# renjie-liang/HUAL

Hardware: AMD Instinct MI355X
Metric: train clips/sec (higher is better)
Workload: dtype f32 (fp16x3 / bf16x3 split-operand MFMA, fp32 accumulate); 1 GPU; Charades-STA SeqPAN train step (fwd+bwd+clip+AdamWD, dropout 0.2), batch 64/GPU, T=128, vdim=1024, L=20, C=8, dim=128, 8 heads, 2 attention layers, random init; ONE batch resident in HBM, batch assembly (hual_assemble_batch) outside the timed region; global_batch=64, T=128, vdim=1024, L=20, parallelism=dp1, launch=hipGraph, video_dtype=f32

## Files before the change

hual_amd/csrc/heads.h:

```cpp
#pragma once
#include "common.h"
#include "rowops.h"

namespace hual {

enum { LA_MATCH_SUM = 0, LA_MASK_SUM = 1, LA_ORTHO = 2, LA_LOC = 3, LA_ALIGN = 4, LA_DENOM = 5 };

struct PoolArgs {
  const float* F2;
  const float* wp;
  const float* Wbot;
  float* alpha;
  float* pooled;
  float* PW;
};
struct AlignPool;
struct AlignPoolBwd;
int launch_pool_align_fwd(const PoolArgs& a, const AlignPool* ap, const RowSpace& rs, hipStream_t s);
struct PoolBwd {
  const float* dFuse;
  float* dPW;
  float* dF2;
  float* dwp;
};
int launch_pool_align_bwd(const PoolArgs& a, const PoolBwd& g, const AlignPool& ap, const AlignPoolBwd& ab, const RowSpace& rs, hipStream_t s);

struct MatchArgs {
  const float* fuse;
  const float* Wm;
  const float* bm;
  const float* E;
  const int32_t* labels;
  float* probs;
  float* probs2;
  float* outputs;
  float* loss_acc;
  float* part;
  const uint32_t* rng;
  float inv_tau;
};
int match_fwd_blocks(int Nv);
struct AlignSim;
int launch_match_fwd(const MatchArgs& a, const RowSpace& rs, const AlignSim* as, hipStream_t s);
struct LossTailArgs {
  float* loss_acc; const float* match_part; int match_nblk; const float* loc_part; int loc_nblk;
  float lambda, override_denom; const float* denom_dev; float* loss_out;
  const uint32_t* ovf; int novf;
  const float* align_rows; int nalign;
};
struct MatchBwd {
  const float* dOut;
  const float* dOut2;
  float* dFuse;
  float* dWm; float* dbm; float* dE;
  const float* dE_ortho;
  float* part;
  float lambda;
  int do_tail; LossTailArgs tail;
};
int match_bwd_blocks(int Nv);
int launch_match_bwd(const MatchArgs& a, const MatchBwd& g, const RowSpace& rs, hipStream_t s);
struct HeadsArgs {
  const float* h[2]; const float* w[2]; const float* b[2];
  float* logit[2];
  const float* vmask;
  const float* y1; const float* y2;
  int64_t* start_index; int64_t* end_index;
  float* ds; float* de;
  int grad_only;
  float* dZ[2];
  float* part[2];
  float* loc_part;
  float inv_batch;
  const uint32_t* ovf; int novf;
};
int launch_heads(const HeadsArgs& a, int B, int T, hipStream_t s);
int launch_loss_tail(const LossTailArgs& a, hipStream_t s);

struct AlignPool {
  const float* F2;
  const float* F1;
  const float* inner;
  float* tpre; float* vpre;
  float* that; float* vhat;
  int ld;
};
struct AlignSim {
  const float* that; const float* vhat; int Bg;
  float* dq; float* da;
  float* row_loss;
  float* dthat; float* dvhat;
  float* loss_acc;
  float scale;
  int ld;
  int row0, nrows;
};
int launch_align_sim(const AlignSim& a, hipStream_t s);
struct AlignPoolBwd {
  const float* dthat; const float* dvhat;
  float* dF2;
  float* dF1;
  const float* col_dq; const float* col_da; int col_Bg;
};

}
```

hual_amd/csrc/heads.hip:

```cpp
#include "heads.h"
#include "philox.h"
#include "prof.h"

using namespace hual;

#if defined(HUAL_STAMPS) && HUAL_STAMPS == 8
static __device__ unsigned long long g_heads_stamps[512 * 64];
extern "C" int hual_debug_stamps(unsigned long long* out, int n) {
  return (int)hipMemcpyFromSymbol(out, HIP_SYMBOL(g_heads_stamps), sizeof(unsigned long long) * (size_t)n);
}
#define HEADS_STAMP(i) do { if (threadIdx.x == 0 && blockIdx.x < 512) g_heads_stamps[blockIdx.x * 64 + (i)] = __builtin_readcyclecounter(); } while (0)
#else
#define HEADS_STAMP(i) do { } while (0)
#endif

__device__ __forceinline__ float block_sum(float v, float* sm) {
  v = wave_sum64(v);
  const int w = threadIdx.x >> 6;
  __syncthreads();
  if ((threadIdx.x & 63) == 0) sm[w] = v;
  __syncthreads();
  float s = 0.f;
  for (int i = 0; i < (int)(blockDim.x >> 6); ++i) s += sm[i];
  return s;
}
__device__ __forceinline__ double block_sum_d(double v, double* sm) {
  for (int off = 32; off >= 1; off >>= 1) v += __shfl_xor(v, off);
  const int w = threadIdx.x >> 6;
  __syncthreads();
  if ((threadIdx.x & 63) == 0) sm[w] = v;
  __syncthreads();
  double s = 0.0;
  for (int i = 0; i < (int)(blockDim.x >> 6); ++i) s += sm[i];
  return s;
}
__device__ __forceinline__ float block_max(float v, float* sm) {
  v = wave_max64(v);
  const int w = threadIdx.x >> 6;
  __syncthreads();
  if ((threadIdx.x & 63) == 0) sm[w] = v;
  __syncthreads();
  float s = -INFINITY;
  for (int i = 0; i < (int)(blockDim.x >> 6); ++i) s = fmaxf(s, sm[i]);
  return s;
}

__device__ __forceinline__ void pool_fwd_body(const PoolArgs& a, const RowSpace& rs, int b) {
  __shared__ float al[256];
  __shared__ float pooled[HUAL_D];
  __shared__ float part[HUAL_D];
  const int tid = threadIdx.x;
  const bool on = tid < 256;
  const int l32 = tid & 31, grp = tid >> 5;
  const int L = rs.L;
  const float* F = a.F2 + (size_t)(rs.Nv + b * L) * HUAL_D;
  const float* m = rs.rowmask + rs.Nv + b * L;
  if (on) {
    const float4 w4 = ld4(a.wp + 4 * l32);
    for (int l = grp; l < L; l += 8) {
      const float4 f = ld4(F + (size_t)l * HUAL_D + 4 * l32);
      const float d = half_sum32(f.x * w4.x + f.y * w4.y + f.z * w4.z + f.w * w4.w);
      if (l32 == 0) al[l] = d * m[l] + HUAL_MASK_VALUE * (1.0f - m[l]);
    }
  }
  __syncthreads();
  float mx = -INFINITY;
  for (int l = 0; l < L; ++l) mx = fmaxf(mx, al[l]);
  float sum = 0.f;
  for (int l = 0; l < L; ++l) sum += __expf(al[l] - mx);
  const float inv = 1.0f / sum;
  const int c = tid & 127, half = (tid >> 7) & 1;
  if (on && half == 0) {
    float p = 0.f;
    for (int l = 0; l < L; ++l) {
      const float alpha = __expf(al[l] - mx) * inv;
      if (c == 0) a.alpha[b * L + l] = alpha;
      p = fmaf(alpha, F[(size_t)l * HUAL_D + c], p);
    }
    pooled[c] = p;
    a.pooled[b * HUAL_D + c] = p;
  }
  __syncthreads();
  float o = 0.f;
  if (on) {
#pragma unroll 8
    for (int k = half * 64; k < half * 64 + 64; ++k) o = fmaf(pooled[k], a.Wbot[(size_t)k * HUAL_D + c], o);
    if (half) part[c] = o;
  }
  __syncthreads();
  if (on && !half) a.PW[b * HUAL_D + c] = o + part[c];
}

__device__ __forceinline__ float gumbel_noise(uint32_t w) {
  const float u = (float)(w >> 8) * 5.9604644775390625e-08f;
  return -logf(-logf(u + 1e-20f) + 1e-20f);
}
__device__ __forceinline__ void match_fwd_body(const MatchArgs& a, const RowSpace& rs, int bid, int nblk) {
  __shared__ float red[2][8];
  const int l32 = threadIdx.x & 31, grp = threadIdx.x >> 5;
  const int col = 4 * l32;
  float ce_sum = 0.f, m_sum = 0.f;
  float4 w0 = ld4(a.Wm + (col + 0) * 4), w1 = ld4(a.Wm + (col + 1) * 4), w2 = ld4(a.Wm + (col + 2) * 4), w3 = ld4(a.Wm + (col + 3) * 4);
  const float4 bm = ld4(a.bm);
  float4 e0 = ld4(a.E + col), e1 = ld4(a.E + HUAL_D + col), e2 = ld4(a.E + 2 * HUAL_D + col), e3 = ld4(a.E + 3 * HUAL_D + col);
  uint3 gk = make_uint3(0u, 0u, 0u);
  if (a.rng) gk = make_uint3(a.rng[0], a.rng[1], a.rng[2]);
  for (int row = bid * 8 + grp; row < rs.Nv; row += nblk * 8) {
    const size_t off = (size_t)row * HUAL_D + col;
    const float4 f = ld4(a.fuse + off);
    float l0 = f.x * w0.x + f.y * w1.x + f.z * w2.x + f.w * w3.x;
    float l1 = f.x * w0.y + f.y * w1.y + f.z * w2.y + f.w * w3.y;
    float l2 = f.x * w0.z + f.y * w1.z + f.z * w2.z + f.w * w3.z;
    float l3 = f.x * w0.w + f.y * w1.w + f.z * w2.w + f.w * w3.w;
    l0 = half_sum32(l0) + bm.x; l1 = half_sum32(l1) + bm.y; l2 = half_sum32(l2) + bm.z; l3 = half_sum32(l3) + bm.w;
    if (a.rng) {
      const uint4_ r = philox4x32(0u, (uint32_t)row, (uint32_t)HUAL_SITE_GUMBEL, gk.z, gk.x, gk.y);
      l0 = (l0 + gumbel_noise(r.x)) * a.inv_tau; l1 = (l1 + gumbel_noise(r.y)) * a.inv_tau;
      l2 = (l2 + gumbel_noise(r.z)) * a.inv_tau; l3 = (l3 + gumbel_noise(r.w)) * a.inv_tau;
    }
    const float mx = fmaxf(fmaxf(l0, l1), fmaxf(l2, l3));
    const float x0 = expf(l0 - mx), x1 = expf(l1 - mx), x2 = expf(l2 - mx), x3 = expf(l3 - mx);
    const float sum = x0 + x1 + x2 + x3;
    const float inv = 1.0f / sum;
    const float p0 = x0 * inv, p1 = x1 * inv, p2 = x2 * inv, p3 = x3 * inv;
    const float mk = rs.rowmask[row];
    if (l32 == 0) {
      *reinterpret_cast<float4*>(a.probs + (size_t)row * 4) = make_float4(p0, p1, p2, p3);
      if (a.probs2) *reinterpret_cast<float4*>(a.probs2 + (size_t)row * 4) = make_float4(p0, p1, p2, p3);
      if (a.labels) {
        const int lab = a.labels[row];
        const float ll = lab == 0 ? l0 : (lab == 1 ? l1 : (lab == 2 ? l2 : l3));
        ce_sum += (mx + logf(sum) - ll) * mk;
        m_sum += mk;
      }
    }
    float4 o = make_float4((f.x + p0 * e0.x + p1 * e1.x + p2 * e2.x + p3 * e3.x) * mk,
                           (f.y + p0 * e0.y + p1 * e1.y + p2 * e2.y + p3 * e3.y) * mk,
                           (f.z + p0 * e0.z + p1 * e1.z + p2 * e2.z + p3 * e3.z) * mk,
                           (f.w + p0 * e0.w + p1 * e1.w + p2 * e2.w + p3 * e3.w) * mk);
    st4(a.outputs + off, o);
  }
  if (a.labels && a.loss_acc) {
    if (l32 == 0) { red[0][grp] = ce_sum; red[1][grp] = m_sum; }
    __syncthreads();
    if (threadIdx.x == 0) {
      float c = 0.f, m = 0.f;
      for (int i = 0; i < 8; ++i) { c += red[0][i]; m += red[1][i]; }
      if (a.part) { a.part[2 * bid] = c; a.part[2 * bid + 1] = m; }
      else { atomicAdd(a.loss_acc + LA_MATCH_SUM, c); atomicAdd(a.loss_acc + LA_MASK_SUM, m); }
    }
  }
}

__device__ __forceinline__ float loss_tail_body(const LossTailArgs& a, float* sm, bool write);
__global__ __launch_bounds__(256) void match_bwd_kernel(MatchArgs a, MatchBwd g, RowSpace rs) {
  __shared__ float4 red[8][8][32];
  __shared__ float redb[8][4];
  const int l32 = threadIdx.x & 31, grp = threadIdx.x >> 5;
  const int col = 4 * l32;
  float4 w0 = ld4(a.Wm + (col + 0) * 4), w1 = ld4(a.Wm + (col + 1) * 4), w2 = ld4(a.Wm + (col + 2) * 4), w3 = ld4(a.Wm + (col + 3) * 4);
  float4 e0 = ld4(a.E + col), e1 = ld4(a.E + HUAL_D + col), e2 = ld4(a.E + 2 * HUAL_D + col), e3 = ld4(a.E + 3 * HUAL_D + col);
  const int row0 = min((int)blockIdx.x * 8 + grp, rs.Nv - 1);
  const size_t off0 = (size_t)row0 * HUAL_D + col;
  float pmk = rs.rowmask[row0];
  float4 pd = ld4(g.dOut + off0), pd2 = g.dOut2 ? ld4(g.dOut2 + off0) : f4zero();
  float4 pf = ld4(a.fuse + off0), pp = *reinterpret_cast<const float4*>(a.probs + (size_t)row0 * 4);
  float denom = 1.0f;
  if (g.do_tail) {
    __shared__ float smt[12];
    denom = loss_tail_body(g.tail, smt, blockIdx.x == 0);
  } else if (a.labels) {
    denom = a.loss_acc[LA_DENOM];
  }
  const float ce_scale = a.labels ? g.lambda / denom : 0.f;
  float4 dE0 = f4zero(), dE1 = f4zero(), dE2 = f4zero(), dE3 = f4zero();
  float4 dW0 = f4zero(), dW1 = f4zero(), dW2 = f4zero(), dW3 = f4zero();
  float db0 = 0.f, db1 = 0.f, db2 = 0.f, db3 = 0.f;
  for (int row = blockIdx.x * 8 + grp; row < rs.Nv; row += gridDim.x * 8) {
    const size_t off = (size_t)row * HUAL_D + col;
    const float mk = pmk;
    float4 d = pd;
    if (g.dOut2) d = make_float4(d.x + pd2.x, d.y + pd2.y, d.z + pd2.z, d.w + pd2.w);
    const float4 f = pf, p = pp;
    {
      const int rn = min(row + (int)gridDim.x * 8, rs.Nv - 1);
      const size_t offn = (size_t)rn * HUAL_D + col;
      pmk = rs.rowmask[rn];
      pd = ld4(g.dOut + offn);
      if (g.dOut2) pd2 = ld4(g.dOut2 + offn);
      pf = ld4(a.fuse + offn);
      pp = *reinterpret_cast<const float4*>(a.probs + (size_t)rn * 4);
    }
    d = make_float4(d.x * mk, d.y * mk, d.z * mk, d.w * mk);
    float q0 = half_sum32(d.x * e0.x + d.y * e0.y + d.z * e0.z + d.w * e0.w);
    float q1 = half_sum32(d.x * e1.x + d.y * e1.y + d.z * e1.z + d.w * e1.w);
    float q2 = half_sum32(d.x * e2.x + d.y * e2.y + d.z * e2.z + d.w * e2.w);
    float q3 = half_sum32(d.x * e3.x + d.y * e3.y + d.z * e3.z + d.w * e3.w);
    const float dot = p.x * q0 + p.y * q1 + p.z * q2 + p.w * q3;
    float dl0 = p.x * (q0 - dot), dl1 = p.y * (q1 - dot), dl2 = p.z * (q2 - dot), dl3 = p.w * (q3 - dot);
    if (a.labels) {
      const int lab = a.labels[row];
      const float cs = ce_scale * mk;
      dl0 += cs * (p.x - (lab == 0 ? 1.f : 0.f));
      dl1 += cs * (p.y - (lab == 1 ? 1.f : 0.f));
      dl2 += cs * (p.z - (lab == 2 ? 1.f : 0.f));
      dl3 += cs * (p.w - (lab == 3 ? 1.f : 0.f));
    }
    if (a.rng) { dl0 *= a.inv_tau; dl1 *= a.inv_tau; dl2 *= a.inv_tau; dl3 *= a.inv_tau; }
    st4(g.dFuse + off, make_float4(d.x + dl0 * w0.x + dl1 * w0.y + dl2 * w0.z + dl3 * w0.w,
                                   d.y + dl0 * w1.x + dl1 * w1.y + dl2 * w1.z + dl3 * w1.w,
                                   d.z + dl0 * w2.x + dl1 * w2.y + dl2 * w2.z + dl3 * w2.w,
                                   d.w + dl0 * w3.x + dl1 * w3.y + dl2 * w3.z + dl3 * w3.w));
    dE0 = make_float4(dE0.x + p.x * d.x, dE0.y + p.x * d.y, dE0.z + p.x * d.z, dE0.w + p.x * d.w);
    dE1 = make_float4(dE1.x + p.y * d.x, dE1.y + p.y * d.y, dE1.z + p.y * d.z, dE1.w + p.y * d.w);
    dE2 = make_float4(dE2.x + p.z * d.x, dE2.y + p.z * d.y, dE2.z + p.z * d.z, dE2.w + p.z * d.w);
    dE3 = make_float4(dE3.x + p.w * d.x, dE3.y + p.w * d.y, dE3.z + p.w * d.z, dE3.w + p.w * d.w);
    dW0 = make_float4(dW0.x + f.x * dl0, dW0.y + f.y * dl0, dW0.z + f.z * dl0, dW0.w + f.w * dl0);
    dW1 = make_float4(dW1.x + f.x * dl1, dW1.y + f.y * dl1, dW1.z + f.z * dl1, dW1.w + f.w * dl1);
    dW2 = make_float4(dW2.x + f.x * dl2, dW2.y + f.y * dl2, dW2.z + f.z * dl2, dW2.w + f.w * dl2);
    dW3 = make_float4(dW3.x + f.x * dl3, dW3.y + f.y * dl3, dW3.z + f.z * dl3, dW3.w + f.w * dl3);
    if (l32 == 0) { db0 += dl0; db1 += dl1; db2 += dl2; db3 += dl3; }
  }
  red[0][grp][l32] = dE0; red[1][grp][l32] = dE1; red[2][grp][l32] = dE2; red[3][grp][l32] = dE3;
  red[4][grp][l32] = dW0; red[5][grp][l32] = dW1; red[6][grp][l32] = dW2; red[7][grp][l32] = dW3;
  if (l32 == 0) { redb[grp][0] = db0; redb[grp][1] = db1; redb[grp][2] = db2; redb[grp][3] = db3; }
  __syncthreads();
  float* part = g.part + (size_t)blockIdx.x * 9 * HUAL_D;
  for (int idx = threadIdx.x; idx < 8 * 128; idx += 256) {
    const int vec = idx >> 7, c = idx & 127;
    float s = 0.f;
#pragma unroll
    for (int k = 0; k < 8; ++k) s += reinterpret_cast<const float*>(&red[vec][k][c >> 2])[c & 3];
    if (vec < 4) {
      if (g.dE_ortho && blockIdx.x == 0) s += g.dE_ortho[vec * HUAL_D + c];
      part[vec * HUAL_D + c] = s;
    } else {
      part[4 * HUAL_D + c * 4 + (vec - 4)] = s;
    }
  }
  if (threadIdx.x < HUAL_D) {
    float s = 0.f;
    if (threadIdx.x < 4)
      for (int k = 0; k < 8; ++k) s += redb[k][threadIdx.x];
    part[8 * HUAL_D + threadIdx.x] = s;
  }
}

__device__ __forceinline__ void block_max2(float& a, float& b, float* sm) {
  a = wave_max64(a); b = wave_max64(b);
  const int w = threadIdx.x >> 6, nw = blockDim.x >> 6;
  __syncthreads();
  if ((threadIdx.x & 63) == 0) { sm[w] = a; sm[nw + w] = b; }
  __syncthreads();
  float x = -INFINITY, y = -INFINITY;
  for (int i = 0; i < nw; ++i) { x = fmaxf(x, sm[i]); y = fmaxf(y, sm[nw + i]); }
  a = x; b = y;
}
__device__ __forceinline__ void block_sum2_d(double& a, double& b, double* sm) {
  for (int off = 32; off >= 1; off >>= 1) { a += __shfl_xor(a, off); b += __shfl_xor(b, off); }
  const int w = threadIdx.x >> 6, nw = blockDim.x >> 6;
  __syncthreads();
  if ((threadIdx.x & 63) == 0) { sm[w] = a; sm[nw + w] = b; }
  __syncthreads();
  double x = 0.0, y = 0.0;
  for (int i = 0; i < nw; ++i) { x += sm[i]; y += sm[nw + i]; }
  a = x; b = y;
}
__device__ __forceinline__ void block_sum3(float& a, float& b, float& c, float* sm) {
  a = wave_sum64(a); b = wave_sum64(b); c = wave_sum64(c);
  const int w = threadIdx.x >> 6, nw = blockDim.x >> 6;
  __syncthreads();
  if ((threadIdx.x & 63) == 0) { sm[w] = a; sm[nw + w] = b; sm[2 * nw + w] = c; }
  __syncthreads();
  float x = 0.f, y = 0.f, z = 0.f;
  for (int i = 0; i < nw; ++i) { x += sm[i]; y += sm[nw + i]; z += sm[2 * nw + i]; }
  a = x; b = y; c = z;
}

template <int NR>
__global__ __launch_bounds__(512) void heads_kernel(HeadsArgs a, int T, int B) {
  __shared__ float zs_[256], ze_[256], ps[256], pe[256], dls[256], dle[256];
  __shared__ float sm[24];
  __shared__ double smd[16];
  __shared__ float wtot[2][4];
  __shared__ float bestv[2][4];
  __shared__ int besti[2][4];
  __shared__ float4 red[2][16][32];
  __shared__ float redb[2][16];
  const int b = xcd_tile(blockIdx.x, gridDim.x), tid = threadIdx.x;
  if (b >= B) return;
  const int l32 = tid & 31, grp = tid >> 5;
  const int col = 4 * l32;
  HEADS_STAMP(0);
  float4 hs[NR], he[NR];
  float4 ws = f4zero(), we = f4zero();
  float poison = 0.f;
  if (a.ovf) {
    bool bad = false;
    for (int i = tid & 63; i < a.novf; i += 64) bad |= a.ovf[i] != 0u;
    if (__any(bad)) poison = __builtin_nanf("");
  }
  if (a.h[0]) {
    ws = ld4(a.w[0] + col); we = ld4(a.w[1] + col);
#pragma unroll
    for (int u = 0; u < NR; ++u) {
      const int t = min(grp + 16 * u, T - 1);
      hs[u] = ld4(a.h[0] + (size_t)(b * T + t) * HUAL_D + col);
      he[u] = ld4(a.h[1] + (size_t)(b * T + t) * HUAL_D + col);
    }
  }
  if (a.grad_only) {
    if (tid < T) { dls[tid] = a.ds[b * T + tid]; dle[tid] = a.de[b * T + tid]; }
  } else if (a.h[0]) {
    const float bs = a.b[0][0] + poison, be = a.b[1][0] + poison;
#pragma unroll
    for (int u = 0; u < NR; ++u) {
      const int t = grp + 16 * u;
      const float ds = half_sum32(hs[u].x * ws.x + hs[u].y * ws.y + hs[u].z * ws.z + hs[u].w * ws.w) + bs;
      const float de = half_sum32(he[u].x * we.x + he[u].y * we.y + he[u].z * we.z + he[u].w * we.w) + be;
      if (l32 == 0 && t < T) { zs_[t] = ds; ze_[t] = de; a.logit[0][b * T + t] = ds; a.logit[1][b * T + t] = de; }
    }
  } else if (tid < T) {
    zs_[tid] = a.logit[0][b * T + tid];
    ze_[tid] = a.logit[1][b * T + tid];
  }
  __syncthreads();
  HEADS_STAMP(1);
  if (!a.grad_only) {
    const int t = tid;
    const bool in = t < T;
    const float m = in ? a.vmask[b * T + t] : 0.f;
    float zs = -INFINITY, ze = -INFINITY;
    if (in) {
      zs = zs_[t] * m + HUAL_MASK_VALUE * (1.0f - m);
      ze = ze_[t] * m + HUAL_MASK_VALUE * (1.0f - m);
    }
    float mxs = zs, mxe = ze;
    block_max2(mxs, mxe, sm);
    const float xs = in ? (float)exp((double)(zs - mxs)) : 0.f;
    const float xe = in ? (float)exp((double)(ze - mxe)) : 0.f;
    double dss = (double)xs, dse = (double)xe;
    block_sum2_d(dss, dse, smd);
    const float sums = (float)dss, sume = (float)dse;
    const float p_s = __fdiv_rn(xs, sums), p_e = __fdiv_rn(xe, sume);
    HEADS_STAMP(2);
    if (a.y1) {
      const float y1 = in ? a.y1[b * T + t] : 0.f, y2 = in ? a.y2[b * T + t] : 0.f;
      const float lsm_s = zs - mxs - logf(sums), lsm_e = ze - mxe - logf(sume);
      float lsum = in ? -(y1 * lsm_s + y2 * lsm_e) : 0.f, y1s = y1, y2s = y2;
      block_sum3(lsum, y1s, y2s, sm);
      if (t == 0 && a.loc_part) a.loc_part[b] = lsum * a.inv_batch;
      if (in) {
        const float ds = (p_s * y1s - y1) * m * a.inv_batch, de = (p_e * y2s - y2) * m * a.inv_batch;
        dls[t] = ds; dle[t] = de;
        if (a.ds) { a.ds[b * T + t] = ds; a.de[b * T + t] = de; }
      }
    }
    HEADS_STAMP(3);
    if (tid < 256) {
      const int lane = tid & 63, w = tid >> 6;
      float pre = in ? p_s : 0.f, suf = in ? p_e : 0.f;
#pragma unroll
      for (int off = 1; off < 64; off <<= 1) {
        const float up = __shfl_up(pre, off), dn = __shfl_down(suf, off);
        if (lane >= off) pre = fmaxf(pre, up);
        if (lane + off < 64) suf = fmaxf(suf, dn);
      }
      if (lane == 63) wtot[0][w] = pre;
      if (lane == 0) wtot[1][w] = suf;
      ps[tid] = pre; pe[tid] = suf;
    }
    const int nanlogit = __syncthreads_or(in && (zs_[t] != zs_[t] || ze_[t] != ze_[t]));
    float vs = -1.f, ve = -1.f;
    if (in) {
      const int w = t >> 6;
      float premax = ps[t], sufmax = pe[t];
      for (int k = 0; k < w; ++k) premax = fmaxf(premax, wtot[0][k]);
      for (int k = w + 1; k < 4; ++k) sufmax = fmaxf(sufmax, wtot[1][k]);
      vs = p_s * sufmax;
      ve = premax * p_e;
    }
    if (tid < 256) {
      int is = t, ie = t;
      for (int off = 32; off >= 1; off >>= 1) {
        float ovs = __shfl_xor(vs, off); int ois = __shfl_xor(is, off);
        if (ovs > vs || (ovs == vs && ois < is)) { vs = ovs; is = ois; }
        float ove = __shfl_xor(ve, off); int oie = __shfl_xor(ie, off);
        if (ove > ve || (ove == ve && oie < ie)) { ve = ove; ie = oie; }
      }
      if ((t & 63) == 0) { bestv[0][t >> 6] = vs; besti[0][t >> 6] = is; bestv[1][t >> 6] = ve; besti[1][t >> 6] = ie; }
    }
    __syncthreads();
    if (t == 0) {
      float v = bestv[0][0]; int i = besti[0][0];
      for (int w = 1; w < 4; ++w) if (bestv[0][w] > v || (bestv[0][w] == v && besti[0][w] < i)) { v = bestv[0][w]; i = besti[0][w]; }
      a.start_index[b] = i;
      v = bestv[1][0]; i = besti[1][0];
      for (int w = 1; w < 4; ++w) if (bestv[1][w] > v || (bestv[1][w] == v && besti[1][w] < i)) { v = bestv[1][w]; i = besti[1][w]; }
      a.end_index[b] = i;
      if (poison != poison || nanlogit) { a.start_index[b] = -1; a.end_index[b] = -1; }
    }
  } else {
    __syncthreads();
  }
  HEADS_STAMP(4);
  HEADS_STAMP(5);
  if (a.dZ[0] && (a.y1 || a.grad_only)) {
    float4 dws = f4zero(), dwe = f4zero();
    float dbs = 0.f, dbe = 0.f;
#pragma unroll
    for (int u = 0; u < NR; ++u) {
      const int tt = grp + 16 * u;
      if (tt >= T) continue;
      const size_t off = (size_t)(b * T + tt) * HUAL_D + col;
      const float dl0 = dls[tt], dl1 = dle[tt];
      st4(a.dZ[0] + off, make_float4(hs[u].x > 0.f ? dl0 * ws.x : 0.f, hs[u].y > 0.f ? dl0 * ws.y : 0.f, hs[u].z > 0.f ? dl0 * ws.z : 0.f,
                                     hs[u].w > 0.f ? dl0 * ws.w : 0.f));
      st4(a.dZ[1] + off, make_float4(he[u].x > 0.f ? dl1 * we.x : 0.f, he[u].y > 0.f ? dl1 * we.y : 0.f, he[u].z > 0.f ? dl1 * we.z : 0.f,
                                     he[u].w > 0.f ? dl1 * we.w : 0.f));
      dws = make_float4(dws.x + dl0 * hs[u].x, dws.y + dl0 * hs[u].y, dws.z + dl0 * hs[u].z, dws.w + dl0 * hs[u].w);
      dwe = make_float4(dwe.x + dl1 * he[u].x, dwe.y + dl1 * he[u].y, dwe.z + dl1 * he[u].z, dwe.w + dl1 * he[u].w);
      if (l32 == 0) { dbs += dl0; dbe += dl1; }
    }
    red[0][grp][l32] = dws; red[1][grp][l32] = dwe;
    if (l32 == 0) { redb[0][grp] = dbs; redb[1][grp] = dbe; }
    __syncthreads();
    if (tid < 256) {
      const int hd = tid >> 7, c = tid & 127;
      float sw = 0.f;
#pragma unroll
      for (int k = 0; k < 16; ++k) sw += reinterpret_cast<const float*>(&red[hd][k][c >> 2])[c & 3];
      float sb = 0.f;
      if (c == 0)
        for (int k = 0; k < 16; ++k) sb += redb[hd][k];
      float* part = a.part[hd] + (size_t)b * 2 * HUAL_D;
      part[c] = sw;
      part[HUAL_D + c] = sb;
    }
  }
  HEADS_STAMP(6);
}

__device__ __forceinline__ float loss_tail_body(const LossTailArgs& a, float* sm, bool write) {
  const int tid = threadIdx.x;
  float cs = 0.f, ms = 0.f, ls = 0.f;
  for (int i = tid; i < a.match_nblk; i += 256) { cs += a.match_part[2 * i]; ms += a.match_part[2 * i + 1]; }
  if (write)
    for (int i = tid; i < a.loc_nblk; i += 256) ls += a.loc_part[i];
  int bad = 0;
  if (write) {
    for (int i = tid; i < a.novf; i += 256) bad |= a.ovf[i] != 0u;
    bad = __syncthreads_or(bad);
  }
  block_sum3(cs, ms, ls, sm);
  const float denom = a.denom_dev ? *a.denom_dev : (a.override_denom > 0.f ? a.override_denom : ms + 1e-12f);
  if (write && tid == 0) {
    float* la = a.loss_acc;
    la[LA_MATCH_SUM] = cs; la[LA_MASK_SUM] = ms; la[LA_LOC] = ls;
    la[LA_DENOM] = denom;
    if (a.align_rows) {
      float l = 0.f;
      for (int i = 0; i < a.nalign; ++i) l += a.align_rows[i];
      la[LA_ALIGN] = l;
    }
    if (a.loss_out) {
      const float match = cs / denom + la[LA_ORTHO];
      const float align = la[LA_ALIGN];
      const float poison = bad ? __builtin_nanf("") : 0.f;
      a.loss_out[0] = ls + a.lambda * match + align + poison;
      a.loss_out[1] = ls + poison;
      a.loss_out[2] = match + poison;
      a.loss_out[3] = align + poison;
    }
  }
  return denom;
}
__global__ __launch_bounds__(256) void loss_tail_kernel(LossTailArgs a) {
  __shared__ float sm[12];
  loss_tail_body(a, sm, true);
}

#define L2_EPS 1e-12f
__device__ __forceinline__ void align_pool_body(const AlignPool& a, const RowSpace& rs, int b) {
  __shared__ float sm[8];
  __shared__ float part[2][4][HUAL_D];
  const int c = threadIdx.x & 127, grp = threadIdx.x >> 7;
  const int L = rs.L, T = rs.T;
  float tc = 0.f, vc = 0.f;
  for (int l = threadIdx.x; l < L; l += 512) tc += rs.rowmask[rs.Nv + b * L + l];
  for (int t = threadIdx.x; t < T; t += 512) vc += rs.rowmask[b * T + t];
  tc = block_sum(tc, sm);
  vc = block_sum(vc, sm);
  float ts = 0.f, vs = 0.f;
#pragma unroll 8
  for (int l = grp; l < L; l += 4) ts += a.F2[(size_t)(rs.Nv + b * L + l) * HUAL_D + c];
#pragma unroll 8
  for (int t = grp; t < T; t += 4) vs += a.F1[(size_t)(b * T + t) * HUAL_D + c] * (a.inner[b * T + t] / vc);
  part[0][grp][c] = ts;
  part[1][grp][c] = vs;
  __syncthreads();
  ts = part[0][0][c] + part[0][1][c] + part[0][2][c] + part[0][3][c];
  vs = part[1][0][c] + part[1][1][c] + part[1][2][c] + part[1][3][c];
  const float tp = ts / tc;
  const float tn = block_sum(grp == 0 ? tp * tp : 0.f, sm);
  const float vn = block_sum(grp == 0 ? vs * vs : 0.f, sm);
  if (grp == 0) {
    a.tpre[b * HUAL_D + c] = tp;
    a.vpre[b * HUAL_D + c] = vs;
    a.that[(size_t)b * a.ld + c] = tp * rsqrtf(fmaxf(tn, L2_EPS));
    a.vhat[(size_t)b * a.ld + c] = vs * rsqrtf(fmaxf(vn, L2_EPS));
  }
}

__device__ __forceinline__ double block_max_d(double v, double* sm) {
  for (int off = 32; off >= 1; off >>= 1) v = fmax(v, __shfl_xor(v, off));
  const int w = threadIdx.x >> 6;
  __syncthreads();
  if ((threadIdx.x & 63) == 0) sm[w] = v;
  __syncthreads();
  double s = sm[0];
  for (int i = 1; i < (int)(blockDim.x >> 6); ++i) s = fmax(s, sm[i]);
  return s;
}
__device__ __forceinline__ void align_sim_rows_body(const AlignSim& a, int i) {
  __shared__ float ti[HUAL_D], vi[HUAL_D];
  __shared__ double sm[4];
  __shared__ double sa[1024], sq[1024];
  const int tid = threadIdx.x, Bg = a.Bg;
  const int ld = a.ld;
  if (tid < HUAL_D) { ti[tid] = a.that[(size_t)i * ld + tid]; vi[tid] = a.vhat[(size_t)i * ld + tid]; }
  __syncthreads();
  double mxa = -INFINITY, mxq = -INFINITY;
  for (int j0 = 0; j0 < Bg; j0 += 64) {
    const int j = j0 + (tid >> 2), kq = (tid & 3) * 32;
    const float* vj = a.vhat + (size_t)min(j, Bg - 1) * ld + kq;
    double da = 0.0, dq = 0.0;
#pragma unroll 8
    for (int k = 0; k < 32; ++k) { const double v = (double)vj[k]; da = fma((double)vi[kq + k], v, da); dq = fma((double)ti[kq + k], v, dq); }
    da += __shfl_xor(da, 1); dq += __shfl_xor(dq, 1);
    da += __shfl_xor(da, 2); dq += __shfl_xor(dq, 2);
    if ((tid & 3) == 0 && j < Bg) { sa[j] = da; sq[j] = dq; }
  }
  __syncthreads();
  for (int j = tid; j < Bg; j += 256) { mxa = fmax(mxa, sa[j]); mxq = fmax(mxq, sq[j]); }
  mxa = block_max_d(mxa, sm);
  mxq = block_max_d(mxq, sm);
  double suma = 0.0, sumq = 0.0;
  for (int j = tid; j < Bg; j += 256) { suma += exp(sa[j] - mxa); sumq += exp(sq[j] - mxq); }
  suma = block_sum_d(suma, sm);
  sumq = block_sum_d(sumq, sm);
  const double lsa = mxa + log(suma), lsq = mxq + log(sumq);
  double li = 0.0, dotq = 0.0, dota = 0.0;
  for (int j = tid; j < Bg; j += 256) {
    const double lpv = sa[j] - lsa, lpq = sq[j] - lsq;
    const double pv = exp(lpv), pq = exp(lpq);
    li += pq * lpq + pv * lpv - 2.0 * pq * pv;
    dotq += pq * (lpq + 1.0 - 2.0 * pv);
    dota += pv * (lpv + 1.0 - 2.0 * pq);
  }
  li = block_sum_d(li, sm);
  dotq = block_sum_d(dotq, sm);
  dota = block_sum_d(dota, sm);
  if (tid == 0) {
    if (a.row_loss) a.row_loss[i] = (float)li;
    else if (a.loss_acc) atomicAdd(a.loss_acc + LA_ALIGN, (float)li);
  }
  __syncthreads();
  for (int j = tid; j < Bg; j += 256) {
    const double lpv = sa[j] - lsa, lpq = sq[j] - lsq;
    const double pv = exp(lpv), pq = exp(lpq);
    const double gq = pq * ((lpq + 1.0 - 2.0 * pv) - dotq) * (double)a.scale;
    const double ga = pv * ((lpv + 1.0 - 2.0 * pq) - dota) * (double)a.scale;
    a.dq[(size_t)i * Bg + j] = (float)gq;
    a.da[(size_t)i * Bg + j] = (float)ga;
    sq[j] = gq; sa[j] = ga;
  }
  __syncthreads();
  if (tid < HUAL_D && i >= a.row0 && i < a.row0 + a.nrows) {
    double st = 0.0, sv = 0.0;
#pragma unroll 8
    for (int j = 0; j < Bg; ++j) {
      const double v = (double)a.vhat[(size_t)j * ld + tid];
      st = fma(sq[j], v, st);
      sv = fma(sa[j], v, sv);
    }
    a.dthat[(i - a.row0) * HUAL_D + tid] = (float)st;
    a.dvhat[(i - a.row0) * HUAL_D + tid] = (float)sv;
  }
}
__global__ __launch_bounds__(256) void align_sim_rows_kernel(AlignSim a) { align_sim_rows_body(a, blockIdx.x); }
__global__ __launch_bounds__(256) void match_align_fwd_kernel(MatchArgs ma, RowSpace rs, AlignSim as, int nmatch) {
  if ((int)blockIdx.x < nmatch) match_fwd_body(ma, rs, blockIdx.x, nmatch);
  else align_sim_rows_body(as, (int)blockIdx.x - nmatch);
}
__global__ __launch_bounds__(256) void align_sim_cols_kernel(AlignSim a) {
  __shared__ float cq[1024], ca[1024];
  __shared__ float part[HUAL_D];
  const int j = a.row0 + blockIdx.x, c = threadIdx.x & 127, half = threadIdx.x >> 7, Bg = a.Bg, ld = a.ld;
  for (int i = threadIdx.x; i < Bg; i += 256) { cq[i] = a.dq[(size_t)i * Bg + j]; ca[i] = a.da[(size_t)i * Bg + j]; }
  __syncthreads();
  float s = 0.f;
#pragma unroll 4
  for (int i = half; i < Bg; i += 2)
    s += cq[i] * a.that[(size_t)i * ld + c] + ca[i] * a.vhat[(size_t)i * ld + c];
  if (half) part[c] = s;
  __syncthreads();
  if (!half) a.dvhat[blockIdx.x * HUAL_D + c] += s + part[c];
  if (a.row_loss && blockIdx.x == 0 && threadIdx.x == 0) {
    float l = 0.f;
    for (int i = 0; i < Bg; ++i) l += a.row_loss[i];
    a.loss_acc[LA_ALIGN] = l;
  }
}

__global__ __launch_bounds__(512) void pool_align_fwd_kernel(PoolArgs pa, AlignPool ap, RowSpace rs) {
  const int clip = xcd_tile(blockIdx.x, gridDim.x);
  if (clip >= rs.B) return;
  if (blockIdx.y == 0) {
    pool_fwd_body(pa, rs, clip);
  } else {
    align_pool_body(ap, rs, clip);
  }
}
template <int KT, int KL>
__global__ __launch_bounds__(512) void pool_align_bwd_kernel(PoolArgs pa, PoolBwd pb, AlignPool ap, AlignPoolBwd ab, RowSpace rs) {
  __shared__ float sm[48];
  __shared__ float part[4][HUAL_D];
  __shared__ float vecs[2][HUAL_D];
  __shared__ float da[256], al[256], qm[256], dap[2][256];
  const int b = xcd_tile(blockIdx.x, gridDim.x), tid = threadIdx.x;
  if (b >= rs.B) return;
  const int c = tid & 127, grp = tid >> 7;
  const int L = rs.L, T = rs.T;
  const size_t vrow0 = (size_t)b * T, qrow0 = (size_t)rs.Nv + (size_t)b * L;
  __shared__ float inl[256];
  float rdf[KT], rf1[KT], rF[KL];
#pragma unroll
  for (int k = 0; k < KT; ++k) {
    const int t = min(grp + 4 * k, T - 1);
    rdf[k] = pb.dFuse[(vrow0 + t) * HUAL_D + c];
    rf1[k] = ab.dF1[(vrow0 + t) * HUAL_D + c];
  }
  for (int t = tid; t < T; t += 512) inl[t] = ap.inner[vrow0 + t];
#pragma unroll
  for (int k = 0; k < KL; ++k) rF[k] = pa.F2[(qrow0 + min(grp + 4 * k, L - 1)) * HUAL_D + c];
  const float tp = ap.tpre[b * HUAL_D + c], vp = ap.vpre[b * HUAL_D + c];
  const float th = ap.that[(size_t)b * ap.ld + c], vh = ap.vhat[(size_t)b * ap.ld + c];
  const float dth = ab.dthat[b * HUAL_D + c];
  float dvh = ab.dvhat[b * HUAL_D + c];
  const float wpc = pa.wp[c];
  float tc = 0.f, vc = 0.f;
  for (int l = tid; l < L; l += 512) { const float m = rs.rowmask[qrow0 + l]; qm[l] = m; al[l] = pa.alpha[b * L + l]; tc += m; }
  for (int t = tid; t < T; t += 512) vc += rs.rowmask[vrow0 + t];
  float colsum = 0.f;
  if (ab.col_dq) {
    const int Bg = ab.col_Bg;
#pragma unroll 4
    for (int i = grp; i < Bg; i += 4)
      colsum += ab.col_dq[(size_t)i * Bg + b] * ap.that[(size_t)i * ap.ld + c] + ab.col_da[(size_t)i * Bg + b] * ap.vhat[(size_t)i * ap.ld + c];
  }
  float sdf = 0.f;
#pragma unroll
  for (int k = 0; k < KT; ++k) sdf += (grp + 4 * k < T) ? rdf[k] : 0.f;
  part[grp][c] = sdf;
  __syncthreads();
  const float dpw = (part[0][c] + part[1][c]) + (part[2][c] + part[3][c]);
  if (grp == 0) { pb.dPW[b * HUAL_D + c] = dpw; vecs[1][c] = dpw; }
  __syncthreads();
  if (ab.col_dq) {
    part[grp][c] = colsum;
    __syncthreads();
    dvh += (part[0][c] + part[1][c]) + (part[2][c] + part[3][c]);
    __syncthreads();
  }
  {
    const float w0 = grp == 0 ? 1.f : 0.f;
    float v[6] = {w0 * tp * tp, w0 * vp * vp, w0 * th * dth, w0 * vh * dvh, tc, vc};
#pragma unroll
    for (int q = 0; q < 6; ++q) v[q] = wave_sum64(v[q]);
    if ((tid & 63) == 0)
      for (int q = 0; q < 6; ++q) sm[q * 8 + (tid >> 6)] = v[q];
  }
  __syncthreads();
  float red6[6];
#pragma unroll
  for (int q = 0; q < 6; ++q) {
    float x = 0.f;
    for (int w = 0; w < 8; ++w) x += sm[q * 8 + w];
    red6[q] = x;
  }
  const float tn = red6[0], vn = red6[1], tdot = red6[2], vdot = red6[3];
  tc = red6[4]; vc = red6[5];
  const float rt = rsqrtf(fmaxf(tn, L2_EPS)), rv = rsqrtf(fmaxf(vn, L2_EPS));
  const float dtp = tn > L2_EPS ? (float)((double)rt * ((double)dth - (double)th * (double)tdot)) : rt * dth;
  const float dvp = vn > L2_EPS ? (float)((double)rv * ((double)dvh - (double)vh * (double)vdot)) : rv * dvh;
  const float dts = dtp / tc;
#pragma unroll
  for (int k = 0; k < KT; ++k) {
    const int t = grp + 4 * k;
    if (t < T) ab.dF1[(vrow0 + t) * HUAL_D + c] = rf1[k] + dvp * (inl[t] / vc);
  }
  {
    float dp = 0.f;
    const float* wrow = pa.Wbot + (size_t)c * HUAL_D + grp * 32;
#pragma unroll
    for (int n = 0; n < 32; n += 4) {
      const float4 w = ld4(wrow + n);
      const float* d = vecs[1] + grp * 32 + n;
      dp += d[0] * w.x + d[1] * w.y + d[2] * w.z + d[3] * w.w;
    }
    part[grp][c] = dp;
  }
  __syncthreads();
  const float dpc = (part[0][c] + part[1][c]) + (part[2][c] + part[3][c]);
  __syncthreads();
#pragma unroll
  for (int k = 0; k < KL; ++k) {
    const int l = grp + 4 * k;
    const float d = wave_sum64(dpc * rF[k]);
    if ((tid & 63) == 0 && l < L) dap[(tid >> 6) & 1][l] = d;
  }
  __syncthreads();
  if (tid < L) da[tid] = dap[0][tid] + dap[1][tid];
  __syncthreads();
  float dot_acc = 0.f;
  for (int l = 0; l < L; ++l) dot_acc += al[l] * da[l];
  float dw = 0.f;
#pragma unroll
  for (int k = 0; k < KL; ++k) {
    const int l = grp + 4 * k;
    if (l >= L) continue;
    const float alpha = al[l];
    const float dal = alpha * (da[l] - dot_acc) * qm[l];
    ab.dF2[(qrow0 + l) * HUAL_D + c] = dts + alpha * dpc + dal * wpc;
    dw = fmaf(dal, rF[k], dw);
  }
  part[grp][c] = dw;
  __syncthreads();
  if (grp == 0) atomicAdd(pb.dwp + c, (part[0][c] + part[1][c]) + (part[2][c] + part[3][c]));
}

namespace hual {

int launch_pool_align_fwd(const PoolArgs& a, const AlignPool* ap, const RowSpace& rs, hipStream_t s) {
  HUAL_REQUIRE(rs.L <= 256, "pool: L <= 256");
  AlignPool z{};
  HUAL_LAUNCH(0.0, 512.0 * (rs.Nq + (ap ? rs.R : 0) + 4.0 * rs.B), pool_align_fwd_kernel, dim3(xcd_round8(rs.B), ap ? 2 : 1), dim3(512), 0, s, a, ap ? *ap : z, rs);
  HUAL_CHECK_HIP(hipGetLastError());
  return 0;
}
int launch_pool_align_bwd(const PoolArgs& a, const PoolBwd& g, const AlignPool& ap, const AlignPoolBwd& ab, const RowSpace& rs, hipStream_t s) {
  HUAL_REQUIRE(rs.T <= 256 && rs.L <= 256, "pool_align_bwd: T, L <= 256");
  HUAL_REQUIRE(ab.dF2 == g.dF2, "pool_align_bwd: the two parts write the same query rows");
  const double pab = 512.0 * (3.0 * rs.Nv + 2.0 * rs.Nq);
#define PAB(KT, KL) HUAL_LAUNCH(0.0, pab, (pool_align_bwd_kernel<KT, KL>), dim3(xcd_round8(rs.B)), dim3(512), 0, s, a, g, ap, ab, rs)
  if (rs.T <= 128) {
    if (rs.L <= 32) PAB(32, 8); else if (rs.L <= 64) PAB(32, 16); else if (rs.L <= 128) PAB(32, 32); else PAB(64, 64);
  } else {
    if (rs.L <= 32) PAB(64, 8); else if (rs.L <= 64) PAB(64, 16); else if (rs.L <= 128) PAB(64, 32); else PAB(64, 64);
  }
#undef PAB
  HUAL_CHECK_HIP(hipGetLastError());
  return 0;
}
static int rowgrid(int R, int cap) {
  int g = cdiv(R, 8);
  return g < cap ? (g > 0 ? g : 1) : cap;
}
int match_fwd_blocks(int Nv) { return rowgrid(Nv, 512); }
int match_bwd_blocks(int Nv) { return rowgrid(Nv, 256); }
int launch_match_fwd(const MatchArgs& a, const RowSpace& rs, const AlignSim* as, hipStream_t s) {
  HUAL_REQUIRE(a.part != nullptr, "match_fwd: partial-sum scratch");
  const int nm = match_fwd_blocks(rs.Nv);
  AlignSim z{};
  if (as) {
    HUAL_REQUIRE(as->Bg >= 1 && as->Bg <= 1024 && as->ld >= HUAL_D && as->row0 == 0 && as->nrows == as->Bg, "align: global batch <= 1024");
    z = *as;
  }
  HUAL_LAUNCH(0.0, (1024.0 + 32.0) * rs.Nv, match_align_fwd_kernel, dim3(nm + (as ? as->Bg : 0)), dim3(256), 0, s, a, rs, z, nm);
  HUAL_CHECK_HIP(hipGetLastError());
  return 0;
}
int launch_match_bwd(const MatchArgs& a, const MatchBwd& g, const RowSpace& rs, hipStream_t s) {
  HUAL_REQUIRE(g.part != nullptr, "match_bwd: partial-sum scratch");
  HUAL_LAUNCH(0.0, 4.0 * 512.0 * rs.Nv, match_bwd_kernel, dim3(match_bwd_blocks(rs.Nv)), dim3(256), 0, s, a, g, rs);
  HUAL_CHECK_HIP(hipGetLastError());
  return 0;
}
int launch_heads(const HeadsArgs& a, int B, int T, hipStream_t s) {
  HUAL_REQUIRE(T >= 1 && T <= 256 && B >= 1, "heads: T <= 256");
  HUAL_REQUIRE(a.grad_only ? (a.ds && a.de && a.dZ[0]) : (a.logit[0] && a.logit[1] && a.vmask && a.start_index && a.end_index), "heads: null tensor");
  HUAL_REQUIRE(!a.h[0] || (a.h[1] && a.w[0] && a.w[1] && a.b[0] && a.b[1]), "heads: hidden layers incomplete");
  HUAL_REQUIRE(!a.dZ[0] || (a.dZ[1] && a.part[0] && a.part[1] && a.h[0]), "heads: gradient outputs incomplete");
  const double hb = (a.dZ[0] ? 4.0 : 2.0) * 512.0 * B * T + 16.0 * B * T;
  if (T <= 128) HUAL_LAUNCH(0.0, hb, heads_kernel<8>, dim3(xcd_round8(B)), dim3(512), 0, s, a, T, B);
  else HUAL_LAUNCH(0.0, hb, heads_kernel<16>, dim3(xcd_round8(B)), dim3(512), 0, s, a, T, B);
  HUAL_CHECK_HIP(hipGetLastError());
  return 0;
}
int launch_loss_tail(const LossTailArgs& a, hipStream_t s) {
  HUAL_REQUIRE(a.loss_acc && a.match_part && a.loc_part, "loss_tail: null");
  HUAL_LAUNCH(0.0, 0.0, loss_tail_kernel, dim3(1), dim3(256), 0, s, a);
  HUAL_CHECK_HIP(hipGetLastError());
  return 0;
}
int launch_align_sim(const AlignSim& a, hipStream_t s) {
  HUAL_REQUIRE(a.Bg >= 1 && a.Bg <= 1024, "align: global batch <= 1024");
  HUAL_REQUIRE(a.ld >= HUAL_D && a.row0 >= 0 && a.nrows >= 1 && a.row0 + a.nrows <= a.Bg, "align: row window / leading dimension");
  HUAL_LAUNCH(0.0, 0.0, align_sim_rows_kernel, dim3(a.Bg), dim3(256), 0, s, a);
  HUAL_LAUNCH(0.0, 0.0, align_sim_cols_kernel, dim3(a.nrows), dim3(256), 0, s, a);
  HUAL_CHECK_HIP(hipGetLastError());
  return 0;
}

}
```

hual_amd/csrc/mproj.hip:

```cpp
#include "mproj.h"
#include "tilecore.h"
#include "prof.h"
#include <cstdlib>
#include <cstddef>

using namespace hual;

#define ld4 ld4_global
#define st4 st4_global

#define MP_ROWS 64
enum { MPF_A2 = 1, MPF_BF16 = 2, MPF_DROP = 4, MPF_ADD = 8, MPF_LN = 16, MPF_REUSE = 32, MPF_QUAD = 64, MPF_POOL = 128 };

template <int NT, int F>
__device__ __forceinline__ void mproj_body(const MProjArgs& a, const DropCfg& drop, int tile = -1) {
  extern __shared__ __attribute__((aligned(16))) char mp_lds[];
  char* S0 = mp_lds;
  char* S1 = S0 + 2 * MP_ROWS * 256;
  float* ainv0 = reinterpret_cast<float*>(S1 + 2 * MP_ROWS * 256);
  float* ainv1 = ainv0 + MP_ROWS;
  const int lane = threadIdx.x & 63, wave = threadIdx.x >> 6;
  const int l32 = threadIdx.x & 31, grp = threadIdx.x >> 5;
  const int col = 4 * l32;
  const int MT = a.MT, R = a.R;
  if (tile < 0) {
    const int nblk = xcd_round8((R + MT - 1) / MT);
    if ((int)blockIdx.x >= nblk) return;
    tile = xcd_tile(blockIdx.x, nblk);
  }
  const int r0 = tile * MT;
  if (r0 >= R) return;
  const int RE = min(R, r0 + MT);
  const int j = lane & 15, g = lane >> 4, ecol = 16 * wave + 4 * g;
  const DropRegs dr = drop_load(drop);
  constexpr int NU = NT;

  constexpr int SW = sizeof(MProjStep) / 4;
  __shared__ uint32_t sdesc[MP_MAX * SW];
  {
    const uint32_t* ka = reinterpret_cast<const uint32_t*>(&a.s[0]);
    for (int i = threadIdx.x; i < a.nsteps * SW; i += CB_THREADS) sdesc[i] = ka[i];
  }
  __syncthreads();
  static_assert(SW <= 64, "a step descriptor fits one dword per lane");
  auto step_at = [&](int si) {
    struct alignas(8) Raw { uint32_t w[SW]; } r;
    const uint32_t mine = sdesc[si * SW + min(lane, SW - 1)];
#pragma unroll
    for (int q = 0; q < SW; ++q) r.w[q] = __builtin_amdgcn_readlane(mine, q);
    return __builtin_bit_cast(MProjStep, r);
  };
  int nflat = 0;
  for (int i = 0; i < a.nsteps; ++i) nflat += (int)__builtin_amdgcn_readfirstlane(sdesc[i * SW + offsetof(MProjStep, rep) / 4]);
  auto expand = [&](int si, int ri) {
    MProjStep st = step_at(si);
    if (st.rep > 1) {
      st.A = st.a_bf16 ? (const void*)(reinterpret_cast<const uint16_t*>(st.A) + 128 * ri) : (const void*)(reinterpret_cast<const float*>(st.A) + 128 * ri);
      st.kw = min(128, st.ktot - 128 * ri);
      st.col0 += 128 * ri;
      st.wimg = reinterpret_cast<const float*>(reinterpret_cast<const char*>(st.wimg) + (size_t)ri * 128 * 512);
      st.first = st.first && ri == 0;
      st.last = st.last && ri == st.rep - 1;
    }
    return st;
  };
  TfW wc, wn;
  tf_load_w(wc, step_at(0).wimg, wave, lane);
  float4 nv[NU], n2[NU];
  auto rows_load = [&](const MProjStep& st) {
    const int kc = min(col, max(st.kw - 4, 0));
#pragma unroll
    for (int u = 0; u < NU; ++u) {
      const size_t row = (size_t)min(r0 + grp + 16 * u, R - 1);
      if ((F & MPF_BF16) && st.a_bf16) {
        const uint2 raw = ld2_global(reinterpret_cast<const uint16_t*>(st.A) + row * st.lda + kc);
        nv[u] = make_float4(__uint_as_float(raw.x), __uint_as_float(raw.y), 0.f, 0.f);
      } else {
        nv[u] = ld4(reinterpret_cast<const float*>(st.A) + row * st.lda + kc);
      }
      if (F & MPF_A2) {
        const float* p2 = st.A2 ? st.A2 : reinterpret_cast<const float*>(st.A);
        const int ld2 = st.A2 ? st.lda2 : st.lda;
        n2[u] = ld4(p2 + row * ld2 + kc);
      }
    }
  };
  auto fill = [&](const MProjStep& st, int slot) {
    char* S = slot ? S1 : S0;
    float* ai = slot ? ainv1 : ainv0;
    const bool cin = col < st.kw;
    uint32_t nb[4] = {15u, 15u, 15u, 15u};
    constexpr int NPR = (NU + 1) / 2;
    if ((F & MPF_DROP) && st.drop_site >= 0 && dr.enabled) {
      const uint32_t c4 = (uint32_t)((st.col0 + col) >> 2);
#pragma unroll
      for (int pr = 0; pr < NPR; ++pr) {
        const int lrA = grp + 32 * pr, lrB = lrA + 16;
        const bool okA = cin && lrA < MT && r0 + lrA < RE, okB = cin && lrB < MT && r0 + lrB < RE;
        uint32_t na, nbb;
        const uint32_t byte = drop_nib2_r(dr, (uint32_t)st.drop_site, a.drop_row0 + (uint32_t)(r0 + lrA), a.drop_row0 + (uint32_t)(r0 + lrB), c4, na, nbb);
        nb[2 * pr] = na; nb[2 * pr + 1] = nbb;
        if (st.keep_out) {
          const bool odd = (c4 & 1u) != 0u;
          if (odd ? okB : okA) st1b_global(st.keep_out + (size_t)(r0 + (odd ? lrB : lrA)) * st.ld_keep + (c4 >> 1), (uint8_t)byte);
        }
      }
    }
#pragma unroll
    for (int u = 0; u < NU; ++u) {
      const int lr = grp + 16 * u, row = r0 + lr;
      const bool ok = row < RE && cin && lr < MT;
      float4 v = nv[u];
      if ((F & MPF_BF16) && st.a_bf16) {
        const uint32_t w0 = __float_as_uint(v.x), w1 = __float_as_uint(v.y);
        v = make_float4(__uint_as_float(w0 << 16), __uint_as_float(w0 & 0xffff0000u), __uint_as_float(w1 << 16), __uint_as_float(w1 & 0xffff0000u));
      }
      if ((F & MPF_A2) && st.A2) v = cb_mul(v, n2[u]);
      if (!ok) v = f4zero();
      if ((F & MPF_DROP) && st.drop_site >= 0 && dr.enabled) v = f4_select(nb[u], make_float4(v.x * dr.scale, v.y * dr.scale, v.z * dr.scale, v.w * dr.scale));
      const float inv = cb_store_operand(S, S + MP_ROWS * 256, lr, l32, v);
      if (l32 == 0) ai[lr] = row < RE ? inv : 0.f;
    }
  };
#define MP_STAMP(i) HUAL_STAMP_K(9, i)
  MP_STAMP(0);
  MProjStep cur = expand(0, 0);
  rows_load(cur);
  fill(cur, 0);
  MP_STAMP(1);
  int slot = 0, si = 0, ri = 0;
  float4 acc[NT];
  float4 qd[(F & MPF_QUAD) ? 4 : 1][NT];
  float4 lastb = f4zero();
  constexpr bool QPRE = (F & MPF_QUAD) && NT <= 3;
  float4 qx[QPRE ? NT : 1], qc[QPRE ? NT : 1], qq[QPRE ? NT : 1];
  if (QPRE && a.quad_x) {
#pragma unroll
    for (int rt = 0; rt < NT; ++rt) {
      const size_t off = (size_t)min(r0 + 16 * rt + j, R - 1) * HUAL_D + ecol;
      qx[rt] = ld4(a.quad_x + off); qc[rt] = ld4(a.quad_c2q + off); qq[rt] = ld4(a.quad_q2c + off);
    }
  }
#pragma unroll
  for (int rt = 0; rt < NT; ++rt) acc[rt] = f4zero();
#pragma unroll 1
  for (int k = 0; k < nflat; ++k) {
    MP_STAMP(2 + 7 * k);
    const MProjStep st = cur;
    const bool more = k + 1 < nflat;
    MProjStep nxt = st;
    if (more) {
      if (++ri == (int)__builtin_amdgcn_readfirstlane(sdesc[si * SW + offsetof(MProjStep, rep) / 4])) { ri = 0; ++si; }
      nxt = expand(si, ri);
    }
    MP_STAMP(3 + 7 * k);
    const bool closes = st.last && st.out && ecol < st.ncol;
    const float* wdummy = st.wimg + 4 * lane;
    const float4 bias = ld4(st.bias ? st.bias + ecol : wdummy);
    float4 addv[NT];
    if (F & MPF_ADD) {
#pragma unroll
      for (int rt = 0; rt < NT; ++rt) {
        const int row = min(r0 + 16 * rt + j, R - 1);
        addv[rt] = ld4((st.add && closes) ? st.add + (size_t)(row / st.add_div) * st.ldadd + ecol : wdummy);
      }
    }
    tf_load_w(wn, nxt.wimg, wave, lane);
    bool refill = true;
    if (F & MPF_REUSE) {
      refill = more && !nxt.reuse;
      if (refill) rows_load(nxt);
    } else {
      rows_load(nxt);
    }
    MP_STAMP(4 + 7 * k);
    cb_barrier();
    MP_STAMP(5 + 7 * k);
    const char* S = slot ? S1 : S0;
    const float* ai = slot ? ainv1 : ainv0;
    f32x4 accp[NT];
    tf_mma<NT, MP_ROWS * 256>(S, wc, lane, accp);
    MP_STAMP(6 + 7 * k);
#pragma unroll
    for (int rt = 0; rt < NT; ++rt) {
      const float ir = ai[16 * rt + j];
      const float4 o = st.first ? f4zero() : acc[rt];
      acc[rt] = make_float4(fmaf(accp[rt][0], ir, o.x), fmaf(accp[rt][1], ir, o.y), fmaf(accp[rt][2], ir, o.z), fmaf(accp[rt][3], ir, o.w));
    }
    lastb = st.bias ? bias : f4zero();
    {
      float* outp = st.out ? st.out : const_cast<float*>(wdummy);
#pragma unroll
      for (int rt = 0; rt < NT; ++rt) {
        const int row = r0 + 16 * rt + j;
        float4 v = st.bias ? cb_add(acc[rt], bias) : acc[rt];
        if (st.act) v = relu_nan4(v);
        if ((F & MPF_ADD) && st.add) v = cb_add(v, addv[rt]);
        if (closes && 16 * rt + j < MT && row < RE) st4(outp + (size_t)row * st.ldo + ecol, v);
        if (F & MPF_QUAD) {
#pragma unroll
          for (int q = 0; q < 4; ++q) if (k == q) qd[q][rt] = v;
        }
      }
    }
    MP_STAMP(7 + 7 * k);
    if (refill && more) { slot ^= 1; fill(nxt, slot); }
    MP_STAMP(8 + 7 * k);
    wc = wn;
    cur = nxt;
  }
  if ((F & MPF_QUAD) && a.quad_x) {
#pragma unroll
    for (int rt = 0; rt < NT; ++rt) {
      const int row = r0 + 16 * rt + j;
      if (16 * rt + j >= MT || row >= RE) continue;
      const size_t off = (size_t)row * HUAL_D + ecol;
      const float4 x = QPRE ? qx[QPRE ? rt : 0] : ld4(a.quad_x + off), c2q = QPRE ? qc[QPRE ? rt : 0] : ld4(a.quad_c2q + off),
                   q2c = QPRE ? qq[QPRE ? rt : 0] : ld4(a.quad_q2c + off);
      const float4 d0 = qd[0][rt], d1 = qd[1][rt], d2 = qd[2][rt], d3 = qd[3][rt];
      st4(a.quad_dc2q + off, make_float4(d1.x + d2.x * x.x, d1.y + d2.y * x.y, d1.z + d2.z * x.z, d1.w + d2.w * x.w));
      st4(a.quad_dq2c + off, make_float4(d3.x * x.x, d3.y * x.y, d3.z * x.z, d3.w * x.w));
      st4(a.quad_dx + off, make_float4(d0.x + d2.x * c2q.x + d3.x * q2c.x, d0.y + d2.y * c2q.y + d3.y * q2c.y,
                                       d0.z + d2.z * c2q.z + d3.z * q2c.z, d0.w + d2.w * c2q.w + d3.w * q2c.w));
    }
    return;
  }
  if ((F & MPF_POOL) && a.pool_cat) {
    const float4 bias = lastb;
    const int C = a.pool_C;
#pragma unroll
    for (int rt = 0; rt < NT; ++rt) {
      const int lr = 16 * rt + j, row = r0 + lr;
      const int p = lr & (C - 1);
      const float4 v4 = cb_add(acc[rt], bias);
      const float vv[4] = {v4.x, v4.y, v4.z, v4.w};
      float best[4];
      int arg[4];
#pragma unroll
      for (int q = 0; q < 4; ++q) {
        const int ch = ecol + q;
        const int k = ch < 10 ? 1 : (ch < 30 ? 2 : (ch < 60 ? 3 : 4));
        best[q] = (p + k <= C) ? vv[q] : -INFINITY;
        arg[q] = p;
      }
      auto merge = [&](int step) {
#pragma unroll
        for (int q = 0; q < 4; ++q) {
          const float ov = dpp_xor_partner(best[q], step);
          const int oa = __builtin_bit_cast(int, dpp_xor_partner(__builtin_bit_cast(float, arg[q]), step));
          const bool take = ov > best[q] || (ov == best[q] && oa < arg[q]);
          best[q] = take ? ov : best[q];
          arg[q] = take ? oa : arg[q];
        }
      };
      if (C > 1) merge(1);
      if (C > 2) merge(2);
      if (C > 4) merge(4);
      if (C > 8) merge(8);
      if (p == 0 && lr < MT && row < RE && ecol < 100) {
        const int word = row / C;
        float o[4];
        int oa[4];
#pragma unroll
        for (int q = 0; q < 4; ++q) {
          const bool pos = best[q] > 0.f;
          o[q] = pos ? best[q] : 0.f;
          oa[q] = pos ? arg[q] : -1;
        }
        float* cp = a.pool_cat + (size_t)word * a.pool_ldcat + a.pool_col0 + ecol;
        if (((a.pool_ldcat | a.pool_col0) & 3) == 0) st4(cp, make_float4(o[0], o[1], o[2], o[3]));
        else { st1f_global(cp, o[0]); st1f_global(cp + 1, o[1]); st1f_global(cp + 2, o[2]); st1f_global(cp + 3, o[3]); }
        st4i_global(a.pool_arg + (size_t)word * 100 + ecol, oa[0], oa[1], oa[2], oa[3]);
      }
    }
    return;
  }
  if (!(F & MPF_LN) || !a.ln_g) return;
  float4* D0 = reinterpret_cast<float4*>(S0);
  cb_barrier();
  {
#pragma unroll
    for (int rt = 0; rt < NT; ++rt) D0[(16 * rt + j) * 32 + (ecol >> 2)] = cb_add(acc[rt], lastb);
  }
  const float4 gam = ld4(a.ln_g + col), bet = ld4(a.ln_b + col);
  cb_barrier();
#pragma unroll
  for (int u = 0; u < NU; ++u) {
    const int lr = grp + 16 * u, row = r0 + lr;
    if (lr >= MT || row >= RE) continue;
    const float4 x = D0[lr * 32 + l32];
    float mean, rstd;
    const float m0 = fast_sum32(cb_hsum(x)) * (1.0f / HUAL_D);
    const float4 d = make_float4(x.x - m0, x.y - m0, x.z - m0, x.w - m0);
    const float var = fast_sum32(cb_hsum(cb_mul(d, d))) * (1.0f / HUAL_D);
    mean = m0; rstd = rsqrtf(var + LN_EPS);
    float4 y = cb_fma(make_float4(d.x * rstd, d.y * rstd, d.z * rstd, d.w * rstd), gam, bet);
    if (a.pos) y = cb_add(y, ld4(a.pos + (size_t)((row + a.row_in_clip0) % a.Tc) * HUAL_D + col));
    const size_t off = (size_t)row * HUAL_D + col;
    if (a.x_out) st4(a.x_out + off, x);
    st4(a.y_out + off, y);
    if (l32 == 0) { st1f_global(a.mean + row, mean); st1f_global(a.rstd + row, rstd); }
  }
}

template <int NT, int F>
__global__ __launch_bounds__(CB_THREADS) void mproj_kernel(MProjArgs a, DropCfg drop) { mproj_body<NT, F>(a, drop); }
__host__ __device__ inline int mproj_pair_lo(int nb, int x) { return nb * x / 8; }
template <int NT, int F>
__global__ __launch_bounds__(CB_THREADS) void mproj_pair_kernel(MProjArgs a0, MProjArgs a1, DropCfg drop) {
  const int x = blockIdx.x & 7;
  int sl = blockIdx.x >> 3;
  const int nb0 = (a0.R + a0.MT - 1) / a0.MT, nb1 = (a1.R + a1.MT - 1) / a1.MT;
  const int lo0 = mproj_pair_lo(nb0, x), n0 = mproj_pair_lo(nb0, x + 1) - lo0;
  if (sl < n0) { mproj_body<NT, F>(a0, drop, lo0 + sl); return; }
  sl -= n0;
  const int lo1 = mproj_pair_lo(nb1, x), n1 = mproj_pair_lo(nb1, x + 1) - lo1;
  if (sl < n1) mproj_body<NT, F>(a1, drop, lo1 + sl);
}

#undef ld4
#undef st4

#if defined(HUAL_STAMPS) && HUAL_STAMPS == 9
extern "C" int hual_debug_stamps(unsigned long long* out, int n) {
  return (int)hipMemcpyFromSymbol(out, HIP_SYMBOL(g_hual_stamps), sizeof(unsigned long long) * (size_t)n);
}
#endif

namespace hual {

static int mproj_pair_grid(int R0, int R1, int t) {
  const int nb0 = cdiv(R0, t), nb1 = cdiv(R1, t);
  int m = 0;
  for (int x = 0; x < 8; ++x) {
    const int n = (mproj_pair_lo(nb0, x + 1) - mproj_pair_lo(nb0, x)) + (mproj_pair_lo(nb1, x + 1) - mproj_pair_lo(nb1, x));
    m = n > m ? n : m;
  }
  return 8 * m;
}
int mproj_rows(int R0, int R1) {
  int t = 16;
  if (R1 > 0) { while (t < MP_ROWS && mproj_pair_grid(R0, R1, t) > 256) ++t; }
  else { while (t < MP_ROWS && cdiv(R0, t) > 256) ++t; }
  return t;
}

static int check_mproj(const MProjArgs& a, double& flops, double& bytes, int& feat) {
  HUAL_REQUIRE(a.nsteps >= 1 && a.nsteps <= MP_MAX && a.R > 0 && a.MT >= 1 && a.MT <= MP_ROWS, "mproj: steps / rows");
  HUAL_REQUIRE(a.s[0].first && !a.s[0].reuse && a.s[a.nsteps - 1].last, "mproj: first step starts a tile, last step closes one");
  for (int k = 0; k < a.nsteps; ++k) {
    const MProjStep& s = a.s[k];
    HUAL_REQUIRE(s.rep >= 1 && (s.rep == 1 || (!s.reuse && s.ktot > 128 * (s.rep - 1) && s.ktot <= 128 * s.rep && (s.ktot % 4) == 0 && !s.A2)), "mproj: repetitions");
    HUAL_REQUIRE(s.reuse || (s.A && (s.rep > 1 || (s.kw >= 4 && s.kw <= 128 && (s.kw % 4) == 0)) && (s.lda % 4) == 0), "mproj: operand");
    HUAL_REQUIRE(!s.reuse || k > 0, "mproj: nothing to reuse");
    HUAL_REQUIRE(s.wimg && s.wrows >= 1, "mproj: weight image");
    feat |= (s.A2 ? MPF_A2 : 0) | (s.a_bf16 ? MPF_BF16 : 0) | (s.drop_site >= 0 ? MPF_DROP : 0) | (s.add ? MPF_ADD : 0) | (s.reuse ? MPF_REUSE : 0);
    HUAL_REQUIRE(!s.last || (a.ln_g && k == a.nsteps - 1 && !s.out) || (a.quad_x && !s.out) || (a.pool_cat && k == a.nsteps - 1 && !s.out) ||
                 (s.out && (s.ldo % 4) == 0 && s.ncol >= 4 && s.ncol <= 128 && (s.ncol % 4) == 0), "mproj: closing step needs a destination");
    HUAL_REQUIRE(!s.add || s.add_div >= 1, "mproj: add_div");
    HUAL_REQUIRE(k == 0 || s.first == a.s[k - 1].last, "mproj: a tile starts exactly behind a closed one");
    const double kdeep = s.rep > 1 ? s.ktot : (s.reuse ? a.s[k - 1].kw : s.kw);
    flops += 2.0 * a.R * kdeep * 128.0;
    if (!s.reuse) bytes += (s.a_bf16 ? 2.0 : 4.0) * a.R * kdeep + (s.A2 ? 4.0 * a.R * kdeep : 0.0);
    bytes += 4.0 * 128.0 * (s.rep > 1 ? s.ktot : (s.wrows < 128 ? s.wrows : 128));
    if (s.last && s.out) bytes += 4.0 * a.R * s.ncol;
  }
  if (a.quad_x) {
    feat |= MPF_QUAD;
    HUAL_REQUIRE(a.nsteps == 4 && a.quad_c2q && a.quad_q2c && a.quad_dc2q && a.quad_dq2c && a.quad_dx && !a.ln_g, "mproj: quad epilogue");
    for (int k = 0; k < 4; ++k) HUAL_REQUIRE(a.s[k].first && a.s[k].last && a.s[k].rep == 1 && !a.s[k].out, "mproj: quad epilogue takes four closing steps");
    bytes += 4.0 * a.R * 128.0 * 6.0;
  }
  if (a.pool_cat) {
    feat |= MPF_POOL;
    const int C = a.pool_C;
    HUAL_REQUIRE(a.pool_arg && (C == 1 || C == 2 || C == 4 || C == 8 || C == 16) && (a.MT % C) == 0 && (a.R % C) == 0 && !a.ln_g && !a.quad_x,
                 "mproj: pool epilogue needs a power-of-two window count <= 16 that divides the rows of a workgroup");
    bytes += 8.0 * (a.R / C) * 100.0;
  }
  if (a.ln_g) {
    feat |= MPF_LN;
    HUAL_REQUIRE(a.ln_b && a.y_out && a.mean && a.rstd && (!a.pos || a.Tc >= 1), "mproj: layer-norm outputs");
    bytes += 4.0 * a.R * 128.0 * (a.x_out ? 2.0 : 1.0);
  }
  return 0;
}

int launch_mproj(const MProjArgs* a, int nprob, const DropCfg& drop, hipStream_t s) {
  HUAL_REQUIRE(a && (nprob == 1 || nprob == 2), "mproj: one or two problems");
  double flops = 0.0, bytes = 0.0;
  int blocks = 0, feat = 0;
  for (int i = 0; i < nprob; ++i) {
    int rc = check_mproj(a[i], flops, bytes, feat);
    if (rc) return rc;
    const int nb = cdiv(a[i].R, a[i].MT);
    blocks = nb > blocks ? nb : blocks;
  }
  blocks = xcd_round8(blocks);
  const size_t lds = (size_t)4 * MP_ROWS * 256 + 2 * MP_ROWS * sizeof(float);
  if (nprob == 2) HUAL_REQUIRE(a[0].MT == a[1].MT, "mproj: problems of one launch share the rows per workgroup");
  const int nt = (a[0].MT + 15) / 16;
  const int fsets[] = {0, MPF_REUSE, MPF_A2, MPF_ADD, MPF_REUSE | MPF_ADD, MPF_A2 | MPF_BF16 | MPF_DROP | MPF_ADD | MPF_LN | MPF_REUSE,
                       MPF_REUSE | MPF_QUAD};
  int fs = 5;
  for (int i = 4; i >= 0; --i) if ((feat & ~fsets[i]) == 0) fs = i;
  if (feat & MPF_QUAD) {
    HUAL_REQUIRE((feat & ~fsets[6]) == 0, "mproj: the quad epilogue goes with plain / reused operands only");
    fs = 6;
  }
  if (feat & MPF_POOL) {
    HUAL_REQUIRE(feat == MPF_POOL, "mproj: the pool epilogue goes with plain operands only");
    fs = 7;
  }
#define MPROJ_LAUNCH(NT, FS)                                                                                               \
  do {                                                                                                                     \
    HUAL_DYN_LDS((mproj_kernel<NT, FS>), 96 * 1024);                                                                       \
    HUAL_DYN_LDS((mproj_pair_kernel<NT, FS>), 96 * 1024);                                                                  \
    if (nprob == 1) HUAL_LAUNCH(flops, bytes, (mproj_kernel<NT, FS>), dim3(blocks), dim3(CB_THREADS), lds, s, a[0], drop); \
    else HUAL_LAUNCH(flops, bytes, (mproj_pair_kernel<NT, FS>), dim3(mproj_pair_grid(a[0].R, a[1].R, a[0].MT)), dim3(CB_THREADS), lds, s, a[0], a[1], drop); \
  } while (0)
#define MPROJ_NT(FS)                                                                                                       \
  do {                                                                                                                     \
    if (nt <= 2) MPROJ_LAUNCH(2, FS);                                                                                      \
    else if (nt == 3) MPROJ_LAUNCH(3, FS);                                                                                 \
    else MPROJ_LAUNCH(4, FS);                                                                                              \
  } while (0)
  static_assert(MPF_A2 == 1 && MPF_ADD == 8 && MPF_REUSE == 32 && MPF_QUAD == 64 && MPF_POOL == 128 && (MPF_A2 | MPF_BF16 | MPF_DROP | MPF_ADD | MPF_LN | MPF_REUSE) == 63,
                "feature-set literals below");
  switch (fs) {
    case 0: MPROJ_NT(0); break;
    case 1: MPROJ_NT(32); break;
    case 2: MPROJ_NT(1); break;
    case 3: MPROJ_NT(8); break;
    case 4: MPROJ_NT(40); break;
    case 6: MPROJ_NT(96); break;
    case 7: MPROJ_NT(128); break;
    default: MPROJ_NT(63); break;
  }
#undef MPROJ_NT
#undef MPROJ_LAUNCH
  HUAL_CHECK_HIP(hipGetLastError());
  return 0;
}

}
```

hual_amd/csrc/prof.cpp:

```cpp
#include <stdlib.h>
#include "prof.h"
#include <map>
#include <string>
#include <vector>
#include <string.h>
#include "../../include/hual_seqpan.h"

namespace hual {

namespace {
struct Rec { std::string name; hipEvent_t a, b; double flops, bytes; };
struct Agg { std::string name; int64_t launches = 0; double usec = 0.0, flops = 0.0, bytes = 0.0; };
struct State {
  bool on = false;
  std::vector<Rec> recs;
  std::vector<Agg> aggs;
};
thread_local State g_prof;

std::string clean(const char* s) {
  std::string n(s);
  while (!n.empty() && (n.front() == '(' || n.front() == ' ')) n.erase(n.begin());
  while (!n.empty() && (n.back() == ')' || n.back() == ' ')) n.pop_back();
  return n;
}
}

bool prof_on() { return g_prof.on; }
bool lds_poison_on() {
  static const bool on = getenv("HUAL_DEBUG_LDS_POISON") != nullptr && atoi(getenv("HUAL_DEBUG_LDS_POISON")) != 0;
  return on;
}

void prof_events(const char* name, double flops, double bytes, hipEvent_t* start, hipEvent_t* stop) {
  *start = *stop = nullptr;
  hipEvent_t a, b;
  if (hipEventCreate(&a) != hipSuccess) return;
  if (hipEventCreate(&b) != hipSuccess) { hipEventDestroy(a); return; }
  g_prof.recs.push_back(Rec{clean(name), a, b, flops, bytes});
  *start = a;
  *stop = b;
}

}

extern "C" {

int hual_prof_begin(void) {
  hual::g_prof.on = true;
  hual::g_prof.recs.clear();
  hual::g_prof.aggs.clear();
  return 0;
}

int hual_prof_end(void) {
  using namespace hual;
  g_prof.on = false;
  std::map<std::string, size_t> idx;
  g_prof.aggs.clear();
  for (auto& r : g_prof.recs) {
    hipEventSynchronize(r.b);
    float ms = 0.f;
    const bool ok = hipEventElapsedTime(&ms, r.a, r.b) == hipSuccess;
    auto it = idx.find(r.name);
    if (it == idx.end()) {
      it = idx.emplace(r.name, g_prof.aggs.size()).first;
      g_prof.aggs.push_back(Agg{r.name});
    }
    Agg& a = g_prof.aggs[it->second];
    if (ok) { a.launches += 1; a.usec += (double)ms * 1e3; a.flops += r.flops; a.bytes += r.bytes; }
    hipEventDestroy(r.a);
    hipEventDestroy(r.b);
  }
  g_prof.recs.clear();
  return (int)g_prof.aggs.size();
}

int hual_prof_get(int i, char* name, int name_cap, int64_t* launches, double* usec, double* flops, double* bytes) {
  using namespace hual;
  if (i < 0 || i >= (int)g_prof.aggs.size() || !name || name_cap < 1) return HUAL_ERR_INVALID;
  const Agg& a = g_prof.aggs[i];
  strncpy(name, a.name.c_str(), (size_t)name_cap - 1);
  name[name_cap - 1] = 0;
  if (launches) *launches = a.launches;
  if (usec) *usec = a.usec;
  if (flops) *flops = a.flops;
  if (bytes) *bytes = a.bytes;
  return 0;
}

int hual_prof_kernel_pipe(const char* kernel, int* pipe, int* passes) {
  if (!kernel || !pipe || !passes) return HUAL_ERR_INVALID;
  struct Row { const char* prefix; int pipe, passes; };
  static const Row rows[] = {
      {"conv_block_", HUAL_PIPE_MATRIX16, 3}, {"ln_proj", HUAL_PIPE_MATRIX16, 3}, {"da_post", HUAL_PIPE_MATRIX16, 3},
      {"da_mid_bwd", HUAL_PIPE_MATRIX16, 3},  {"ln2_mid_bwd", HUAL_PIPE_MATRIX16, 3}, {"mproj_", HUAL_PIPE_MATRIX16, 3},
      {"feature_", HUAL_PIPE_MATRIX16, 3},    {"dw_f16_", HUAL_PIPE_MATRIX16, 3},
      {"attn_", HUAL_PIPE_MATRIX16, 3},      {"cq_fwd_staged", HUAL_PIPE_MATRIX16, 3}, {"cq_bwd_staged", HUAL_PIPE_MATRIX16, 3},
      {"cq_fwd_wide", HUAL_PIPE_MATRIX16, 3}, {"cq_bwd_wide", HUAL_PIPE_MATRIX16, 3},
      {"cq_", HUAL_PIPE_MATRIX32, 1},
  };
  for (const Row& r : rows)
    if (strncmp(kernel, r.prefix, strlen(r.prefix)) == 0) { *pipe = r.pipe; *passes = r.passes; return 0; }
  *pipe = HUAL_PIPE_NONE; *passes = 0;
  return 0;
}

}
```

hual_amd/csrc/seqpan.hip:

```cpp
#include "attn.h"
#include "prof.h"
#include "cq.h"
#include "convblock.h"
#include "dablock.h"
#include "embed.h"
#include "gemm.h"
#include "heads.h"
#include "mproj.h"
#include "optim.h"
#include "params.h"
#include "rowops.h"
#include <stdlib.h>
#include <string.h>
#include <algorithm>
#include <unordered_map>
#include <vector>

namespace hual {
const char* last_error_cstr();
}
using namespace hual;

namespace {

// ... 68 lines not shown
  int part_seq = 0;
  void stage(int st, int sub = 0) { active = sel_stage < 0 || st == ST_ALWAYS || (st == sel_stage && (st != ST_DA || sub == sel_sub)); }
  bool stage_on(int st, int sub = 0) const { return sel_stage < 0 || (st == sel_stage && (st != ST_DA || sub == sel_sub)); }
  bool live() const { return !dry && active && rc == 0; }
  void push_dw(const DwJob& j) { if (active) dwjobs.push_back(j); }

  void ln_bwd(const LnBwd& a0) {
    LnBwd a = a0;
    const int nblk = ln_bwd_blocks(a.R);
    a.part = buf("part." + std::to_string(part_seq++), (size_t)nblk * 4, HUAL_D);
    ColsumJob cj{};
    cj.src = a.part; cj.nblk = nblk; cj.nvec = 4;
    cj.dst[0] = a.dg1; cj.dst[1] = a.db1; cj.dst[2] = a.dg2; cj.dst[3] = a.db2;
    if (active) colsum.push_back(cj);
    if (live()) chk(launch_ln_bwd(a, drop, stream));
  }
  void ln_bwd_split(const LnBwd& a0, float* dg_lo, float* db_lo, float* dg_hi, float* db_hi, const PosBwdJob* pos = nullptr, int npos = 0) {
    LnBwd a = a0;
    const int nlo = ln_bwd_blocks(a.split), nhi = ln_bwd_blocks(a.R - a.split);
    a.part = buf("part." + std::to_string(part_seq++), (size_t)(nlo + nhi) * 4, HUAL_D);
    ColsumJob cj{};
    cj.src = a.part; cj.nblk = nlo; cj.nvec = 4;
    cj.dst[0] = dg_lo; cj.dst[1] = db_lo;
    if (active) colsum.push_back(cj);
    cj.src = a.part + (size_t)nlo * 4 * HUAL_D; cj.nblk = nhi;
    cj.dst[0] = dg_hi; cj.dst[1] = db_hi;
    if (active) colsum.push_back(cj);
    if (live()) chk(launch_ln_bwd(a, drop, stream, pos, npos, &rs));
  }
  void ln_proj_bwd(const LnProjBwdArgs& a0, float* dg1, float* db1, float* dg2, float* db2) {
    LnProjBwdArgs a = a0;
    a.MT = ln_proj_bwd_rows(a.R, a.Nv);
    const int nblk = ln_proj_bwd_blocks(a.R, a.Nv);
    a.part = buf("part." + std::to_string(part_seq++), (size_t)nblk * 4, HUAL_D);
    ColsumJob cj{};
    cj.src = a.part; cj.nblk = nblk; cj.nvec = 4;
    cj.dst[0] = dg1; cj.dst[1] = db1; cj.dst[2] = dg2; cj.dst[3] = db2;
    if (active) colsum.push_back(cj);
    if (live()) chk(launch_ln_proj_bwd(a, drop, stream));
  }
  void ln2_mid_bwd(const LnProjBwdArgs& a0, const DaMidBwdArgs& m0, float* dg1, float* db1) {
    LnProjBwdArgs a = a0;
    DaMidBwdArgs m = m0;
    a.MT = ln_proj_bwd_rows(a.R, a.Nv);
    m.MT = da_post_rows(m.R, m.Nv);
    const int nblk = ln_proj_bwd_blocks(a.R, a.Nv);
    a.part = buf("part." + std::to_string(part_seq++), (size_t)nblk * 4, HUAL_D);
    ColsumJob cj{};
    cj.src = a.part; cj.nblk = nblk; cj.nvec = 4;
    cj.dst[0] = dg1; cj.dst[1] = db1;
    if (active) colsum.push_back(cj);
    if (!live()) return;
#ifndef HUAL_NO_DA_BWD_FUSE
    if (sel_stage < 0 && ln2_mid_bwd_fits(a, m)) { chk(launch_ln2_mid_bwd(a, m, drop, stream)); return; }
#endif
    chk(launch_ln_proj_bwd(a, drop, stream));
    if (ok()) chk(launch_da_mid_bwd(m, stream));
  }
  void flush_colsum(const EmbedUnpack* unpack = nullptr) {
    for (size_t i = 0; i < colsum.size() && !dry && ok(); i += HUAL_COLSUM_MAX_JOBS) {
      const bool last = i + HUAL_COLSUM_MAX_JOBS >= colsum.size();
      chk(launch_colsum(colsum.data() + i, (int)std::min<size_t>(HUAL_COLSUM_MAX_JOBS, colsum.size() - i), stream, last ? unpack : nullptr));
    }
    if (colsum.empty() && unpack && !dry && ok()) chk(launch_colsum(nullptr, 0, stream, unpack));
    colsum.clear();
  }
  void attn_fwd(const AttnJob* j, int n) { if (live()) chk(launch_attn_fwd(j, n, drop, stream)); }
  void attn_bwd(const AttnJob* j, int n) {
    if (live()) chk(launch_attn_bwd(j, n, drop, stream));
  }
};

void set_embed_scratch(EmbedArgs& ea, float* base, int Nq, int C, int char_dim) {
  const EmbedLayout el = embed_layout(Nq, C, char_dim);
  ea.cemb = base + el.cemb; ea.ball = base + el.ball;
  ea.yall = base + el.yall; ea.dxall = base + el.dxall; ea.dfall = base + el.dfall;
}
void fill_embed_args(Ctx& c, EmbedArgs& ea, const hual_batch* bt, float* cat, int catw, int32_t* char_arg, float* scratch) {
  const ParamMap& pm = c.pm;
  ea.word_ids = bt->word_ids; ea.char_ids = bt->char_ids; ea.word_table = c.word_table; ea.unk = c.p(pm.unk);
  ea.char_table = c.p(pm.char_table);
  for (int i = 0; i < 4; ++i) { ea.filt[i] = c.p(pm.filt[i]); ea.fbias[i] = c.p(pm.fbias[i]); }
  ea.cat = cat; ea.ldcat = catw; ea.char_arg = char_arg;
  set_embed_scratch(ea, scratch, c.rs.Nq, c.C, c.cfg->char_dim);
  ea.word_dim = c.cfg->word_dim; ea.char_dim = c.cfg->char_dim; ea.C = c.C; ea.num_chars = c.cfg->num_chars;
  ea.wall_img = reinterpret_cast<const float*>(c.PKT + c.wall_boff);
  ea.wall_img_t = reinterpret_cast<const float*>(c.PKN + c.wall_boff);
}
DwJob mkdw(const float* A, int lda, int K, const float* dY, int ldy, int M, float* dW, float* db, int N = HUAL_D) {
  DwJob j;
  dw_job_init(j);
  j.npieces = 1;
  j.A[0] = A; j.lda[0] = lda; j.kw[0] = K; j.dW[0] = dW; j.ldw = N;
  j.dY = dY; j.ldy = ldy; j.M = M; j.N = N; j.db = db;
  return j;
}

MProjStep mstep(const float* A, int lda, int kw, const float* img, int wrows, bool first, bool last) {
  MProjStep s{};
  s.A = A; s.lda = lda; s.kw = kw; s.wimg = img; s.wrows = wrows; s.first = first ? 1 : 0; s.last = last ? 1 : 0;
  s.drop_site = -1; s.rep = 1; s.add_div = 1; s.ncol = HUAL_D;
  return s;
}
MProjStep mstep_reuse(const float* img, int wrows, bool first, bool last) {
  MProjStep s = mstep(nullptr, 0, 0, img, wrows, first, last);
  s.reuse = 1;
  return s;
}
void mstep_out(MProjStep& s, float* out, int ldo, const float* bias = nullptr, int ncol = HUAL_D) { s.out = out; s.ldo = ldo; s.bias = bias; s.ncol = ncol; }
MProjArgs margs(int R, int R_other = 0) {
  MProjArgs a{};
  a.R = R; a.MT = mproj_rows(R, R_other); a.drop_row0 = 0;
  return a;
}

void flush_dw(Ctx& c) {
  const size_t n = c.dwjobs.size();
  if (n == 0) return;
  std::stable_sort(c.dwjobs.begin(), c.dwjobs.end(), [](const DwJob& a, const DwJob& b) { return a.M > b.M; });
  DwJob* table = reinterpret_cast<DwJob*>(c.buf("dw.table.0", 1, dw_table_words(n)));
  if (!c.dry && c.ext_table) {
    if (4 * dw_table_words(n) > c.ext_table_bytes) { c.chk(fail(HUAL_ERR_INVALID, "hual_run_opts.dw_table too small: hual_seqpan_dw_table_bytes()")); return; }
    table = reinterpret_cast<DwJob*>(c.ext_table);
  }
  if (!c.dry && c.ok()) c.chk(launch_dw(c.dwjobs.data(), (int)n, c.drop, c.stream, table, !c.static_tables));
  c.dwjobs.clear();
}

int setup_ctx(Ctx& c, const hual_cfg* cfg, int B, int T, int L, int C) {
  HUAL_REQUIRE(cfg != nullptr, "null cfg");
  int rc = build_param_map(*cfg, c.pm);
  if (rc) return rc;
  HUAL_REQUIRE(B >= 1 && T >= 1 && L >= 1, "empty batch");
  HUAL_REQUIRE(T <= cfg->max_vlen && L <= cfg->max_vlen, "sequence longer than max_vlen (assert_less_equal, modules.py:44)");
  HUAL_REQUIRE(T <= 256 && L <= 256, "T, L <= 256");
  HUAL_REQUIRE(C >= 4, "char_ids need C >= 4 (conv width 4, VALID)");
  HUAL_REQUIRE((long long)B * (T + L) * 8 < (1ll << 28), "batch too large for 32-bit RNG row ids");
  HUAL_REQUIRE((long long)B * (T + L) < (1ll << 20), "batch too large: B (T + L) < 2^20 rows (row -> clip lookups, common.h small_div)");
  c.cfg = cfg; c.B = B; c.T = T; c.L = L; c.C = C;
  {
    const ParamMap& pm = c.pm;
    const int D = HUAL_D, catw = cfg->word_dim + 100;
    c.dense.clear();
    const uint8_t TN = HUAL_PACK_T | HUAL_PACK_N;
    auto add = [&](size_t off, int K, uint8_t need) { if (K % 8 == 0) c.dense.push_back({off, K, off * 4, need}); };
    const int qks = ((catw + 3) / 4 + 63) & ~63;
    c.ksplit = (cfg->vdim % 256) == 0 && cfg->vdim <= 1024 && (catw % 8) == 0 && qks <= 256;
    add(pm.vconv.k, cfg->vdim, c.ksplit ? HUAL_PACK_F : HUAL_PACK_T);
    add(pm.qconv.k, catw, (c.ksplit ? HUAL_PACK_F : HUAL_PACK_T) | HUAL_PACK_N);
    add(pm.shid.k, 2 * D, TN); add(pm.ehid.k, 2 * D, TN);
    add(pm.fe_dense.k, D, TN); add(pm.fe_q.k, D, TN); add(pm.fe_k.k, D, TN); add(pm.fe_v.k, D, TN);
    for (int i = 0; i < 4; ++i) { add(pm.fe_cb.pw[i], D, TN); add(pm.cb.pw[i], D, TN); }
    add(pm.cqcat.k, 2 * D, TN); add(pm.cq[0].dense, 4 * D, TN); add(pm.cq[1].dense, 4 * D, TN);
    for (int li = 0; li < cfg->attn_layer; ++li) {
      const DualAttnP& d = pm.da[li];
      const size_t w[] = {d.dense1.k, d.dense2.k, d.bl1_d1, d.bl1_d2, d.bl2_d1, d.bl2_d2, d.guided.k, d.s_gate.k, d.x_gate.k,
                          d.s_dense.k, d.x_dense.k, d.query.k, d.f_key.k, d.f_value.k, d.t_key.k, d.t_value.k};
      for (size_t o : w) add(o, D, TN);
    }
    std::sort(c.dense.begin(), c.dense.end(), [](const Ctx::DenseW& a, const Ctx::DenseW& b) { return a.off < b.off; });
    size_t extra = (pm.word_table != (size_t)-1 ? pm.word_table : pm.total) * 4;
    extra = (extra + 255) & ~(size_t)255;
    for (auto& d : c.dense)
      if (d.K % 128) { d.boff = extra; extra += (size_t)((d.K + 127) / 128) * HUAL_PACK_BLOCK_BYTES; }
    c.wall_K = 4 * embed_cpad(cfg->char_dim);
    c.wall_off = (uint32_t)(extra / 4);
    c.wall_boff = (uint32_t)extra;
    const size_t wf = (size_t)c.wall_K * 512, wb = (size_t)((c.wall_K + 127) / 128) * HUAL_PACK_BLOCK_BYTES;
    extra += wf > wb ? wf : wb;
    c.pk_bytes = extra;
  }
  c.rs.B = B; c.rs.T = T; c.rs.L = L; c.rs.Nv = B * T; c.rs.Nq = B * L; c.rs.R = B * (T + L); c.rs.rowmask = nullptr;
  c.rsv = c.rs; c.rsv.Nq = 0; c.rsv.L = 0; c.rsv.R = c.rs.Nv;
  return 0;
}

struct Res {
  Ctx& c;
  bool make;
  float* operator()(const std::string& name, size_t rows, size_t cols) const { return make ? c.buf(name, rows, cols) : c.find(name); }
  float* act(const std::string& name) const { return (*this)(name, (size_t)c.rs.R, HUAL_D); }
  float* actv(const std::string& name) const { return (*this)(name, (size_t)c.rs.Nv, HUAL_D); }
  float* vec(const std::string& name) const { return (*this)(name, (size_t)c.rs.R, 1); }
  uint8_t* bits(const std::string& name, size_t rows) const { return reinterpret_cast<uint8_t*>((*this)(name, rows, 4)); }
};

struct CoreBufs { float *rowmask, *loss_acc, *ortho_dE; uint32_t* ovf; };
CoreBufs core_bufs(const Res& r) {
  Ctx& c = r.c;
  CoreBufs k{};
  k.rowmask = r.vec("rowmask"); c.rs.rowmask = k.rowmask; c.rsv.rowmask = k.rowmask;
  k.loss_acc = r("loss_acc", 8, 1);
  const size_t pkw = (c.pk_bytes + 3) / 4;
  c.PKF = reinterpret_cast<char*>(r("params.pkf", pkw, 1));
  c.PKT = reinterpret_cast<char*>(r("params.pkt", pkw, 1));
  c.PKN = reinterpret_cast<char*>(r("params.pkn", pkw, 1));
  k.ortho_dE = r("ortho.dE", 4, HUAL_D);
  std::vector<int> pkK;
  for (const auto& d : c.dense) pkK.push_back(d.K);
  pkK.push_back(c.wall_K);
  const int ovf_words = pack_ovf_words(pkK.data(), (int)pkK.size());
  k.ovf = reinterpret_cast<uint32_t*>(r("params.ovf", (size_t)ovf_words, 1));
  c.novf = (int)pkK.size() <= HUAL_MAX_PACK ? ovf_words : 0;
  return k;
}

struct InputBufs { float* cat; int32_t* char_arg; float *embed_scratch, *lin; uint8_t* vkeep; float *x0, *lin_mean, *lin_rstd, *lin_part; };
InputBufs input_bufs(const Res& r) {
  Ctx& c = r.c;
  InputBufs b{};
  b.cat = r("cat", c.rs.Nq, c.catw());
  b.char_arg = reinterpret_cast<int32_t*>(r("char_arg", c.rs.Nq, 100));
  b.embed_scratch = r("embed.scratch", embed_layout(c.rs.Nq, c.C, c.cfg->char_dim).total, 1);
  b.lin = r.act("lin");
  b.vkeep = reinterpret_cast<uint8_t*>(r("video.keep", (size_t)c.rs.Nv, (size_t)(c.cfg->vdim + 31) / 32));
  b.x0 = r.act("cb.x0");
  b.lin_mean = r.vec("lin.mean"); b.lin_rstd = r.vec("lin.rstd");
  b.lin_part = r("lin.part", (size_t)4 * c.rs.R, HUAL_D);
  return b;
}

struct CbBufs { std::string tag; float *c[4], *y[4], *x[5], *mean[4], *rstd[4]; uint8_t *rb[4], *kb[4]; };
CbBufs cb_bufs(const Res& r, const std::string& tag, float* x0, int R) {
  CbBufs b{};
  b.tag = tag;
  b.x[0] = x0;
  for (int i = 0; i < 4; ++i) {
    const std::string is = std::to_string(i);
    b.c[i] = r(tag + ".c" + is, R, HUAL_D); b.y[i] = r(tag + ".y" + is, R, HUAL_D);
    b.rb[i] = r.bits(tag + ".rb" + is, R); b.kb[i] = r.bits(tag + ".kb" + is, R);
    b.x[i + 1] = r(tag + ".x" + std::to_string(i + 1), R, HUAL_D);
    b.mean[i] = r(tag + ".mean" + is, R, 1); b.rstd[i] = r(tag + ".rstd" + is, R, 1);
  }
  return b;
}

void set_dmask(const Res& r, AttnJob& a, const std::string& name) {
  a.dmask = reinterpret_cast<uint8_t*>(r(name, (attn_keep_bytes(a.B, a.Tq, a.Tk) + 3) / 4, 1));
  a.stats = r(name + ".st", (size_t)2 * a.B * a.Tq * 8, 1);
}

struct DaLnBufs { float *ln1, *lnt, *mean, *rstd, *qkv, *ktvt; };
struct DaBufs {
  DaLnBufs n; float *s_att, *x_att;
  AttnJob att[4];
  float *sv, *xv, *sg, *xg, *o, *gd, *gate, *val, *mha, *res, *l2, *mean2, *rstd2, *out;
  uint8_t *kb2, *kb3, *kb4;
};
DaLnBufs da_ln_bufs(const Res& r, int li) {
  const std::string t = "da" + std::to_string(li);
  DaLnBufs n{};
  n.ln1 = r.act(t + ".ln1"); n.lnt = r.act(t + ".lnt"); n.mean = r.vec(t + ".mean"); n.rstd = r.vec(t + ".rstd");
  n.qkv = r(t + ".qkv", r.c.rs.R, 3 * HUAL_D); n.ktvt = r(t + ".ktvt", r.c.rs.R, 2 * HUAL_D);
  return n;
}
DaBufs da_bufs(const Res& r, int li) {
  const Ctx& c = r.c;
  const int D = HUAL_D, T = c.T, L = c.L, Nv = c.rs.Nv, R = c.rs.R;
  const std::string t = "da" + std::to_string(li);
  DaBufs b{};
  b.n = da_ln_bufs(r, li);
  b.s_att = r.act(t + ".s_att"); b.x_att = r.act(t + ".x_att");
  for (int k = 0; k < 4; ++k) {
    const bool cross = k & 1, qside = k >= 2, klong = qside != cross;
    AttnJob& a = b.att[k];
    attn_job_init(a);
    a.Q = b.n.qkv; a.ldq = 3 * D; a.B = c.B; a.qmask = c.rs.rowmask; a.kmask = c.rs.rowmask; a.ldo = D;
    a.K = cross ? b.n.ktvt : b.n.qkv + D; a.V = cross ? b.n.ktvt + D : b.n.qkv + 2 * D; a.ldkv = cross ? 2 * D : 3 * D;
    a.Tq = qside ? L : T; a.Tk = klong ? L : T; a.qrow0 = qside ? Nv : 0; a.krow0 = klong ? Nv : 0;
    a.O = cross ? b.x_att : b.s_att; a.drop_site = HUAL_SITE_DA + 8 * li + (cross ? 1 : 0);
    set_dmask(r, a, t + ".dm" + std::to_string(k));
  }
  b.sv = r.act(t + ".s"); b.xv = r.act(t + ".x"); b.sg = r.act(t + ".sg"); b.xg = r.act(t + ".xg"); b.o = r.act(t + ".o");
  b.gd = r.act(t + ".g"); b.gate = r.act(t + ".gate"); b.val = r.act(t + ".val"); b.mha = r.act(t + ".mha"); b.res = r.act(t + ".res");
  b.l2 = r.act(t + ".l2"); b.mean2 = r.vec(t + ".mean2"); b.rstd2 = r.vec(t + ".rstd2"); b.out = r.act(t + ".out");
  b.kb2 = r.bits(t + ".kb2", R); b.kb3 = r.bits(t + ".kb3", R); b.kb4 = r.bits(t + ".kb4", R);
  return b;
}

struct CqStage { CqBufs b; float* feats; };
CqStage cq_bufs(const Res& r, float* x) {
  const Ctx& c = r.c;
  const size_t mat = cq_mat_elems_host(c.T, c.L);
  CqStage q{};
  CqBufs& cq = q.b;
  cq.X = x;
  cq.D1W = r.act("cq.d1w"); cq.D2 = r.act("cq.d2"); cq.S0 = r.vec("cq.s0"); cq.S1 = r.vec("cq.s1");
  cq.C2Q = r.act("cq.c2q"); cq.Q2C = r.act("cq.q2c");
  cq.SR = r("cq.sr", (size_t)2 * c.B, mat); cq.SC = r("cq.sc", (size_t)2 * c.B, mat);
  cq.M2 = r("cq.m2", (size_t)2 * c.B * cq_m2_rows_host(c.T, c.L), HUAL_D);
  cq.GS = cq_fwd_global(c.B, c.T, c.L) ? r("cq.gs", (size_t)2 * c.B, mat) : nullptr;
  q.feats = r.act("cq.feats");
  return q;
}

struct FuseBufs {
  PoolArgs pool;
  AlignPool align;
  float *fuse, *outputs;
  float *probs;
  float *match_part, *d_that, *d_vhat, *align_scratch;
  float *align_rows;
};
FuseBufs fuse_bufs(const Res& r, float* cqf, const hual_labels* lab) {
  const Ctx& c = r.c;
  const int D = HUAL_D, B = c.B;
  FuseBufs f{};
  f.pool.F2 = cqf; f.pool.wp = c.p(c.pm.pool_w); f.pool.Wbot = c.p(c.pm.cqcat.k) + (size_t)D * D;
  f.pool.alpha = r("pool.alpha", B, c.L); f.pool.pooled = r("pool.pooled", B, D); f.pool.PW = r("pool.pw", B, D);
  AlignPool& ap = f.align;
  ap.F2 = cqf; ap.F1 = cqf; ap.inner = (lab && !c.dry) ? lab->inner_labels : nullptr;
  ap.tpre = r("align.tpre", B, D); ap.vpre = r("align.vpre", B, D);
  ap.that = r("align.tv", B, 2 * D); ap.vhat = ap.that + D; ap.ld = 2 * D;
  f.fuse = r.actv("fuse"); f.outputs = r.actv("outputs");
  f.probs = r("match.probs", c.rs.Nv, 4); f.match_part = r("match.part", (size_t)match_fwd_blocks(c.rs.Nv), 2);
  f.d_that = r("d.align.that", B, D); f.d_vhat = r("d.align.vhat", B, D);
  f.align_scratch = r("align.scratch", (size_t)2 * B, B); f.align_rows = r("align.rowloss", B, 1);
  return f;
}
MatchArgs match_args(const Ctx& c, const CoreBufs& k, const FuseBufs& f, const hual_labels* lab, const hual_run_opts* opt) {
  MatchArgs ma{};
  ma.fuse = f.fuse; ma.Wm = c.p(c.pm.match.k); ma.bm = c.p(c.pm.match.b); ma.E = c.p(c.pm.label_emb);
  ma.labels = (lab && !c.dry) ? lab->match_labels : nullptr;
  ma.outputs = f.outputs; ma.loss_acc = k.loss_acc;
  if (!c.cfg->no_gumbel) { ma.rng = opt->rng_state; ma.inv_tau = 1.0f / c.cfg->tau; }
  return ma;
}

struct FeBufs {
  float *x0, *a, *mean, *rstd, *qkv; uint8_t* kb4;
  CbBufs cb;
  float* att; AttnJob job; float *res, *l2, *mean2, *rstd2, *out; uint8_t *kb6, *kb7, *kb8;
};
FeBufs fe_bufs(const Res& r, int ps) {
  const Ctx& c = r.c;
  const int D = HUAL_D, Nv = c.rs.Nv;
  const std::string t = "fe" + std::to_string(ps);
  FeBufs b{};
  b.x0 = r.actv(t + ".x0"); b.a = r.actv(t + ".a");
  b.mean = r(t + ".ln1.mean", Nv, 1); b.rstd = r(t + ".ln1.rstd", Nv, 1);
  b.qkv = r(t + ".qkv", Nv, 3 * D); b.kb4 = r.bits(t + ".kb4", Nv);
  b.cb = cb_bufs(r, t, b.x0, Nv);
  b.att = r.actv(t + ".att");
  AttnJob& a = b.job;
  attn_job_init(a);
  a.Q = b.qkv; a.ldq = 3 * D; a.K = b.qkv + D; a.V = b.qkv + 2 * D; a.ldkv = 3 * D; a.O = b.att; a.ldo = D;
  a.B = c.B; a.Tq = c.T; a.Tk = c.T; a.qrow0 = 0; a.krow0 = 0; a.qmask = c.rs.rowmask; a.kmask = c.rs.rowmask;
  a.drop_site = HUAL_SITE_FE + 16 * ps + 5;
  set_dmask(r, a, t + ".dm");
  b.res = r.actv(t + ".res"); b.l2 = r.actv(t + ".l2");
  b.mean2 = r(t + ".ln2.mean", Nv, 1); b.rstd2 = r(t + ".ln2.rstd", Nv, 1);
  b.out = r.actv(t + ".out");
  b.kb6 = r.bits(t + ".kb6", Nv); b.kb7 = r.bits(t + ".kb7", Nv); b.kb8 = r.bits(t + ".kb8", Nv);
  return b;
}

struct HeadBufs { float *fn[2], *mean, *rstd, *h[2], *d_logit[2], *dz[2], *part[2], *loc_part; };
HeadBufs head_bufs(const Res& r) {
  const Ctx& c = r.c;
  const int D = HUAL_D, Nv = c.rs.Nv, B = c.B;
  HeadBufs b{};
  b.fn[0] = r.actv("head.sfn"); b.fn[1] = r.actv("head.efn");
  b.mean = r("head.mean", (size_t)2 * Nv, 1); b.rstd = r("head.rstd", (size_t)2 * Nv, 1);
  b.h[0] = r.actv("head.hs"); b.h[1] = r.actv("head.he");
  b.d_logit[0] = r("d.s_logit", B, c.T); b.d_logit[1] = r("d.e_logit", B, c.T);
  b.dz[0] = r.actv("d.head.zs"); b.dz[1] = r.actv("d.head.ze");
  b.part[0] = r("head.part.s", (size_t)B * 2, D); b.part[1] = r("head.part.e", (size_t)B * 2, D);
  b.loc_part = r("loc.part", B, 1);
  return b;
}

void fill_da_ln_proj(Ctx& c, LnProjArgs& lp, int li) {
  const int D = HUAL_D;
  const DualAttnP& d = c.pm.da[li];
  const DaLnBufs n = da_ln_bufs(Res{c, true}, li);
  lp = LnProjArgs{};
  lp.g1 = c.p(d.ln1.g); lp.b1 = c.p(d.ln1.b); lp.y1 = n.ln1; lp.drop_site1 = -1; lp.pre_site = -1;
  lp.g2 = c.p(d.lnt.g); lp.b2 = c.p(d.lnt.b); lp.y2 = n.lnt; lp.mean = n.mean; lp.rstd = n.rstd;
  lp.nproj = 5; lp.R = c.rs.R; lp.Nv = c.rs.Nv; lp.MT = ln_proj_rows(c.rs.R, c.rs.Nv); lp.drop_row0 = 0;
  const DenseP* pr[5] = {&d.query, &d.f_key, &d.f_value, &d.t_key, &d.t_value};
  float* outs[5] = {n.qkv, n.qkv + D, n.qkv + 2 * D, n.ktvt, n.ktvt + D};
  for (int k = 0; k < 5; ++k) {
    lp.wimg[k] = c.timg(pr[k]->k); lp.bias[k] = c.p(pr[k]->b); lp.out[k] = outs[k]; lp.ldo[k] = k < 3 ? 3 * D : 2 * D; lp.src[k] = k < 3 ? 0 : 1;
    lp.out_site[k] = -1;
  }
}

bool cb_no_tail() {
  static const bool no_tail = getenv("HUAL_CB_NO_TAIL") != nullptr && atoi(getenv("HUAL_CB_NO_TAIL")) != 0;
  return no_tail;
}

float* conv_block_fwd(Ctx& c, const CbBufs& b, const ConvBlockP& cp, const RowSpace& rs, int site0,
                      const float* pos_src = nullptr, const float* pos = nullptr, LnProjArgs* tail = nullptr, bool* tail_done = nullptr) {
  CbFwdArgs a{};
  a.x0 = pos_src ? pos_src : b.x[0]; a.pos = pos; a.x0_out = pos_src ? b.x[0] : nullptr;
  a.MT = conv_block_fused_rows(rs.R, rs.Nq > 0 ? rs.Nv : 0); a.drop_row0 = 0;
  for (int i = 0; i < 4; ++i) {
    CbLayerFwd& L = a.l[i];
    L.c = b.c[i];
    L.y = c.debug_taps ? b.y[i] : nullptr;
    L.relu_bits = b.rb[i]; L.keep_bits = b.kb[i]; L.xout = b.x[i + 1]; L.mean = b.mean[i]; L.rstd = b.rstd[i];
    L.ln_g = c.p(cp.ln[i].g); L.ln_b = c.p(cp.ln[i].b); L.dw = c.p(cp.dw[i]);
    L.wimg = c.timg(cp.pw[i]); L.bias = c.p(cp.b[i]);
    L.drop_site = site0 + i;
  }
  const bool fuse = tail && c.sel_stage < 0 && !cb_no_tail();
  if (tail) tail->x = b.x[4];
  if (tail_done) *tail_done = fuse;
  if (c.live()) c.chk(launch_conv_block_fwd(a, rs, c.drop, c.stream, fuse ? tail : nullptr));
  return b.x[4];
}

float* conv_block_bwd(Ctx& c, const CbBufs& b, float* dx, const ConvBlockP& cp, const RowSpace& rs) {
  const int R = rs.R;
  const std::string dt = "d." + b.tag;
  CbBwdArgs a{};
  a.dx_in = dx; a.relu_bits3 = b.rb[3]; a.keep_bits3 = b.kb[3];
  a.dx_out = c.buf(dt + ".x0", R, HUAL_D);
  a.MT = conv_block_fused_rows_bwd(R, rs.Nq > 0 ? rs.Nv : 0); a.drop_row0 = 0;
  const int nblk = conv_block_bwd_blocks(R, rs.Nq > 0 ? rs.Nv : 0);
  for (int i = 3; i >= 0; --i) {
    CbLayerBwd& L = a.l[i];
    L.ln_g = c.p(cp.ln[i].g); L.ln_b = c.p(cp.ln[i].b); L.dw = c.p(cp.dw[i]);
    L.wimg_t = c.nimg(cp.pw[i]);
    L.x = b.x[i]; L.mean = b.mean[i]; L.rstd = b.rstd[i];
    L.relu_prev = i > 0 ? b.rb[i - 1] : nullptr; L.keep_prev = i > 0 ? b.kb[i - 1] : nullptr;
    L.dz = c.buf(dt + ".z" + std::to_string(i), R, HUAL_D);
    L.dz_prev = i > 0 ? c.buf(dt + ".z" + std::to_string(i - 1), R, HUAL_D) : nullptr;
    L.part = c.buf("part." + std::to_string(c.part_seq++), (size_t)nblk * 9, HUAL_D);
    ColsumJob cj{};
    cj.src = L.part; cj.nblk = nblk; cj.nvec = 9;
    for (int k = 0; k < 7; ++k) cj.dst[k] = c.g(cp.dw[i]) + k * HUAL_D;
    cj.dst[7] = c.g(cp.ln[i].g); cj.dst[8] = c.g(cp.ln[i].b);
    if (c.active) c.colsum.push_back(cj);
    c.push_dw(mkdw(b.c[i], HUAL_D, HUAL_D, L.dz, HUAL_D, R, c.g(cp.pw[i]), c.g(cp.b[i])));
  }
  if (c.live()) c.chk(launch_conv_block_bwd(a, rs, c.drop, c.stream));
  return a.dx_out;
}


void fwd_prologue(Ctx& c, const CoreBufs& k, const InputBufs& in, EmbedArgs& ea, const hual_batch* bt, const hual_labels* lab,
                  const hual_run_opts* opt) {
  if (c.dry || !c.ok()) return;
  const ParamMap& pm = c.pm;
  std::vector<uint32_t> offs, boffs; std::vector<int> Ks; std::vector<uint8_t> needs;
  for (const auto& d : c.dense) { offs.push_back((uint32_t)d.off); Ks.push_back(d.K); boffs.push_back((uint32_t)d.boff); needs.push_back(d.need); }
  offs.push_back(c.wall_off); Ks.push_back(c.wall_K); boffs.push_back(c.wall_boff);
  needs.push_back(HUAL_PACK_T | HUAL_PACK_N);
  fill_embed_args(c, ea, bt, in.cat, c.catw(), in.char_arg, in.embed_scratch);
  PackExtra ex{};
  ex.lens = bt->video_seq_len; ex.word_ids = bt->word_ids; ex.rowmask = k.rowmask; ex.loss_acc = k.loss_acc; ex.B = c.B; ex.T = c.T; ex.L = c.L;
  ex.zero_ptr = (lab && opt->grads_prezero && opt->prezero_token) ? opt->grads_prezero : nullptr;
  ex.zero_n = (size_t)((pm.total + 3) & ~(size_t)3);
  ex.E = lab ? c.p(pm.label_emb) : nullptr; ex.lambda = c.cfg->match_lambda; ex.dE_ortho = k.ortho_dE;
  ex.gather_tasks = (c.stage_on(ST_INPUT) && c.word_table) ? embed_gather_tasks(ea, c.rs.Nq) : 0;
  ex.gather_rows = c.rs.Nq; ex.emb = ea; ex.drop = c.drop;
  ex.wall_K = c.wall_K; ex.wall_off = c.wall_off; ex.wall_boff = c.wall_boff;
  if (c.novf) { ex.ovf = k.ovf; ex.novf = c.novf; }
  c.chk(launch_pack_weights(offs.data(), Ks.data(), boffs.data(), (int)offs.size(), c.P, c.PKF, c.stream, &ex,
                            c.PKT, c.want_bwd ? c.PKN : nullptr, needs.data()));
  if (opt->prezero_token) *opt->prezero_token = (ex.zero_ptr && c.ok()) ? (uint64_t)(uintptr_t)ex.zero_ptr : 0;
}

void fwd_input(Ctx& c, const InputBufs& in, const EmbedArgs& ea, const hual_batch* bt) {
  const ParamMap& pm = c.pm;
  const int Nv = c.rs.Nv, Nq = c.rs.Nq, R = c.rs.R, D = HUAL_D, catw = c.catw();
  c.stage(ST_INPUT);
  if (!c.live()) return;
  c.chk(launch_embed_fwd(ea, Nq, c.drop, c.stream));
  if (!c.ok()) return;
  float* x = in.x0;
  if (c.ksplit) {
    const int qks = ((catw + 3) / 4 + 63) & ~63;
    float* vpart = in.lin_part;
    FkJob fj[2];
    fj[0] = FkJob{reinterpret_cast<const float*>(bt->video), c.cfg->vdim, Nv, c.cfg->vdim, c.cfg->vdim / 4,
                  reinterpret_cast<const float*>(c.PKF + pm.vconv.k * 4), vpart, (size_t)R * D, HUAL_SITE_VIDEO, 0,
                  bt->video_dtype == HUAL_DTYPE_BF16 ? 1 : 0, c.want_bwd ? in.vkeep : nullptr, (c.cfg->vdim + 7) / 8};
    fj[1] = FkJob{in.cat, catw, Nq, catw, qks, reinterpret_cast<const float*>(c.PKF + pm.qconv.k * 4),
                  vpart + (size_t)Nv * D, (size_t)R * D, -1, 0, 0, nullptr, 0};
    c.chk(launch_feature_ksplit(fj, 2, c.drop, c.stream));
    LnFwd a{};
    a.R = R; a.g1 = c.p(pm.vln.g); a.b1 = c.p(pm.vln.b); a.y1 = x; a.mean = in.lin_mean; a.rstd = in.lin_rstd;
    a.pos = c.p(pm.pos); a.row0 = 0;
    a.split = Nv; a.g1_hi = c.p(pm.qln.g); a.b1_hi = c.p(pm.qln.b);
    a.x = nullptr; a.part = vpart; a.nparts = 4; a.part_stride = (size_t)R * D; a.part_bias = c.p(pm.vconv.b);
    a.part_bias_hi = c.p(pm.qconv.b); a.x_out = in.lin;
    if (c.ok()) c.chk(launch_ln_fwd(a, c.rs, c.drop, c.stream));
    return;
  }
  const int V = c.cfg->vdim;
  MProjArgs pr[2];
  pr[0] = margs(Nv, Nq); pr[0].nsteps = 1;
  pr[0].s[0] = mstep(reinterpret_cast<const float*>(bt->video), V, std::min(V, 128), c.timg(pm.vconv.k), V, true, true);
  pr[0].s[0].a_bf16 = bt->video_dtype == HUAL_DTYPE_BF16 ? 1 : 0;
  pr[0].s[0].rep = cdiv(V, 128); pr[0].s[0].ktot = V;
  pr[0].s[0].drop_site = HUAL_SITE_VIDEO; pr[0].s[0].col0 = 0;
  pr[0].s[0].keep_out = c.want_bwd ? in.vkeep : nullptr; pr[0].s[0].ld_keep = (V + 7) / 8; pr[0].s[0].bias = c.p(pm.vconv.b);
  pr[0].ln_g = c.p(pm.vln.g); pr[0].ln_b = c.p(pm.vln.b); pr[0].pos = c.p(pm.pos); pr[0].row_in_clip0 = 0; pr[0].Tc = c.T;
  pr[0].x_out = in.lin; pr[0].y_out = x; pr[0].mean = in.lin_mean; pr[0].rstd = in.lin_rstd;
  pr[1] = margs(Nq, Nv); pr[1].nsteps = 1;
  pr[1].s[0] = mstep(in.cat, catw, std::min(catw, 128), c.timg(pm.qconv.k), catw, true, true);
  pr[1].s[0].rep = cdiv(catw, 128); pr[1].s[0].ktot = catw; pr[1].s[0].bias = c.p(pm.qconv.b);
  pr[1].ln_g = c.p(pm.qln.g); pr[1].ln_b = c.p(pm.qln.b); pr[1].pos = c.p(pm.pos); pr[1].row_in_clip0 = 0; pr[1].Tc = c.L;
  pr[1].x_out = in.lin + (size_t)Nv * D; pr[1].y_out = x + (size_t)Nv * D; pr[1].mean = in.lin_mean + Nv; pr[1].rstd = in.lin_rstd + Nv;
  c.chk(launch_mproj(pr, 2, c.drop, c.stream));
}

float* fwd_conv(Ctx& c, float* x0, bool& da_lp_done) {
  c.stage(ST_CONV);
  LnProjArgs da0_lp{};
  fill_da_ln_proj(c, da0_lp, 0);
  const CbBufs cb = cb_bufs(Res{c, true}, "cb", x0, c.rs.R);
  return conv_block_fwd(c, cb, c.pm.cb, c.rs, HUAL_SITE_CONV, nullptr, nullptr, &da0_lp, &da_lp_done);
}

float* fwd_da(Ctx& c, int li, float* x, bool& da_lp_done) {
  const DualAttnP& d = c.pm.da[li];
  const int R = c.rs.R, Nv = c.rs.Nv;
  c.stage(ST_DA, li);
  const DaBufs b = da_bufs(Res{c, true}, li);
  if (!da_lp_done) {
    LnProjArgs lp{};
    fill_da_ln_proj(c, lp, li);
    lp.x = x;
    if (c.live()) c.chk(launch_ln_proj(lp, c.drop, c.stream));
  }
  c.attn_fwd(b.att, 4);
  DaPostArgs pa{};
  pa.s_att = b.s_att; pa.x_att = b.x_att; pa.ln1 = b.n.ln1; pa.x = x; pa.rowmask = c.rs.rowmask;
  const size_t wo[11] = {d.s_dense.k, d.x_dense.k, d.s_gate.k, d.x_gate.k, d.guided.k, d.bl1_d1, d.bl1_d2, d.bl2_d1, d.bl2_d2,
                         d.dense1.k, d.dense2.k};
  const size_t bo[9] = {d.s_dense.b, d.x_dense.b, d.s_gate.b, d.x_gate.b, d.guided.b, d.bl1_b, d.bl2_b, d.dense1.b, d.dense2.b};
  for (int k = 0; k < 11; ++k) pa.w[k] = c.timg(wo[k]);
  for (int k = 0; k < 9; ++k) pa.b[k] = c.p(bo[k]);
  pa.ln2_g = c.p(d.ln2.g); pa.ln2_b = c.p(d.ln2.b);
  pa.sv = b.sv; pa.xv = b.xv; pa.sg = b.sg; pa.xg = b.xg; pa.o = b.o; pa.gd = b.gd; pa.gate = b.gate; pa.val = b.val; pa.mha = b.mha;
  pa.res = b.res; pa.l2 = b.l2; pa.out = b.out; pa.mean2 = b.mean2; pa.rstd2 = b.rstd2;
  pa.site = HUAL_SITE_DA + 8 * li; pa.R = R; pa.Nv = Nv; pa.MT = da_post_rows(R, Nv); pa.drop_row0 = 0;
  pa.bits2 = b.kb2; pa.bits3 = b.kb3; pa.bits4 = b.kb4;
  LnProjArgs nlp{};
  const bool fuse = li + 1 < c.cfg->attn_layer && c.sel_stage < 0 && !cb_no_tail();
  if (fuse) { fill_da_ln_proj(c, nlp, li + 1); nlp.x = b.out; }
  if (c.live()) c.chk(launch_da_post(pa, c.drop, c.stream, fuse ? &nlp : nullptr));
  da_lp_done = fuse;
  return b.out;
}

CqStage fwd_cq(Ctx& c, float* x) {
  const ParamMap& pm = c.pm;
  const int Nv = c.rs.Nv, Nq = c.rs.Nq, D = HUAL_D;
  c.stage(ST_CQ);
  const CqStage q = cq_bufs(Res{c, true}, x);
  CqParams cqp{};
  for (int i = 0; i < 2; ++i) { cqp.w0[i] = c.p(pm.cq[i].w0); cqp.w1[i] = c.p(pm.cq[i].w1); cqp.wm[i] = c.p(pm.cq[i].wm); }
  if (c.live()) c.chk(launch_cq_fwd(q.b, cqp, c.rs, c.drop, c.stream));
  if (c.live()) {
    MProjArgs pr[2];
    for (int sd = 0; sd < 2; ++sd) {
      const size_t ro = sd == 0 ? 0 : (size_t)Nv * D;
      pr[sd] = margs(sd == 0 ? Nv : Nq, sd == 0 ? Nq : Nv);
      pr[sd].nsteps = 4;
      const float* a1[4] = {x + ro, q.b.C2Q + ro, x + ro, x + ro};
      const float* a2[4] = {nullptr, nullptr, q.b.C2Q + ro, q.b.Q2C + ro};
      for (int p = 0; p < 4; ++p) {
        pr[sd].s[p] = mstep(a1[p], D, D, c.timg(pm.cq[sd].dense, p), D, p == 0, p == 3);
        pr[sd].s[p].A2 = a2[p]; pr[sd].s[p].lda2 = D;
      }
      mstep_out(pr[sd].s[3], q.feats + ro, D);
    }
    c.chk(launch_mproj(pr, 2, c.drop, c.stream));
  }
  return q;
}

FuseBufs fwd_fuse(Ctx& c, const CoreBufs& k, float* cqf, const hual_labels* lab, const hual_outputs* out, const hual_run_opts* opt) {
  const ParamMap& pm = c.pm;
  const int D = HUAL_D, B = c.B;
  c.stage(ST_FUSE);
  const FuseBufs f = fuse_bufs(Res{c, true}, cqf, lab);
  if (c.live()) c.chk(launch_pool_align_fwd(f.pool, lab ? &f.align : nullptr, c.rs, c.stream));
  if (c.live()) {
    MProjArgs pr = margs(c.rs.Nv); pr.nsteps = 1;
    pr.s[0] = mstep(cqf, D, D, c.timg(pm.cqcat.k), D, true, true);
    mstep_out(pr.s[0], f.fuse, D, c.p(pm.cqcat.b));
    pr.s[0].add = f.pool.PW; pr.s[0].ldadd = D; pr.s[0].add_div = c.T;
    c.chk(launch_mproj(&pr, 1, c.drop, c.stream));
  }
  if (c.live()) {
    MatchArgs ma = match_args(c, k, f, lab, opt);
    ma.probs = out->match_scores;
    ma.probs2 = lab ? f.probs : nullptr;
    ma.part = f.match_part;
    AlignSim as{f.align.that, f.align.vhat, B, f.align_scratch, f.align_scratch + (size_t)B * B, f.align_rows, f.d_that, f.d_vhat,
                k.loss_acc, 1.0f, f.align.ld, 0, B};
    c.chk(launch_match_fwd(ma, c.rs, (lab && !opt->align_external) ? &as : nullptr, c.stream));
  }
  return f;
}

void fill_fe_ln_proj(const Ctx& c, LnProjArgs& lp, const FeBufs& b, int site) {
  const ParamMap& pm = c.pm;
  const int D = HUAL_D;
  lp = LnProjArgs{};
  lp.g1 = c.p(pm.fe_ln1.g); lp.b1 = c.p(pm.fe_ln1.b); lp.y1 = b.a; lp.drop_site1 = site + 4; lp.pre_site = -1; lp.y1_bits = b.kb4;
  lp.mean = b.mean; lp.rstd = b.rstd; lp.nproj = 3; lp.R = c.rs.Nv; lp.MT = ln_proj_rows(c.rs.Nv); lp.drop_row0 = 0;
  const DenseP* pr[3] = {&pm.fe_q, &pm.fe_k, &pm.fe_v};
  for (int k = 0; k < 3; ++k) {
    lp.wimg[k] = c.timg(pr[k]->k); lp.bias[k] = c.p(pr[k]->b); lp.out[k] = b.qkv + k * D; lp.ldo[k] = 3 * D; lp.out_site[k] = -1;
  }
}

float* fwd_fe(Ctx& c, int ps, float* fin) {
  const ParamMap& pm = c.pm;
  const int D = HUAL_D, Nv = c.rs.Nv;
  const int site = HUAL_SITE_FE + 16 * ps;
  const FeBufs b = fe_bufs(Res{c, true}, ps);
  LnProjArgs lp1{};
  fill_fe_ln_proj(c, lp1, b, site);
  bool lp_done = false;
  float* f = conv_block_fwd(c, b.cb, pm.fe_cb, c.rsv, site, fin, c.p(pm.fe_pos), &lp1, &lp_done);
  if (!lp_done && c.live()) c.chk(launch_ln_proj(lp1, c.drop, c.stream));
  c.attn_fwd(&b.job, 1);
  LnProjArgs lp{};
  lp.x = f; lp.xa = b.att; lp.pre_site = site + 6; lp.x_out = b.res;
  lp.pre_bits = b.kb6; lp.y1_bits = b.kb7; lp.out_bits[0] = b.kb8;
  lp.g1 = c.p(pm.fe_ln2.g); lp.b1 = c.p(pm.fe_ln2.b); lp.y1 = b.l2; lp.drop_site1 = site + 7; lp.mean = b.mean2; lp.rstd = b.rstd2;
  lp.nproj = 1; lp.R = Nv; lp.MT = ln_proj_rows(Nv); lp.drop_row0 = 0;
  lp.wimg[0] = c.timg(pm.fe_dense.k); lp.bias[0] = c.p(pm.fe_dense.b); lp.out[0] = b.out; lp.ldo[0] = D; lp.out_site[0] = site + 8; lp.add_x[0] = 1;
  if (c.live()) c.chk(launch_ln_proj(lp, c.drop, c.stream));
  return b.out;
}

void fwd_heads(Ctx& c, const CoreBufs& k, const FuseBufs& fu, float* const feo[2], const hual_labels* lab, const hual_outputs* out,
               const hual_run_opts* opt) {
  const ParamMap& pm = c.pm;
  const int D = HUAL_D, Nv = c.rs.Nv, B = c.B;
  const HeadBufs b = head_bufs(Res{c, true});
  if (!c.live()) return;
  LnProjArgs lp2[2];
  for (int h = 0; h < 2; ++h) {
    const DenseP& hp = h == 0 ? pm.shid : pm.ehid;
    const LnP& lnp = h == 0 ? pm.sln : pm.eln;
    LnProjArgs lp{};
    lp.x = feo[h]; lp.g1 = c.p(lnp.g); lp.b1 = c.p(lnp.b); lp.y1 = b.fn[h]; lp.drop_site1 = -1; lp.pre_site = -1;
    lp.mean = b.mean + (size_t)h * Nv; lp.rstd = b.rstd + (size_t)h * Nv; lp.x2 = fu.outputs;
    lp.nproj = 2; lp.R = Nv; lp.MT = ln_proj_pair_rows(Nv); lp.drop_row0 = 0;
    lp.wimg[0] = c.timg(hp.k, 0); lp.src[0] = 0; lp.accum[0] = 1; lp.out_site[0] = -1;
    lp.wimg[1] = c.timg(hp.k, 1); lp.src[1] = 1; lp.bias[1] = c.p(hp.b);
    lp.act[1] = 1; lp.out[1] = b.h[h]; lp.ldo[1] = D; lp.out_site[1] = -1;
    lp2[h] = lp;
  }
  c.chk(launch_ln_proj_pair(lp2[0], lp2[1], c.drop, c.stream));
  if (!c.ok()) return;
  HeadsArgs ha{};
  ha.h[0] = b.h[0]; ha.h[1] = b.h[1]; ha.w[0] = c.p(pm.sdense.k); ha.w[1] = c.p(pm.edense.k); ha.b[0] = c.p(pm.sdense.b); ha.b[1] = c.p(pm.edense.b);
  ha.logit[0] = out->start_logits; ha.logit[1] = out->end_logits; ha.vmask = k.rowmask;
  ha.y1 = lab ? lab->y1 : nullptr; ha.y2 = lab ? lab->y2 : nullptr;
  ha.start_index = out->start_index; ha.end_index = out->end_index;
  ha.ds = lab ? b.d_logit[0] : nullptr; ha.de = lab ? b.d_logit[1] : nullptr;
  if (lab) { ha.dZ[0] = b.dz[0]; ha.dZ[1] = b.dz[1]; ha.part[0] = b.part[0]; ha.part[1] = b.part[1]; }
  ha.loc_part = b.loc_part; ha.inv_batch = 1.0f / (float)B;
  if (!lab && c.novf) { ha.ovf = k.ovf; ha.novf = c.novf; }
  c.chk(launch_heads(ha, B, c.T, c.stream));
  if (lab && c.ok() && !opt->deferred_loss_terms) {
    LossTailArgs lt{k.loss_acc, fu.match_part, match_fwd_blocks(Nv), b.loc_part, B, c.cfg->match_lambda, opt->match_denom_override,
                    opt->match_denom_dev, out->loss_terms, k.ovf, c.novf, opt->align_external ? nullptr : fu.align_rows, B};
    c.chk(launch_loss_tail(lt, c.stream));
  }
}

int forward_graph(Ctx& c, const hual_batch* bt, const hual_labels* lab, const hual_outputs* out, const hual_run_opts* opt) {
  c.stage(ST_ALWAYS);
  const CoreBufs core = core_bufs(Res{c, true});
  const InputBufs in = input_bufs(Res{c, true});
  EmbedArgs ea{};
  fwd_prologue(c, core, in, ea, bt, lab, opt);
  fwd_input(c, in, ea, bt);
  bool da_lp_done = false;
  float* x = fwd_conv(c, in.x0, da_lp_done);
  for (int li = 0; li < c.cfg->attn_layer; ++li) x = fwd_da(c, li, x, da_lp_done);
  const CqStage cq = fwd_cq(c, x);
  const FuseBufs fu = fwd_fuse(c, core, cq.feats, lab, out, opt);
  c.stage(ST_PRED);
  float* feo[2];
  feo[0] = fwd_fe(c, 0, fu.outputs); feo[1] = fwd_fe(c, 1, feo[0]);
  fwd_heads(c, core, fu, feo, lab, out, opt);
  return c.rc;
}


struct HeadGrads { float *d_fn[2], *d_out; };
HeadGrads bwd_heads(Ctx& c, const HeadBufs& b, float* outputs) {
  const ParamMap& pm = c.pm;
  const int D = HUAL_D, Nv = c.rs.Nv, B = c.B;
  if (c.live() && c.sel_stage >= 0) {
    HeadsArgs ha{};
    ha.grad_only = 1; ha.h[0] = b.h[0]; ha.h[1] = b.h[1]; ha.w[0] = c.p(pm.sdense.k); ha.w[1] = c.p(pm.edense.k); ha.b[0] = c.p(pm.sdense.b); ha.b[1] = c.p(pm.edense.b);
    ha.ds = b.d_logit[0]; ha.de = b.d_logit[1]; ha.dZ[0] = b.dz[0]; ha.dZ[1] = b.dz[1]; ha.part[0] = b.part[0]; ha.part[1] = b.part[1];
    c.chk(launch_heads(ha, B, c.T, c.stream));
  }
  for (int h = 0; h < 2; ++h) {
    ColsumJob cj{};
    cj.src = b.part[h]; cj.nblk = B; cj.nvec = 2; cj.last_ncols = 1;
    cj.dst[0] = c.g(h == 0 ? pm.sdense.k : pm.edense.k); cj.dst[1] = c.g(h == 0 ? pm.sdense.b : pm.edense.b);
    if (c.active) c.colsum.push_back(cj);
    const DenseP& hp = h == 0 ? pm.shid : pm.ehid;
    DwJob j = mkdw(b.fn[h], D, D, b.dz[h], D, Nv, c.g(hp.k), c.g(hp.b));
    j.npieces = 2; j.A[1] = outputs; j.lda[1] = D; j.kw[1] = D; j.dW[1] = c.g(hp.k) + (size_t)D * D;
    c.push_dw(j);
  }
  HeadGrads g{};
  g.d_fn[0] = c.actv("d.head.sfn"); g.d_fn[1] = c.actv("d.head.efn"); g.d_out = c.actv("d.outputs.heads");
  if (c.live()) {
    MProjArgs pr = margs(Nv);
    pr.nsteps = 4;
    pr.s[0] = mstep(b.dz[0], D, D, c.nimg(pm.shid.k, 0), D, true, true);     mstep_out(pr.s[0], g.d_fn[0], D);
    pr.s[1] = mstep_reuse(c.nimg(pm.shid.k, 1), D, true, false);
    pr.s[2] = mstep(b.dz[1], D, D, c.nimg(pm.ehid.k, 1), D, false, true);    mstep_out(pr.s[2], g.d_out, D);
    pr.s[3] = mstep_reuse(c.nimg(pm.ehid.k, 0), D, true, true);             mstep_out(pr.s[3], g.d_fn[1], D);
    c.chk(launch_mproj(&pr, 1, c.drop, c.stream));
  }
  return g;
}

float* bwd_fe(Ctx& c, int ps, const HeadBufs& hd, float* d_fn, float* d_in) {
  const ParamMap& pm = c.pm;
  const int D = HUAL_D, Nv = c.rs.Nv;
  const std::string dt = "d.fe" + std::to_string(ps);
  const FeBufs b = fe_bufs(Res{c, false}, ps);
  float* f = b.cb.x[4];
  float* dzd = c.actv(dt + ".zd");
  c.push_dw(mkdw(b.l2, D, D, dzd, D, Nv, c.g(pm.fe_dense.k), c.g(pm.fe_dense.b)));
  float* d_res = c.actv(dt + ".res");
  float* d_att = c.actv(dt + ".att");
  {
    LnProjBwdArgs lb{};
    const LnP& hl = ps == 1 ? pm.eln : pm.sln;
    lb.pre_x = b.out; lb.pre_mean = hd.mean + (ps == 1 ? Nv : 0); lb.pre_rstd = hd.rstd + (ps == 1 ? Nv : 0);
    lb.pre_g = c.p(hl.g); lb.pre_dy = d_fn; lb.pre_add = ps == 1 ? nullptr : d_in;
    lb.a_bits[0] = b.kb8; lb.a_save[0] = dzd;
    lb.nsteps = 1; lb.A[0] = nullptr; lb.lda[0] = D; lb.wimg_t[0] = c.nimg(pm.fe_dense.k); lb.dst[0] = 0;
    lb.dy1_bits = b.kb7; lb.x = b.res; lb.mean = b.mean2; lb.rstd = b.rstd2; lb.g1 = c.p(pm.fe_ln2.g);
    lb.dx = d_res; lb.dz = d_att; lb.dz_bits = b.kb6; lb.R = Nv; lb.drop_row0 = 0;
    c.ln_proj_bwd(lb, c.g(pm.fe_ln2.g), c.g(pm.fe_ln2.b), c.g(hl.g), c.g(hl.b));
  }
  float* d_qkv = c.buf(dt + ".qkv", Nv, 3 * D);
  AttnJob a = b.job;
  a.dO = d_att; a.lddo = D; a.dQ = d_qkv; a.lddq = 3 * D; a.dK = d_qkv + D; a.dV = d_qkv + 2 * D; a.lddkv = 3 * D;
  c.attn_bwd(&a, 1);
  const DenseP* pr[3] = {&pm.fe_q, &pm.fe_k, &pm.fe_v};
  for (int k = 0; k < 3; ++k) c.push_dw(mkdw(b.a, D, D, d_qkv + k * D, 3 * D, Nv, c.g(pr[k]->k), c.g(pr[k]->b)));
  float* d_f = c.actv(dt + ".x4");
  {
    LnProjBwdArgs lb{};
    lb.nsteps = 3;
    for (int k = 0; k < 3; ++k) { lb.A[k] = d_qkv + k * D; lb.lda[k] = 3 * D; lb.wimg_t[k] = c.nimg(pr[k]->k); lb.dst[k] = 0; }
    lb.dy1_bits = b.kb4; lb.x = f; lb.mean = b.mean; lb.rstd = b.rstd; lb.g1 = c.p(pm.fe_ln1.g); lb.add1 = d_res;
    lb.dx = d_f; lb.R = Nv; lb.drop_row0 = 0;
    c.ln_proj_bwd(lb, c.g(pm.fe_ln1.g), c.g(pm.fe_ln1.b), nullptr, nullptr);
  }
  return conv_block_bwd(c, b.cb, d_f, pm.fe_cb, c.rsv);
}

float* bwd_fuse(Ctx& c, const CoreBufs& k, const FuseBufs& f, const HeadBufs& hd, float* cqf, float* d_in, float* d_out_heads,
                const hual_labels* lab, const hual_run_opts* opt) {
  const ParamMap& pm = c.pm;
  const int D = HUAL_D, Nv = c.rs.Nv, B = c.B;
  c.stage(ST_FUSE);
  float* d_fuse = c.actv("d.fuse");
  float* match_part_b = c.buf("part." + std::to_string(c.part_seq++), (size_t)match_bwd_blocks(Nv) * 9, D);
  ColsumJob cj{};
  cj.src = match_part_b; cj.nblk = match_bwd_blocks(Nv); cj.nvec = 9; cj.last_ncols = 4;
  for (int i = 0; i < 4; ++i) { cj.dst[i] = c.g(pm.label_emb) + i * D; cj.dst[4 + i] = c.g(pm.match.k) + i * D; }
  cj.dst[8] = c.g(pm.match.b);
  if (c.active) c.colsum.push_back(cj);
  if (c.live()) {
    MatchArgs ma = match_args(c, k, f, lab, opt);
    ma.probs = f.probs;
    MatchBwd mb{};
    mb.dOut = d_in; mb.dOut2 = d_out_heads; mb.dFuse = d_fuse; mb.dWm = c.g(pm.match.k); mb.dbm = c.g(pm.match.b); mb.dE = c.g(pm.label_emb);
    mb.lambda = c.cfg->match_lambda;
    mb.dE_ortho = k.ortho_dE;
    mb.part = match_part_b;
    if (opt->deferred_loss_terms && c.sel_stage < 0) {
      mb.do_tail = 1;
      mb.tail = LossTailArgs{k.loss_acc, f.match_part, match_fwd_blocks(Nv), hd.loc_part, B, c.cfg->match_lambda,
                             opt->match_denom_override, opt->match_denom_dev, opt->deferred_loss_terms, k.ovf, c.novf,
                             opt->align_external ? nullptr : f.align_rows, B};
    }
    c.chk(launch_match_bwd(ma, mb, c.rs, c.stream));
  }
  float* d_cqf = c.act("d.cq.feats");
  c.push_dw(mkdw(cqf, D, D, d_fuse, D, Nv, c.g(pm.cqcat.k), c.g(pm.cqcat.b)));
  if (c.live()) {
    MProjArgs pr = margs(Nv); pr.nsteps = 1;
    pr.s[0] = mstep(d_fuse, D, D, c.nimg(pm.cqcat.k), D, true, true);
    mstep_out(pr.s[0], d_cqf, D);
    c.chk(launch_mproj(&pr, 1, c.drop, c.stream));
  }
  float* d_pw = c.buf("d.pool.pw", B, D);
  if (c.live()) {
    AlignPoolBwd ab{f.d_that, f.d_vhat, d_cqf, d_cqf, nullptr, nullptr, 0};
    if (!opt->align_external && c.sel_stage < 0) {
      ab.col_dq = f.align_scratch; ab.col_da = f.align_scratch + (size_t)B * B; ab.col_Bg = B;
    }
    PoolBwd pb{d_fuse, d_pw, d_cqf, c.g(pm.pool_w)};
    c.chk(launch_pool_align_bwd(f.pool, pb, f.align, ab, c.rs, c.stream));
  }
  c.push_dw(mkdw(f.pool.pooled, D, D, d_pw, D, B, c.g(pm.cqcat.k) + (size_t)D * D, nullptr));
  return d_cqf;
}

float* bwd_cq(Ctx& c, const CqStage& q, float* d_cqf) {
  const ParamMap& pm = c.pm;
  const int D = HUAL_D, Nv = c.rs.Nv, Nq = c.rs.Nq, B = c.B, T = c.T, L = c.L;
  const CqBufs& cq = q.b;
  const float* xf = cq.X;
  c.stage(ST_CQ);
  for (int s = 0; s < 2; ++s) {
    const size_t ro = s == 0 ? 0 : (size_t)Nv * D;
    DwJob j = mkdw(xf + ro, D, D, d_cqf + ro, D, s == 0 ? Nv : Nq, c.g(pm.cq[s].dense), nullptr);
    j.npieces = 4;
    const float* a1[4] = {xf + ro, cq.C2Q + ro, xf + ro, xf + ro};
    const float* a2[4] = {nullptr, nullptr, cq.C2Q + ro, cq.Q2C + ro};
    for (int p = 0; p < 4; ++p) {
      j.A[p] = a1[p]; j.A2[p] = a2[p]; j.lda[p] = D; j.lda2[p] = D; j.kw[p] = D;
      j.dW[p] = c.g(pm.cq[s].dense) + (size_t)p * D * D;
    }
    c.push_dw(j);
  }
  CqBwdBufs cg{};
  cg.dCat = nullptr; cg.ldcat = 4 * D; cg.dC2Q = c.act("d.cq.c2q"); cg.dQ2C = c.act("d.cq.q2c"); cg.dX = c.act("d.cq.x");
  if (c.live()) {
    MProjArgs pr[2];
    for (int sd = 0; sd < 2; ++sd) {
      const size_t ro = sd == 0 ? 0 : (size_t)Nv;
      pr[sd] = margs(sd == 0 ? Nv : Nq, sd == 0 ? Nq : Nv);
      pr[sd].nsteps = 4;
      for (int p = 0; p < 4; ++p) {
        const float* img = c.nimg(pm.cq[sd].dense, p);
        pr[sd].s[p] = p == 0 ? mstep(d_cqf + ro * D, D, D, img, D, true, true) : mstep_reuse(img, D, true, true);
      }
      pr[sd].quad_x = xf + ro * D; pr[sd].quad_c2q = cq.C2Q + ro * D; pr[sd].quad_q2c = cq.Q2C + ro * D;
      pr[sd].quad_dc2q = cg.dC2Q + ro * D; pr[sd].quad_dq2c = cg.dQ2C + ro * D; pr[sd].quad_dx = cg.dX + ro * D;
    }
    c.chk(launch_mproj(pr, 2, c.drop, c.stream));
  }
  cg.dD1W = c.act("d.cq.d1w"); cg.dD2 = c.act("d.cq.d2"); cg.dS0 = c.vec("d.cq.s0"); cg.dS1 = c.vec("d.cq.s1");
  cg.dM2 = c.buf("d.cq.m2", (size_t)2 * B * cq_m2_rows_host(T, L), D);
  cg.GD = cq_bwd_global(B, T, L) ? c.buf("d.cq.gd", (size_t)4 * B, cq_mat_elems_host(T, L)) : nullptr;
  float *dXa = c.act("d.cq.xa"), *dXb = c.act("d.cq.xb");
  CqParams cqp{};
  CqGrads cqg{};
  for (int i = 0; i < 2; ++i) {
    cqp.w0[i] = c.p(pm.cq[i].w0); cqp.w1[i] = c.p(pm.cq[i].w1); cqp.wm[i] = c.p(pm.cq[i].wm);
    cqg.w0[i] = c.g(pm.cq[i].w0); cqg.w1[i] = c.g(pm.cq[i].w1); cqg.wm[i] = c.g(pm.cq[i].wm);
  }
  const int tri_nv = tri_bwd_blocks_v(c.rs), tri_nq = tri_bwd_blocks_q(c.rs);
  float* tri_part = c.buf("part." + std::to_string(c.part_seq++), (size_t)(tri_nv + tri_nq) * 3, D);
  for (int side = 0; side < 2; ++side) {
    ColsumJob cj{};
    cj.src = tri_part + (side == 0 ? 0 : (size_t)tri_nv * 3 * D); cj.nblk = side == 0 ? tri_nv : tri_nq; cj.nvec = 3;
    cj.dst[0] = cqg.wm[side]; cj.dst[1] = cqg.w0[side]; cj.dst[2] = cqg.w1[1 - side];
    if (c.active) c.colsum.push_back(cj);
  }
  if (c.live()) {
    c.chk(launch_cq_bwd_impl(cq, cg, c.rs, dXa, dXb, c.stream));
    if (c.ok()) c.chk(launch_tri_bwd_impl(cq, cg, cqp, tri_part, c.rs, c.drop, dXa, dXb, c.stream));
  }
  return cg.dX;
}

float* bwd_da(Ctx& c, int li, float* dx) {
  const DualAttnP& d = c.pm.da[li];
  const int D = HUAL_D, R = c.rs.R, Nv = c.rs.Nv;
  const Res r{c, false};
  c.stage(ST_DA, li);
  const DaBufs b = da_bufs(r, li);
  float* xin = li == 0 ? r.act("cb.x4") : r.act("da" + std::to_string(li - 1) + ".out");
  const std::string dt = "d.da" + std::to_string(li);
  float* dz2 = c.act(dt + ".z2");
  c.push_dw(mkdw(b.l2, D, D, dz2, D, R, c.g(d.dense2.k), c.g(d.dense2.b)));
  float *d_res = c.act(dt + ".res"), *dz1 = c.act(dt + ".z1"), *d_sc = c.act(dt + ".sc"), *d_val = c.act(dt + ".val");
  float *d_ln1a = c.act(dt + ".ln1a"), *d_g = c.act(dt + ".g"), *dz_sg = c.act(dt + ".zsg"), *dz_xg = c.act(dt + ".zxg");
  float *d_sv = c.act(dt + ".s"), *d_xv = c.act(dt + ".x"), *d_satt = c.act(dt + ".s_att"), *d_xatt = c.act(dt + ".x_att");
  const bool dz2_ready = li < c.cfg->attn_layer - 1 && c.sel_stage < 0;
  c.push_dw(mkdw(b.mha, D, D, dz1, D, R, c.g(d.dense1.k), c.g(d.dense1.b)));
  for (int k = 0; k < 2; ++k) {
    DwJob j = mkdw(b.n.ln1, D, D, k == 0 ? d_sc : d_val, D, R, c.g(k == 0 ? d.bl1_d1 : d.bl2_d1), c.g(k == 0 ? d.bl1_b : d.bl2_b));
    j.npieces = 2; j.A[1] = b.gd; j.lda[1] = D; j.kw[1] = D; j.dW[1] = c.g(k == 0 ? d.bl1_d2 : d.bl2_d2);
    c.push_dw(j);
  }
  c.push_dw(mkdw(b.o, D, D, d_g, D, R, c.g(d.guided.k), c.g(d.guided.b)));
  c.push_dw(mkdw(b.sv, D, D, dz_sg, D, R, c.g(d.s_gate.k), c.g(d.s_gate.b)));
  c.push_dw(mkdw(b.xv, D, D, dz_xg, D, R, c.g(d.x_gate.k), c.g(d.x_gate.b)));
  c.push_dw(mkdw(b.s_att, D, D, d_sv, D, R, c.g(d.s_dense.k), c.g(d.s_dense.b)));
  c.push_dw(mkdw(b.x_att, D, D, d_xv, D, R, c.g(d.x_dense.k), c.g(d.x_dense.b)));
  {
    LnProjBwdArgs lb{};
    lb.nsteps = 1; lb.lda[0] = D; lb.wimg_t[0] = c.nimg(d.dense2.k); lb.dst[0] = 0;
    if (dz2_ready) { lb.A[0] = dz2; }
    else { lb.A[0] = dx; lb.a_bits[0] = b.kb4; lb.a_save[0] = dz2; }
    lb.dy1_bits = b.kb3; lb.x = b.res; lb.mean = b.mean2; lb.rstd = b.rstd2; lb.g1 = c.p(d.ln2.g); lb.add1 = dx;
    lb.dx = d_res; lb.dz = dz1; lb.dz_bits = b.kb2; lb.R = R; lb.Nv = Nv; lb.drop_row0 = 0;
    DaMidBwdArgs mb{};
    mb.dz1 = dz1; mb.gate = b.gate; mb.val = b.val; mb.sg = b.sg; mb.xg = b.xg; mb.sv = b.sv; mb.xv = b.xv;
    const size_t wo[10] = {d.dense1.k, d.bl1_d1, d.bl2_d1, d.bl1_d2, d.bl2_d2, d.guided.k, d.s_gate.k, d.x_gate.k, d.s_dense.k, d.x_dense.k};
    for (int k = 0; k < 10; ++k) mb.w[k] = c.nimg(wo[k]);
    mb.d_sc = d_sc; mb.d_val = d_val; mb.d_ln1a = d_ln1a; mb.d_g = d_g; mb.dz_sg = dz_sg; mb.dz_xg = dz_xg; mb.d_sv = d_sv; mb.d_xv = d_xv;
    mb.d_satt = d_satt; mb.d_xatt = d_xatt; mb.R = R; mb.Nv = Nv;
    c.ln2_mid_bwd(lb, mb, c.g(d.ln2.g), c.g(d.ln2.b));
  }
  float *dq_self = c.act(dt + ".q_self"), *dq_cross = c.act(dt + ".q_cross");
  float *d_qkv = c.buf(dt + ".qkv", R, 3 * D), *d_ktvt = c.buf(dt + ".ktvt", R, 2 * D);
  AttnJob a[4];
  for (int k = 0; k < 4; ++k) {
    const bool cross = k & 1;
    a[k] = b.att[k];
    a[k].lddo = D; a[k].lddq = D; a[k].dO = cross ? d_xatt : d_satt; a[k].dQ = cross ? dq_cross : dq_self;
    a[k].dK = cross ? d_ktvt : d_qkv + D; a[k].dV = cross ? d_ktvt + D : d_qkv + 2 * D; a[k].lddkv = cross ? 2 * D : 3 * D;
  }
  c.attn_bwd(a, 4);
  const float* As[6] = {dq_self, dq_cross, d_qkv + D, d_qkv + 2 * D, d_ktvt, d_ktvt + D};
  const int lds_[6] = {D, D, 3 * D, 3 * D, 2 * D, 2 * D};
  const DenseP* pr[6] = {&d.query, &d.query, &d.f_key, &d.f_value, &d.t_key, &d.t_value};
  for (int k = 0; k < 6; ++k) c.push_dw(mkdw(k < 4 ? b.n.ln1 : b.n.lnt, D, D, As[k], lds_[k], R, c.g(pr[k]->k), c.g(pr[k]->b)));
  float* d_xin = c.act(dt + ".in");
  float* nz = nullptr; const uint8_t* nz_bits = nullptr;
  if (li > 0) { nz = c.act("d.da" + std::to_string(li - 1) + ".z2"); nz_bits = r.bits("da" + std::to_string(li - 1) + ".kb4", R); }
  {
    LnProjBwdArgs lb{};
    lb.nsteps = 6;
    for (int k = 0; k < 6; ++k) { lb.A[k] = As[k]; lb.lda[k] = lds_[k]; lb.wimg_t[k] = c.nimg(pr[k]->k); lb.dst[k] = k < 4 ? 0 : 1; }
    lb.add_dy1 = d_ln1a; lb.x = xin; lb.mean = b.n.mean; lb.rstd = b.n.rstd; lb.g1 = c.p(d.ln1.g); lb.g2 = c.p(d.lnt.g);
    lb.add1 = d_res; lb.dx = d_xin; lb.dz = nz; lb.dz_bits = nz_bits; lb.R = R; lb.Nv = Nv; lb.drop_row0 = 0;
    c.ln_proj_bwd(lb, c.g(d.ln1.g), c.g(d.ln1.b), c.g(d.lnt.g), c.g(d.lnt.b));
  }
  return d_xin;
}

bool bwd_input(Ctx& c, const InputBufs& in, float* d_x0, float* const fe_dx0[2], const hual_batch* bt, EmbedArgs& ea, EmbedGrads& eg) {
  const ParamMap& pm = c.pm;
  const int D = HUAL_D, Nv = c.rs.Nv, Nq = c.rs.Nq, catw = c.catw();
  c.stage(ST_ALWAYS);
  PosBwdJob pj[2];
  int npj = 0;
  if (!c.dry && c.stage_on(ST_INPUT)) pj[npj++] = PosBwdJob{{d_x0, nullptr}, c.g(pm.pos), 1, 1};
  if (!c.dry && c.stage_on(ST_PRED)) pj[npj++] = PosBwdJob{{fe_dx0[1], fe_dx0[0]}, c.g(pm.fe_pos), 1, 0};
  const bool pos_rides = c.sel_stage < 0;
  if (c.live() && npj && !pos_rides) c.chk(launch_pos_bwd(pj, npj, c.rs, c.stream));
  c.stage(ST_INPUT);
  float* d_lin = c.act("d.lin");
  LnBwd a{};
  a.x = in.lin; a.mean = in.lin_mean; a.rstd = in.lin_rstd; a.R = c.rs.R; a.dy1 = d_x0; a.g1 = c.p(pm.vln.g);
  a.dx = d_lin; a.split = Nv; a.g1_hi = c.p(pm.qln.g);
  c.ln_bwd_split(a, c.g(pm.vln.g), c.g(pm.vln.b), c.g(pm.qln.g), c.g(pm.qln.b), pj, pos_rides ? npj : 0);
  DwJob j = mkdw(c.dry ? nullptr : reinterpret_cast<const float*>(bt->video), c.cfg->vdim, c.cfg->vdim, d_lin, D, Nv, c.g(pm.vconv.k), c.g(pm.vconv.b));
  j.a_drop_site = HUAL_SITE_VIDEO; j.a_drop_row0 = 0;
  j.a_bf16 = (!c.dry && bt->video_dtype == HUAL_DTYPE_BF16) ? 1 : 0;
  j.a_keep = in.vkeep; j.ld_keep = (c.cfg->vdim + 7) / 8;
  c.push_dw(j);
  c.push_dw(mkdw(in.cat, catw, catw, d_lin + (size_t)Nv * D, D, Nq, c.g(pm.qconv.k), c.g(pm.qconv.b)));
  float* d_cat = c.buf("d.cat", Nq, catw);
  if (c.live()) {
    if (cdiv(catw, 128) > MP_MAX) { c.chk(fail(-1, "invalid argument: internal: query_conv1d image")); return c.active; }
    MProjArgs pr = margs(Nq);
    pr.nsteps = cdiv(catw, 128);
    for (int p = 0; p < pr.nsteps; ++p) {
      const float* img = c.nimg(pm.qconv.k, p);
      pr.s[p] = p == 0 ? mstep(d_lin + (size_t)Nv * D, D, D, img, D, true, true) : mstep_reuse(img, D, true, true);
      mstep_out(pr.s[p], d_cat + (size_t)p * D, catw, nullptr, std::min(D, catw - p * D));
    }
    c.chk(launch_mproj(&pr, 1, c.drop, c.stream));
  }
  set_embed_scratch(ea, in.embed_scratch, Nq, c.C, c.cfg->char_dim);
  ea.word_dim = c.cfg->word_dim; ea.char_dim = c.cfg->char_dim; ea.C = c.C; ea.num_chars = c.cfg->num_chars;
  DwJob embed_dw;
  embed_dw_job(ea, Nq, &embed_dw);
  if (c.live()) {
    fill_embed_args(c, ea, bt, in.cat, catw, in.char_arg, in.embed_scratch);
    eg.dcat = d_cat; eg.lddcat = catw; eg.dunk = c.g(pm.unk); eg.dchar_table = c.g(pm.char_table);
    if (pm.word_table != (size_t)-1) { eg.dword_table = c.g(pm.word_table); eg.dword_rows = c.cfg->num_words - 2; }
    for (int i = 0; i < 4; ++i) { eg.dfilt[i] = c.g(pm.filt[i]); eg.dfbias[i] = c.g(pm.fbias[i]); }
    c.chk(launch_embed_bwd(ea, eg, Nq, c.drop, c.stream, &embed_dw, false));
  }
  c.push_dw(embed_dw);
  return c.active;
}

void bwd_flush(Ctx& c, const EmbedArgs& ea, const EmbedGrads& eg, bool input_ran) {
  c.stage(ST_ALWAYS);
  flush_dw(c);
  EmbedUnpack eu{};
  const bool unpack = !c.dry && input_ran && c.active;
  if (unpack) {
    eu.a = ea; eu.g = eg; eu.CP = embed_unpack_cpad(ea); eu.ntasks = embed_unpack_tasks(ea);
    eu.finish_blocks = embed_finish_blocks(ea, c.rs.Nq); eu.finish_lds = embed_finish_lds(ea); eu.nrows = c.rs.Nq; eu.drop = c.drop;
  }
  c.flush_colsum(unpack ? &eu : nullptr);
}

int backward_graph(Ctx& c, const hual_batch* bt, const hual_labels* lab, const hual_run_opts* opt) {
  const Res r{c, false};
  c.dwjobs.clear(); c.colsum.clear(); c.part_seq = 0;
  c.stage(ST_ALWAYS);
  const CoreBufs core = core_bufs(r);
  const InputBufs in = input_bufs(r);
  const CqStage cq = cq_bufs(r, r.act("da" + std::to_string(c.cfg->attn_layer - 1) + ".out"));
  const FuseBufs fu = fuse_bufs(r, cq.feats, lab);
  const HeadBufs hd = head_bufs(r);
  {
    const bool prezeroed = !c.dry && opt->prezero_token && *opt->prezero_token == (uint64_t)(uintptr_t)c.G && c.sel_stage < 0;
    if (!c.dry && opt->prezero_token) *opt->prezero_token = 0;
    if (c.live() && !prezeroed) c.chk(launch_zero(c.G, c.pm.total, c.stream));
  }
  c.stage(ST_PRED);
  const HeadGrads hg = bwd_heads(c, hd, fu.outputs);
  float* fe_dx0[2] = {nullptr, nullptr};
  fe_dx0[1] = bwd_fe(c, 1, hd, hg.d_fn[1], nullptr);
  fe_dx0[0] = bwd_fe(c, 0, hd, hg.d_fn[0], fe_dx0[1]);
  float* d_cqf = bwd_fuse(c, core, fu, hd, cq.feats, fe_dx0[0], hg.d_out, lab, opt);
  float* dx = bwd_cq(c, cq, d_cqf);
  for (int li = c.cfg->attn_layer - 1; li >= 0; --li) dx = bwd_da(c, li, dx);
  c.stage(ST_CONV);
  float* d_x0 = conv_block_bwd(c, cb_bufs(r, "cb", in.x0, c.rs.R), dx, c.pm.cb, c.rs);
  EmbedArgs ea{}; EmbedGrads eg{};
  const bool input_ran = bwd_input(c, in, d_x0, fe_dx0, bt, ea, eg);
  bwd_flush(c, ea, eg, input_ran);
  return c.rc;
}

int plan(Ctx& c, const hual_cfg* cfg, int B, int T, int L, int C) {
  int rc = setup_ctx(c, cfg, B, T, L, C);
  if (rc) return rc;
  c.dry = true;
  c.base = nullptr;
  hual_run_opts o{};
  rc = forward_graph(c, nullptr, nullptr, nullptr, &o);
  if (rc) return rc;
  return backward_graph(c, nullptr, nullptr, &o);
}

}

extern "C" {

int hual_seqpan_validate(const hual_cfg* cfg) {
  HUAL_REQUIRE(cfg != nullptr, "null cfg");
  return validate_cfg(*cfg);
}

#define HUAL_DW_TABLE_JOBS 256
uint64_t hual_seqpan_dw_table_bytes(void) { return 4 * dw_table_words(HUAL_DW_TABLE_JOBS); }

int hual_seqpan_param_count(const hual_cfg* cfg, uint64_t* padded_floats, uint64_t* count) {
  HUAL_REQUIRE(cfg != nullptr, "null cfg");
  ParamMap pm;
  int rc = build_param_map(*cfg, pm);
  if (rc) return rc;
  if (padded_floats) *padded_floats = pm.total;
  if (count) *count = pm.count;
  return 0;
}

int hual_seqpan_param_table(const hual_cfg* cfg, hual_param_entry* out, int max_entries) {
  HUAL_REQUIRE(cfg != nullptr, "null cfg");
  ParamMap pm;
  int rc = build_param_map(*cfg, pm);
  if (rc) return rc;
  const int n = (int)pm.entries.size();
  for (int i = 0; i < n && i < max_entries && out; ++i) {
    const ParamEntry& e = pm.entries[i];
    memset(&out[i], 0, sizeof(out[i]));
    strncpy(out[i].name, e.name.c_str(), sizeof(out[i].name) - 1);
    out[i].offset = e.off; out[i].size = e.size; out[i].ndim = e.ndim; out[i].decay = e.decay;
    for (int k = 0; k < 4; ++k) out[i].shape[k] = e.shape[k];
  }
  return n;
}

int hual_seqpan_query_workspace(const hual_cfg* cfg, int B, int T, int L, int C, uint64_t* bytes) {
  HUAL_REQUIRE(bytes != nullptr, "null bytes");
  Ctx c;
  int rc = plan(c, cfg, B, T, L, C);
  if (rc) return rc;
  *bytes = c.used + 4096;
  return 0;
}

// ... 249 lines not shown
```

Measured before the change: 53960 clips/s.

## Fuse matching head into fuse projection epilogue and ride align-sim on heads kernel

Adds a fuse_fwd kernel that runs the cqcat projection (with pooled addend) and applies the matching-head softmax, probs, CE partials and outputs in the GEMM epilogue from LDS. This removes the separate match_fwd launch and the re-read of `fuse` from HBM. The align-similarity row work moves off the match_align_fwd launch onto extra leading blocks of the heads kernel, with align_sim_rows_body adapted to 512-thread blocks. Match partial sums are now per-tile, so the loss tail's partial count changes accordingly. The cost is extra LDS and register pressure in the projection kernel and a larger heads grid.

```diff
diff --git a/hual_amd/csrc/heads.h b/hual_amd/csrc/heads.h
--- a/hual_amd/csrc/heads.h
+++ b/hual_amd/csrc/heads.h
@@ -42,6 +42,9 @@
 int match_fwd_blocks(int Nv);
 struct AlignSim;
 int launch_match_fwd(const MatchArgs& a, const RowSpace& rs, const AlignSim* as, hipStream_t s);
+struct MProjArgs;
+int fuse_fwd_tiles(int Nv);
+int launch_fuse_fwd(const MProjArgs& p, const DropCfg& drop, const MatchArgs& a, const RowSpace& rs, hipStream_t s);
 struct LossTailArgs {
   float* loss_acc; const float* match_part; int match_nblk; const float* loc_part; int loc_nblk;
   float lambda, override_denom; const float* denom_dev; float* loss_out;
@@ -74,7 +77,8 @@
   float inv_batch;
   const uint32_t* ovf; int novf;
 };
-int launch_heads(const HeadsArgs& a, int B, int T, hipStream_t s);
+struct AlignSim;
+int launch_heads(const HeadsArgs& a, int B, int T, hipStream_t s, const AlignSim* as = nullptr);
 int launch_loss_tail(const LossTailArgs& a, hipStream_t s);
 
 struct AlignPool {
diff --git a/hual_amd/csrc/heads.hip b/hual_amd/csrc/heads.hip
--- a/hual_amd/csrc/heads.hip
+++ b/hual_amd/csrc/heads.hip
@@ -1,8 +1,11 @@
 #include "heads.h"
+#include "match_row.h"
 #include "philox.h"
 #include "prof.h"
 
 using namespace hual;
+
+#include "mproj_body.h"
 
 #if defined(HUAL_STAMPS) && HUAL_STAMPS == 8
 static __device__ unsigned long long g_heads_stamps[512 * 64];
@@ -91,54 +94,15 @@
   if (on && !half) a.PW[b * HUAL_D + c] = o + part[c];
 }
 
-__device__ __forceinline__ float gumbel_noise(uint32_t w) {
-  const float u = (float)(w >> 8) * 5.9604644775390625e-08f;
-  return -logf(-logf(u + 1e-20f) + 1e-20f);
-}
 __device__ __forceinline__ void match_fwd_body(const MatchArgs& a, const RowSpace& rs, int bid, int nblk) {
   __shared__ float red[2][8];
   const int l32 = threadIdx.x & 31, grp = threadIdx.x >> 5;
   const int col = 4 * l32;
   float ce_sum = 0.f, m_sum = 0.f;
-  float4 w0 = ld4(a.Wm + (col + 0) * 4), w1 = ld4(a.Wm + (col + 1) * 4), w2 = ld4(a.Wm + (col + 2) * 4), w3 = ld4(a.Wm + (col + 3) * 4);
-  const float4 bm = ld4(a.bm);
-  float4 e0 = ld4(a.E + col), e1 = ld4(a.E + HUAL_D + col), e2 = ld4(a.E + 2 * HUAL_D + col), e3 = ld4(a.E + 3 * HUAL_D + col);
-  uint3 gk = make_uint3(0u, 0u, 0u);
-  if (a.rng) gk = make_uint3(a.rng[0], a.rng[1], a.rng[2]);
+  const MatchRowW w = match_row_weights(a, col);
   for (int row = bid * 8 + grp; row < rs.Nv; row += nblk * 8) {
-    const size_t off = (size_t)row * HUAL_D + col;
-    const float4 f = ld4(a.fuse + off);
-    float l0 = f.x * w0.x + f.y * w1.x + f.z * w2.x + f.w * w3.x;
-    float l1 = f.x * w0.y + f.y * w1.y + f.z * w2.y + f.w * w3.y;
-    float l2 = f.x * w0.z + f.y * w1.z + f.z * w2.z + f.w * w3.z;
-    float l3 = f.x * w0.w + f.y * w1.w + f.z * w2.w + f.w * w3.w;
-    l0 = half_sum32(l0) + bm.x; l1 = half_sum32(l1) + bm.y; l2 = half_sum32(l2) + bm.z; l3 = half_sum32(l3) + bm.w;
-    if (a.rng) {
-      const uint4_ r = philox4x32(0u, (uint32_t)row, (uint32_t)HUAL_SITE_GUMBEL, gk.z, gk.x, gk.y);
-      l0 = (l0 + gumbel_noise(r.x)) * a.inv_tau; l1 = (l1 + gumbel_noise(r.y)) * a.inv_tau;
-      l2 = (l2 + gumbel_noise(r.z)) * a.inv_tau; l3 = (l3 + gumbel_noise(r.w)) * a.inv_tau;
-    }
-    const float mx = fmaxf(fmaxf(l0, l1), fmaxf(l2, l3));
-    const float x0 = expf(l0 - mx), x1 = expf(l1 - mx), x2 = expf(l2 - mx), x3 = expf(l3 - mx);
-    const float sum = x0 + x1 + x2 + x3;
-    const float inv = 1.0f / sum;
-    const float p0 = x0 * inv, p1 = x1 * inv, p2 = x2 * inv, p3 = x3 * inv;
-    const float mk = rs.rowmask[row];
-    if (l32 == 0) {
-      *reinterpret_cast<float4*>(a.probs + (size_t)row * 4) = make_float4(p0, p1, p2, p3);
-      if (a.probs2) *reinterpret_cast<float4*>(a.probs2 + (size_t)row * 4) = make_float4(p0, p1, p2, p3);
-      if (a.labels) {
-        const int lab = a.labels[row];
-        const float ll = lab == 0 ? l0 : (lab == 1 ? l1 : (lab == 2 ? l2 : l3));
-        ce_sum += (mx + logf(sum) - ll) * mk;
-        m_sum += mk;
-      }
-    }
-    float4 o = make_float4((f.x + p0 * e0.x + p1 * e1.x + p2 * e2.x + p3 * e3.x) * mk,
-                           (f.y + p0 * e0.y + p1 * e1.y + p2 * e2.y + p3 * e3.y) * mk,
-                           (f.z + p0 * e0.z + p1 * e1.z + p2 * e2.z + p3 * e3.z) * mk,
-                           (f.w + p0 * e0.w + p1 * e1.w + p2 * e2.w + p3 * e3.w) * mk);
-    st4(a.outputs + off, o);
+    const float4 f = ld4(a.fuse + (size_t)row * HUAL_D + col);
+    match_row(a, w, row, l32, f, rs.rowmask[row], ce_sum, m_sum);
   }
   if (a.labels && a.loss_acc) {
     if (l32 == 0) { red[0][grp] = ce_sum; red[1][grp] = m_sum; }
@@ -277,8 +241,14 @@
   a = x; b = y; c = z;
 }
 
+__device__ __forceinline__ void align_sim_rows_body(const AlignSim& a, int i);
 template <int NR>
-__global__ __launch_bounds__(512) void heads_kernel(HeadsArgs a, int T, int B) {
+__global__ __launch_bounds__(512) void heads_kernel(HeadsArgs a, int T, int B, AlignSim as, int nsim) {
+  const int nride = xcd_round8(nsim);
+  if ((int)blockIdx.x < nride) {
+    if ((int)blockIdx.x < nsim) align_sim_rows_body(as, blockIdx.x);
+    return;
+  }
   __shared__ float zs_[256], ze_[256], ps[256], pe[256], dls[256], dle[256];
   __shared__ float sm[24];
   __shared__ double smd[16];
@@ -287,7 +257,7 @@
   __shared__ int besti[2][4];
   __shared__ float4 red[2][16][32];
   __shared__ float redb[2][16];
-  const int b = xcd_tile(blockIdx.x, gridDim.x), tid = threadIdx.x;
+  const int b = xcd_tile(blockIdx.x - nride, gridDim.x - nride), tid = threadIdx.x;
   if (b >= B) return;
   const int l32 = tid & 31, grp = tid >> 5;
   const int col = 4 * l32;
@@ -524,14 +494,15 @@
 }
 __device__ __forceinline__ void align_sim_rows_body(const AlignSim& a, int i) {
   __shared__ float ti[HUAL_D], vi[HUAL_D];
-  __shared__ double sm[4];
+  __shared__ double sm[8];
   __shared__ double sa[1024], sq[1024];
   const int tid = threadIdx.x, Bg = a.Bg;
+  const int tj = tid < 256 ? tid : Bg;
   const int ld = a.ld;
   if (tid < HUAL_D) { ti[tid] = a.that[(size_t)i * ld + tid]; vi[tid] = a.vhat[(size_t)i * ld + tid]; }
   __syncthreads();
   double mxa = -INFINITY, mxq = -INFINITY;
-  for (int j0 = 0; j0 < Bg; j0 += 64) {
+  for (int j0 = tid < 256 ? 0 : Bg; j0 < Bg; j0 += 64) {
     const int j = j0 + (tid >> 2), kq = (tid & 3) * 32;
     const float* vj = a.vhat + (size_t)min(j, Bg - 1) * ld + kq;
     double da = 0.0, dq = 0.0;
@@ -542,16 +513,16 @@
     if ((tid & 3) == 0 && j < Bg) { sa[j] = da; sq[j] = dq; }
   }
   __syncthreads();
-  for (int j = tid; j < Bg; j += 256) { mxa = fmax(mxa, sa[j]); mxq = fmax(mxq, sq[j]); }
+  for (int j = tj; j < Bg; j += 256) { mxa = fmax(mxa, sa[j]); mxq = fmax(mxq, sq[j]); }
   mxa = block_max_d(mxa, sm);
   mxq = block_max_d(mxq, sm);
   double suma = 0.0, sumq = 0.0;
-  for (int j = tid; j < Bg; j += 256) { suma += exp(sa[j] - mxa); sumq += exp(sq[j] - mxq); }
+  for (int j = tj; j < Bg; j += 256) { suma += exp(sa[j] - mxa); sumq += exp(sq[j] - mxq); }
   suma = block_sum_d(suma, sm);
   sumq = block_sum_d(sumq, sm);
   const double lsa = mxa + log(suma), lsq = mxq + log(sumq);
   double li = 0.0, dotq = 0.0, dota = 0.0;
-  for (int j = tid; j < Bg; j += 256) {
+  for (int j = tj; j < Bg; j += 256) {
     const double lpv = sa[j] - lsa, lpq = sq[j] - lsq;
     const double pv = exp(lpv), pq = exp(lpq);
     li += pq * lpq + pv * lpv - 2.0 * pq * pv;
@@ -566,7 +537,7 @@
     else if (a.loss_acc) atomicAdd(a.loss_acc + LA_ALIGN, (float)li);
   }
   __syncthreads();
-  for (int j = tid; j < Bg; j += 256) {
+  for (int j = tj; j < Bg; j += 256) {
     const double lpv = sa[j] - lsa, lpq = sq[j] - lsq;
     const double pv = exp(lpv), pq = exp(lpq);
     const double gq = pq * ((lpq + 1.0 - 2.0 * pv) - dotq) * (double)a.scale;
@@ -592,6 +563,10 @@
 __global__ __launch_bounds__(256) void match_align_fwd_kernel(MatchArgs ma, RowSpace rs, AlignSim as, int nmatch) {
   if ((int)blockIdx.x < nmatch) match_fwd_body(ma, rs, blockIdx.x, nmatch);
   else align_sim_rows_body(as, (int)blockIdx.x - nmatch);
+}
+template <int NT>
+__global__ __launch_bounds__(CB_THREADS) void fuse_fwd_kernel(MProjArgs p, DropCfg drop, MatchArgs ma, const float* rowmask) {
+  mproj_body<NT, MPF_ADD | MPF_MATCH>(p, drop, -1, &ma, rowmask);
 }
 __global__ __launch_bounds__(256) void align_sim_cols_kernel(AlignSim a) {
   __shared__ float cq[1024], ca[1024];
@@ -769,6 +744,28 @@
 }
 int match_fwd_blocks(int Nv) { return rowgrid(Nv, 512); }
 int match_bwd_blocks(int Nv) { return rowgrid(Nv, 256); }
+int fuse_fwd_tiles(int Nv) { return cdiv(Nv, mproj_rows(Nv)); }
+int launch_fuse_fwd(const MProjArgs& p, const DropCfg& drop, const MatchArgs& a, const RowSpace& rs, hipStream_t s) {
+  const MProjStep& st = p.s[0];
+  HUAL_REQUIRE(p.nsteps == 1 && p.R == rs.Nv && p.MT == mproj_rows(rs.Nv) && !p.ln_g && !p.quad_x && !p.pool_cat, "fuse_fwd: one plain step over the video rows");
+  HUAL_REQUIRE(st.A && !st.a_bf16 && !st.A2 && !st.reuse && st.rep == 1 && st.drop_site < 0 && st.first && st.last && st.kw == HUAL_D && (st.lda % 4) == 0 &&
+               st.wimg && st.wrows >= 1, "fuse_fwd: operand / weight image");
+  HUAL_REQUIRE(st.out == a.fuse && st.ldo == HUAL_D && st.ncol == HUAL_D && st.add && st.add_div >= 1, "fuse_fwd: the tile is `fuse`, with the pooled addend");
+  HUAL_REQUIRE(a.part != nullptr && a.probs && a.outputs && rs.rowmask, "fuse_fwd: matching head's tensors");
+  const int blocks = xcd_round8(fuse_fwd_tiles(rs.Nv));
+  const size_t lds = (size_t)4 * MP_ROWS * 256 + 2 * MP_ROWS * sizeof(float);
+  const int nt = (p.MT + 15) / 16;
+  const double flops = 2.0 * rs.Nv * HUAL_D * HUAL_D, bytes = (3.0 * 512.0 + 32.0) * rs.Nv + 4.0 * HUAL_D * HUAL_D;
+#define FUSE_FWD(NT)                                                                                                         \
+  do {                                                                                                                       \
+    HUAL_DYN_LDS(fuse_fwd_kernel<NT>, 96 * 1024);                                                                            \
+    HUAL_LAUNCH(flops, bytes, fuse_fwd_kernel<NT>, dim3(blocks), dim3(CB_THREADS), lds, s, p, drop, a, rs.rowmask);           \
+  } while (0)
+  if (nt <= 2) FUSE_FWD(2); else if (nt == 3) FUSE_FWD(3); else FUSE_FWD(4);
+#undef FUSE_FWD
+  HUAL_CHECK_HIP(hipGetLastError());
+  return 0;
+}
 int launch_match_fwd(const MatchArgs& a, const RowSpace& rs, const AlignSim* as, hipStream_t s) {
   HUAL_REQUIRE(a.part != nullptr, "match_fwd: partial-sum scratch");
   const int nm = match_fwd_blocks(rs.Nv);
@@ -787,14 +784,21 @@
   HUAL_CHECK_HIP(hipGetLastError());
   return 0;
 }
-int launch_heads(const HeadsArgs& a, int B, int T, hipStream_t s) {
+int launch_heads(const HeadsArgs& a, int B, int T, hipStream_t s, const AlignSim* as) {
   HUAL_REQUIRE(T >= 1 && T <= 256 && B >= 1, "heads: T <= 256");
   HUAL_REQUIRE(a.grad_only ? (a.ds && a.de && a.dZ[0]) : (a.logit[0] && a.logit[1] && a.vmask && a.start_index && a.end_index), "heads: null tensor");
   HUAL_REQUIRE(!a.h[0] || (a.h[1] && a.w[0] && a.w[1] && a.b[0] && a.b[1]), "heads: hidden layers incomplete");
   HUAL_REQUIRE(!a.dZ[0] || (a.dZ[1] && a.part[0] && a.part[1] && a.h[0]), "heads: gradient outputs incomplete");
   const double hb = (a.dZ[0] ? 4.0 : 2.0) * 512.0 * B * T + 16.0 * B * T;
-  if (T <= 128) HUAL_LAUNCH(0.0, hb, heads_kernel<8>, dim3(xcd_round8(B)), dim3(512), 0, s, a, T, B);
-  else HUAL_LAUNCH(0.0, hb, heads_kernel<16>, dim3(xcd_round8(B)), dim3(512), 0, s, a, T, B);
+  AlignSim z{};
+  int nsim = 0;
+  if (as) {
+    HUAL_REQUIRE(as->Bg >= 1 && as->Bg <= 1024 && as->ld >= HUAL_D && as->row0 == 0 && as->nrows == as->Bg, "align: global batch <= 1024");
+    z = *as; nsim = as->Bg;
+  }
+  const int grid = xcd_round8(nsim) + xcd_round8(B);
+  if (T <= 128) HUAL_LAUNCH(0.0, hb, heads_kernel<8>, dim3(grid), dim3(512), 0, s, a, T, B, z, nsim);
+  else HUAL_LAUNCH(0.0, hb, heads_kernel<16>, dim3(grid), dim3(512), 0, s, a, T, B, z, nsim);
   HUAL_CHECK_HIP(hipGetLastError());
   return 0;
 }
diff --git a/hual_amd/csrc/match_row.h b/hual_amd/csrc/match_row.h
--- /dev/null
+++ b/hual_amd/csrc/match_row.h
@@ -0,0 +1,59 @@
+#pragma once
+#include "heads.h"
+#include "philox.h"
+
+namespace hual {
+
+__device__ __forceinline__ float gumbel_noise(uint32_t w) {
+  const float u = (float)(w >> 8) * 5.9604644775390625e-08f;
+  return -logf(-logf(u + 1e-20f) + 1e-20f);
+}
+struct MatchRowW {
+  float4 w0, w1, w2, w3, bm, e0, e1, e2, e3;
+  uint3 gk;
+};
+__device__ __forceinline__ MatchRowW match_row_weights(const MatchArgs& a, int col) {
+  MatchRowW w;
+  w.w0 = ld4(a.Wm + (col + 0) * 4); w.w1 = ld4(a.Wm + (col + 1) * 4); w.w2 = ld4(a.Wm + (col + 2) * 4); w.w3 = ld4(a.Wm + (col + 3) * 4);
+  w.bm = ld4(a.bm);
+  w.e0 = ld4(a.E + col); w.e1 = ld4(a.E + HUAL_D + col); w.e2 = ld4(a.E + 2 * HUAL_D + col); w.e3 = ld4(a.E + 3 * HUAL_D + col);
+  w.gk = make_uint3(0u, 0u, 0u);
+  if (a.rng) w.gk = make_uint3(a.rng[0], a.rng[1], a.rng[2]);
+  return w;
+}
+__device__ __forceinline__ void match_row(const MatchArgs& a, const MatchRowW& w, int row, int l32, float4 f, float mk, float& ce_sum, float& m_sum) {
+  const float4 w0 = w.w0, w1 = w.w1, w2 = w.w2, w3 = w.w3, bm = w.bm, e0 = w.e0, e1 = w.e1, e2 = w.e2, e3 = w.e3;
+  const size_t off = (size_t)row * HUAL_D + 4 * l32;
+  float l0 = f.x * w0.x + f.y * w1.x + f.z * w2.x + f.w * w3.x;
+  float l1 = f.x * w0.y + f.y * w1.y + f.z * w2.y + f.w * w3.y;
+  float l2 = f.x * w0.z + f.y * w1.z + f.z * w2.z + f.w * w3.z;
+  float l3 = f.x * w0.w + f.y * w1.w + f.z * w2.w + f.w * w3.w;
+  l0 = half_sum32(l0) + bm.x; l1 = half_sum32(l1) + bm.y; l2 = half_sum32(l2) + bm.z; l3 = half_sum32(l3) + bm.w;
+  if (a.rng) {
+    const uint4_ r = philox4x32(0u, (uint32_t)row, (uint32_t)HUAL_SITE_GUMBEL, w.gk.z, w.gk.x, w.gk.y);
+    l0 = (l0 + gumbel_noise(r.x)) * a.inv_tau; l1 = (l1 + gumbel_noise(r.y)) * a.inv_tau;
+    l2 = (l2 + gumbel_noise(r.z)) * a.inv_tau; l3 = (l3 + gumbel_noise(r.w)) * a.inv_tau;
+  }
+  const float mx = fmaxf(fmaxf(l0, l1), fmaxf(l2, l3));
+  const float x0 = expf(l0 - mx), x1 = expf(l1 - mx), x2 = expf(l2 - mx), x3 = expf(l3 - mx);
+  const float sum = x0 + x1 + x2 + x3;
+  const float inv = 1.0f / sum;
+  const float p0 = x0 * inv, p1 = x1 * inv, p2 = x2 * inv, p3 = x3 * inv;
+  if (l32 == 0) {
+    *reinterpret_cast<float4*>(a.probs + (size_t)row * 4) = make_float4(p0, p1, p2, p3);
+    if (a.probs2) *reinterpret_cast<float4*>(a.probs2 + (size_t)row * 4) = make_float4(p0, p1, p2, p3);
+    if (a.labels) {
+      const int lab = a.labels[row];
+      const float ll = lab == 0 ? l0 : (lab == 1 ? l1 : (lab == 2 ? l2 : l3));
+      ce_sum += (mx + logf(sum) - ll) * mk;
+      m_sum += mk;
+    }
+  }
+  float4 o = make_float4((f.x + p0 * e0.x + p1 * e1.x + p2 * e2.x + p3 * e3.x) * mk,
+                         (f.y + p0 * e0.y + p1 * e1.y + p2 * e2.y + p3 * e3.y) * mk,
+                         (f.z + p0 * e0.z + p1 * e1.z + p2 * e2.z + p3 * e3.z) * mk,
+                         (f.w + p0 * e0.w + p1 * e1.w + p2 * e2.w + p3 * e3.w) * mk);
+  st4(a.outputs + off, o);
+}
+
+}
diff --git a/hual_amd/csrc/mproj.hip b/hual_amd/csrc/mproj.hip
--- a/hual_amd/csrc/mproj.hip
+++ b/hual_amd/csrc/mproj.hip
@@ -6,302 +6,7 @@
 
 using namespace hual;
 
-#define ld4 ld4_global
-#define st4 st4_global
-
-#define MP_ROWS 64
-enum { MPF_A2 = 1, MPF_BF16 = 2, MPF_DROP = 4, MPF_ADD = 8, MPF_LN = 16, MPF_REUSE = 32, MPF_QUAD = 64, MPF_POOL = 128 };
-
-template <int NT, int F>
-__device__ __forceinline__ void mproj_body(const MProjArgs& a, const DropCfg& drop, int tile = -1) {
-  extern __shared__ __attribute__((aligned(16))) char mp_lds[];
-  char* S0 = mp_lds;
-  char* S1 = S0 + 2 * MP_ROWS * 256;
-  float* ainv0 = reinterpret_cast<float*>(S1 + 2 * MP_ROWS * 256);
-  float* ainv1 = ainv0 + MP_ROWS;
-  const int lane = threadIdx.x & 63, wave = threadIdx.x >> 6;
-  const int l32 = threadIdx.x & 31, grp = threadIdx.x >> 5;
-  const int col = 4 * l32;
-  const int MT = a.MT, R = a.R;
-  if (tile < 0) {
-    const int nblk = xcd_round8((R + MT - 1) / MT);
-    if ((int)blockIdx.x >= nblk) return;
-    tile = xcd_tile(blockIdx.x, nblk);
-  }
-  const int r0 = tile * MT;
-  if (r0 >= R) return;
-  const int RE = min(R, r0 + MT);
-  const int j = lane & 15, g = lane >> 4, ecol = 16 * wave + 4 * g;
-  const DropRegs dr = drop_load(drop);
-  constexpr int NU = NT;
-
-  constexpr int SW = sizeof(MProjStep) / 4;
-  __shared__ uint32_t sdesc[MP_MAX * SW];
-  {
-    const uint32_t* ka = reinterpret_cast<const uint32_t*>(&a.s[0]);
-    for (int i = threadIdx.x; i < a.nsteps * SW; i += CB_THREADS) sdesc[i] = ka[i];
-  }
-  __syncthreads();
-  static_assert(SW <= 64, "a step descriptor fits one dword per lane");
-  auto step_at = [&](int si) {
-    struct alignas(8) Raw { uint32_t w[SW]; } r;
-    const uint32_t mine = sdesc[si * SW + min(lane, SW - 1)];
-#pragma unroll
-    for (int q = 0; q < SW; ++q) r.w[q] = __builtin_amdgcn_readlane(mine, q);
-    return __builtin_bit_cast(MProjStep, r);
-  };
-  int nflat = 0;
-  for (int i = 0; i < a.nsteps; ++i) nflat += (int)__builtin_amdgcn_readfirstlane(sdesc[i * SW + offsetof(MProjStep, rep) / 4]);
-  auto expand = [&](int si, int ri) {
-    MProjStep st = step_at(si);
-    if (st.rep > 1) {
-      st.A = st.a_bf16 ? (const void*)(reinterpret_cast<const uint16_t*>(st.A) + 128 * ri) : (const void*)(reinterpret_cast<const float*>(st.A) + 128 * ri);
-      st.kw = min(128, st.ktot - 128 * ri);
-      st.col0 += 128 * ri;
-      st.wimg = reinterpret_cast<const float*>(reinterpret_cast<const char*>(st.wimg) + (size_t)ri * 128 * 512);
-      st.first = st.first && ri == 0;
-      st.last = st.last && ri == st.rep - 1;
-    }
-    return st;
-  };
-  TfW wc, wn;
-  tf_load_w(wc, step_at(0).wimg, wave, lane);
-  float4 nv[NU], n2[NU];
-  auto rows_load = [&](const MProjStep& st) {
-    const int kc = min(col, max(st.kw - 4, 0));
-#pragma unroll
-    for (int u = 0; u < NU; ++u) {
-      const size_t row = (size_t)min(r0 + grp + 16 * u, R - 1);
-      if ((F & MPF_BF16) && st.a_bf16) {
-        const uint2 raw = ld2_global(reinterpret_cast<const uint16_t*>(st.A) + row * st.lda + kc);
-        nv[u] = make_float4(__uint_as_float(raw.x), __uint_as_float(raw.y), 0.f, 0.f);
-      } else {
-        nv[u] = ld4(reinterpret_cast<const float*>(st.A) + row * st.lda + kc);
-      }
-      if (F & MPF_A2) {
-        const float* p2 = st.A2 ? st.A2 : reinterpret_cast<const float*>(st.A);
-        const int ld2 = st.A2 ? st.lda2 : st.lda;
-        n2[u] = ld4(p2 + row * ld2 + kc);
-      }
-    }
-  };
-  auto fill = [&](const MProjStep& st, int slot) {
-    char* S = slot ? S1 : S0;
-    float* ai = slot ? ainv1 : ainv0;
-    const bool cin = col < st.kw;
-    uint32_t nb[4] = {15u, 15u, 15u, 15u};
-    constexpr int NPR = (NU + 1) / 2;
-    if ((F & MPF_DROP) && st.drop_site >= 0 && dr.enabled) {
-      const uint32_t c4 = (uint32_t)((st.col0 + col) >> 2);
-#pragma unroll
-      for (int pr = 0; pr < NPR; ++pr) {
-        const int lrA = grp + 32 * pr, lrB = lrA + 16;
-        const bool okA = cin && lrA < MT && r0 + lrA < RE, okB = cin && lrB < MT && r0 + lrB < RE;
-        uint32_t na, nbb;
-        const uint32_t byte = drop_nib2_r(dr, (uint32_t)st.drop_site, a.drop_row0 + (uint32_t)(r0 + lrA), a.drop_row0 + (uint32_t)(r0 + lrB), c4, na, nbb);
-        nb[2 * pr] = na; nb[2 * pr + 1] = nbb;
-        if (st.keep_out) {
-          const bool odd = (c4 & 1u) != 0u;
-          if (odd ? okB : okA) st1b_global(st.keep_out + (size_t)(r0 + (odd ? lrB : lrA)) * st.ld_keep + (c4 >> 1), (uint8_t)byte);
-        }
-      }
-    }
-#pragma unroll
-    for (int u = 0; u < NU; ++u) {
-      const int lr = grp + 16 * u, row = r0 + lr;
-      const bool ok = row < RE && cin && lr < MT;
-      float4 v = nv[u];
-      if ((F & MPF_BF16) && st.a_bf16) {
-        const uint32_t w0 = __float_as_uint(v.x), w1 = __float_as_uint(v.y);
-        v = make_float4(__uint_as_float(w0 << 16), __uint_as_float(w0 & 0xffff0000u), __uint_as_float(w1 << 16), __uint_as_float(w1 & 0xffff0000u));
-      }
-      if ((F & MPF_A2) && st.A2) v = cb_mul(v, n2[u]);
-      if (!ok) v = f4zero();
-      if ((F & MPF_DROP) && st.drop_site >= 0 && dr.enabled) v = f4_select(nb[u], make_float4(v.x * dr.scale, v.y * dr.scale, v.z * dr.scale, v.w * dr.scale));
-      const float inv = cb_store_operand(S, S + MP_ROWS * 256, lr, l32, v);
-      if (l32 == 0) ai[lr] = row < RE ? inv : 0.f;
-    }
-  };
-#define MP_STAMP(i) HUAL_STAMP_K(9, i)
-  MP_STAMP(0);
-  MProjStep cur = expand(0, 0);
-  rows_load(cur);
-  fill(cur, 0);
-  MP_STAMP(1);
-  int slot = 0, si = 0, ri = 0;
-  float4 acc[NT];
-  float4 qd[(F & MPF_QUAD) ? 4 : 1][NT];
-  float4 lastb = f4zero();
-  constexpr bool QPRE = (F & MPF_QUAD) && NT <= 3;
-  float4 qx[QPRE ? NT : 1], qc[QPRE ? NT : 1], qq[QPRE ? NT : 1];
-  if (QPRE && a.quad_x) {
-#pragma unroll
-    for (int rt = 0; rt < NT; ++rt) {
-      const size_t off = (size_t)min(r0 + 16 * rt + j, R - 1) * HUAL_D + ecol;
-      qx[rt] = ld4(a.quad_x + off); qc[rt] = ld4(a.quad_c2q + off); qq[rt] = ld4(a.quad_q2c + off);
-    }
-  }
-#pragma unroll
-  for (int rt = 0; rt < NT; ++rt) acc[rt] = f4zero();
-#pragma unroll 1
-  for (int k = 0; k < nflat; ++k) {
-    MP_STAMP(2 + 7 * k);
-    const MProjStep st = cur;
-    const bool more = k + 1 < nflat;
-    MProjStep nxt = st;
-    if (more) {
-      if (++ri == (int)__builtin_amdgcn_readfirstlane(sdesc[si * SW + offsetof(MProjStep, rep) / 4])) { ri = 0; ++si; }
-      nxt = expand(si, ri);
-    }
-    MP_STAMP(3 + 7 * k);
-    const bool closes = st.last && st.out && ecol < st.ncol;
-    const float* wdummy = st.wimg + 4 * lane;
-    const float4 bias = ld4(st.bias ? st.bias + ecol : wdummy);
-    float4 addv[NT];
-    if (F & MPF_ADD) {
-#pragma unroll
-      for (int rt = 0; rt < NT; ++rt) {
-        const int row = min(r0 + 16 * rt + j, R - 1);
-        addv[rt] = ld4((st.add && closes) ? st.add + (size_t)(row / st.add_div) * st.ldadd + ecol : wdummy);
-      }
-    }
-    tf_load_w(wn, nxt.wimg, wave, lane);
-    bool refill = true;
-    if (F & MPF_REUSE) {
-      refill = more && !nxt.reuse;
-      if (refill) rows_load(nxt);
-    } else {
-      rows_load(nxt);
-    }
-    MP_STAMP(4 + 7 * k);
-    cb_barrier();
-    MP_STAMP(5 + 7 * k);
-    const char* S = slot ? S1 : S0;
-    const float* ai = slot ? ainv1 : ainv0;
-    f32x4 accp[NT];
-    tf_mma<NT, MP_ROWS * 256>(S, wc, lane, accp);
-    MP_STAMP(6 + 7 * k);
-#pragma unroll
-    for (int rt = 0; rt < NT; ++rt) {
-      const float ir = ai[16 * rt + j];
-      const float4 o = st.first ? f4zero() : acc[rt];
-      acc[rt] = make_float4(fmaf(accp[rt][0], ir, o.x), fmaf(accp[rt][1], ir, o.y), fmaf(accp[rt][2], ir, o.z), fmaf(accp[rt][3], ir, o.w));
-    }
-    lastb = st.bias ? bias : f4zero();
-    {
-      float* outp = st.out ? st.out : const_cast<float*>(wdummy);
-#pragma unroll
-      for (int rt = 0; rt < NT; ++rt) {
-        const int row = r0 + 16 * rt + j;
-        float4 v = st.bias ? cb_add(acc[rt], bias) : acc[rt];
-        if (st.act) v = relu_nan4(v);
-        if ((F & MPF_ADD) && st.add) v = cb_add(v, addv[rt]);
-        if (closes && 16 * rt + j < MT && row < RE) st4(outp + (size_t)row * st.ldo + ecol, v);
-        if (F & MPF_QUAD) {
-#pragma unroll
-          for (int q = 0; q < 4; ++q) if (k == q) qd[q][rt] = v;
-        }
-      }
-    }
-    MP_STAMP(7 + 7 * k);
-    if (refill && more) { slot ^= 1; fill(nxt, slot); }
-    MP_STAMP(8 + 7 * k);
-    wc = wn;
-    cur = nxt;
-  }
-  if ((F & MPF_QUAD) && a.quad_x) {
-#pragma unroll
-    for (int rt = 0; rt < NT; ++rt) {
-      const int row = r0 + 16 * rt + j;
-      if (16 * rt + j >= MT || row >= RE) continue;
-      const size_t off = (size_t)row * HUAL_D + ecol;
-      const float4 x = QPRE ? qx[QPRE ? rt : 0] : ld4(a.quad_x + off), c2q = QPRE ? qc[QPRE ? rt : 0] : ld4(a.quad_c2q + off),
-                   q2c = QPRE ? qq[QPRE ? rt : 0] : ld4(a.quad_q2c + off);
-      const float4 d0 = qd[0][rt], d1 = qd[1][rt], d2 = qd[2][rt], d3 = qd[3][rt];
-      st4(a.quad_dc2q + off, make_float4(d1.x + d2.x * x.x, d1.y + d2.y * x.y, d1.z + d2.z * x.z, d1.w + d2.w * x.w));
-      st4(a.quad_dq2c + off, make_float4(d3.x * x.x, d3.y * x.y, d3.z * x.z, d3.w * x.w));
-      st4(a.quad_dx + off, make_float4(d0.x + d2.x * c2q.x + d3.x * q2c.x, d0.y + d2.y * c2q.y + d3.y * q2c.y,
-                                       d0.z + d2.z * c2q.z + d3.z * q2c.z, d0.w + d2.w * c2q.w + d3.w * q2c.w));
-    }
-    return;
-  }
-  if ((F & MPF_POOL) && a.pool_cat) {
-    const float4 bias = lastb;
-    const int C = a.pool_C;
-#pragma unroll
-    for (int rt = 0; rt < NT; ++rt) {
-      const int lr = 16 * rt + j, row = r0 + lr;
-      const int p = lr & (C - 1);
-      const float4 v4 = cb_add(acc[rt], bias);
-      const float vv[4] = {v4.x, v4.y, v4.z, v4.w};
-      float best[4];
-      int arg[4];
-#pragma unroll
-      for (int q = 0; q < 4; ++q) {
-        const int ch = ecol + q;
-        const int k = ch < 10 ? 1 : (ch < 30 ? 2 : (ch < 60 ? 3 : 4));
-        best[q] = (p + k <= C) ? vv[q] : -INFINITY;
-        arg[q] = p;
-      }
-      auto merge = [&](int step) {
-#pragma unroll
-        for (int q = 0; q < 4; ++q) {
-          const float ov = dpp_xor_partner(best[q], step);
-          const int oa = __builtin_bit_cast(int, dpp_xor_partner(__builtin_bit_cast(float, arg[q]), step));
-          const bool take = ov > best[q] || (ov == best[q] && oa < arg[q]);
-          best[q] = take ? ov : best[q];
-          arg[q] = take ? oa : arg[q];
-        }
-      };
-      if (C > 1) merge(1);
-      if (C > 2) merge(2);
-      if (C > 4) merge(4);
-      if (C > 8) merge(8);
-      if (p == 0 && lr < MT && row < RE && ecol < 100) {
-        const int word = row / C;
-        float o[4];
-        int oa[4];
-#pragma unroll
-        for (int q = 0; q < 4; ++q) {
-          const bool pos = best[q] > 0.f;
-          o[q] = pos ? best[q] : 0.f;
-          oa[q] = pos ? arg[q] : -1;
-        }
-        float* cp = a.pool_cat + (size_t)word * a.pool_ldcat + a.pool_col0 + ecol;
-        if (((a.pool_ldcat | a.pool_col0) & 3) == 0) st4(cp, make_float4(o[0], o[1], o[2], o[3]));
-        else { st1f_global(cp, o[0]); st1f_global(cp + 1, o[1]); st1f_global(cp + 2, o[2]); st1f_global(cp + 3, o[3]); }
-        st4i_global(a.pool_arg + (size_t)word * 100 + ecol, oa[0], oa[1], oa[2], oa[3]);
-      }
-    }
-    return;
-  }
-  if (!(F & MPF_LN) || !a.ln_g) return;
-  float4* D0 = reinterpret_cast<float4*>(S0);
-  cb_barrier();
-  {
-#pragma unroll
-    for (int rt = 0; rt < NT; ++rt) D0[(16 * rt + j) * 32 + (ecol >> 2)] = cb_add(acc[rt], lastb);
-  }
-  const float4 gam = ld4(a.ln_g + col), bet = ld4(a.ln_b + col);
-  cb_barrier();
-#pragma unroll
-  for (int u = 0; u < NU; ++u) {
-    const int lr = grp + 16 * u, row = r0 + lr;
-    if (lr >= MT || row >= RE) continue;
-    const float4 x = D0[lr * 32 + l32];
-    float mean, rstd;
-    const float m0 = fast_sum32(cb_hsum(x)) * (1.0f / HUAL_D);
-    const float4 d = make_float4(x.x - m0, x.y - m0, x.z - m0, x.w - m0);
-    const float var = fast_sum32(cb_hsum(cb_mul(d, d))) * (1.0f / HUAL_D);
-    mean = m0; rstd = rsqrtf(var + LN_EPS);
-    float4 y = cb_fma(make_float4(d.x * rstd, d.y * rstd, d.z * rstd, d.w * rstd), gam, bet);
-    if (a.pos) y = cb_add(y, ld4(a.pos + (size_t)((row + a.row_in_clip0) % a.Tc) * HUAL_D + col));
-    const size_t off = (size_t)row * HUAL_D + col;
-    if (a.x_out) st4(a.x_out + off, x);
-    st4(a.y_out + off, y);
-    if (l32 == 0) { st1f_global(a.mean + row, mean); st1f_global(a.rstd + row, rstd); }
-  }
-}
+#include "mproj_body.h"
 
 template <int NT, int F>
 __global__ __launch_bounds__(CB_THREADS) void mproj_kernel(MProjArgs a, DropCfg drop) { mproj_body<NT, F>(a, drop); }
@@ -317,9 +22,6 @@
   const int lo1 = mproj_pair_lo(nb1, x), n1 = mproj_pair_lo(nb1, x + 1) - lo1;
   if (sl < n1) mproj_body<NT, F>(a1, drop, lo1 + sl);
 }
-
-#undef ld4
-#undef st4
 
 #if defined(HUAL_STAMPS) && HUAL_STAMPS == 9
 extern "C" int hual_debug_stamps(unsigned long long* out, int n) {
diff --git a/hual_amd/csrc/mproj_body.h b/hual_amd/csrc/mproj_body.h
--- /dev/null
+++ b/hual_amd/csrc/mproj_body.h
@@ -0,0 +1,338 @@
+#pragma once
+#include "mproj.h"
+#include "heads.h"
+#include "match_row.h"
+#include "tilecore.h"
+#include <cstddef>
+
+#define ld4 ld4_global
+#define st4 st4_global
+
+#define MP_ROWS 64
+enum { MPF_A2 = 1, MPF_BF16 = 2, MPF_DROP = 4, MPF_ADD = 8, MPF_LN = 16, MPF_REUSE = 32, MPF_QUAD = 64, MPF_POOL = 128, MPF_MATCH = 256 };
+
+template <int NT, int F>
+__device__ __forceinline__ void mproj_body(const MProjArgs& a, const DropCfg& drop, int tile = -1, const MatchArgs* ma = nullptr,
+                                           const float* rowmask = nullptr) {
+  extern __shared__ __attribute__((aligned(16))) char mp_lds[];
+  char* S0 = mp_lds;
+  char* S1 = S0 + 2 * MP_ROWS * 256;
+  float* ainv0 = reinterpret_cast<float*>(S1 + 2 * MP_ROWS * 256);
+  float* ainv1 = ainv0 + MP_ROWS;
+  const int lane = threadIdx.x & 63, wave = threadIdx.x >> 6;
+  const int l32 = threadIdx.x & 31, grp = threadIdx.x >> 5;
+  const int col = 4 * l32;
+  const int MT = a.MT, R = a.R;
+  if (tile < 0) {
+    const int nblk = xcd_round8((R + MT - 1) / MT);
+    if ((int)blockIdx.x >= nblk) return;
+    tile = xcd_tile(blockIdx.x, nblk);
+  }
+  const int r0 = tile * MT;
+  if (r0 >= R) return;
+  const int RE = min(R, r0 + MT);
+  const int j = lane & 15, g = lane >> 4, ecol = 16 * wave + 4 * g;
+  const DropRegs dr = drop_load(drop);
+  constexpr int NU = NT;
+
+  constexpr int SW = sizeof(MProjStep) / 4;
+  __shared__ uint32_t sdesc[MP_MAX * SW];
+  {
+    const uint32_t* ka = reinterpret_cast<const uint32_t*>(&a.s[0]);
+    for (int i = threadIdx.x; i < a.nsteps * SW; i += CB_THREADS) sdesc[i] = ka[i];
+  }
+  __syncthreads();
+  static_assert(SW <= 64, "a step descriptor fits one dword per lane");
+  auto step_at = [&](int si) {
+    struct alignas(8) Raw { uint32_t w[SW]; } r;
+    const uint32_t mine = sdesc[si * SW + min(lane, SW - 1)];
+#pragma unroll
+    for (int q = 0; q < SW; ++q) r.w[q] = __builtin_amdgcn_readlane(mine, q);
+    return __builtin_bit_cast(MProjStep, r);
+  };
+  int nflat = 0;
+  for (int i = 0; i < a.nsteps; ++i) nflat += (int)__builtin_amdgcn_readfirstlane(sdesc[i * SW + offsetof(MProjStep, rep) / 4]);
+  auto expand = [&](int si, int ri) {
+    MProjStep st = step_at(si);
+    if (st.rep > 1) {
+      st.A = st.a_bf16 ? (const void*)(reinterpret_cast<const uint16_t*>(st.A) + 128 * ri) : (const void*)(reinterpret_cast<const float*>(st.A) + 128 * ri);
+      st.kw = min(128, st.ktot - 128 * ri);
+      st.col0 += 128 * ri;
+      st.wimg = reinterpret_cast<const float*>(reinterpret_cast<const char*>(st.wimg) + (size_t)ri * 128 * 512);
+      st.first = st.first && ri == 0;
+      st.last = st.last && ri == st.rep - 1;
+    }
+    return st;
+  };
+  TfW wc, wn;
+  tf_load_w(wc, step_at(0).wimg, wave, lane);
+  float4 nv[NU], n2[NU];
+  auto rows_load = [&](const MProjStep& st) {
+    const int kc = min(col, max(st.kw - 4, 0));
+#pragma unroll
+    for (int u = 0; u < NU; ++u) {
+      const size_t row = (size_t)min(r0 + grp + 16 * u, R - 1);
+      if ((F & MPF_BF16) && st.a_bf16) {
+        const uint2 raw = ld2_global(reinterpret_cast<const uint16_t*>(st.A) + row * st.lda + kc);
+        nv[u] = make_float4(__uint_as_float(raw.x), __uint_as_float(raw.y), 0.f, 0.f);
+      } else {
+        nv[u] = ld4(reinterpret_cast<const float*>(st.A) + row * st.lda + kc);
+      }
+      if (F & MPF_A2) {
+        const float* p2 = st.A2 ? st.A2 : reinterpret_cast<const float*>(st.A);
+        const int ld2 = st.A2 ? st.lda2 : st.lda;
+        n2[u] = ld4(p2 + row * ld2 + kc);
+      }
+    }
+  };
+  auto fill = [&](const MProjStep& st, int slot) {
+    char* S = slot ? S1 : S0;
+    float* ai = slot ? ainv1 : ainv0;
+    const bool cin = col < st.kw;
+    uint32_t nb[4] = {15u, 15u, 15u, 15u};
+    constexpr int NPR = (NU + 1) / 2;
+    if ((F & MPF_DROP) && st.drop_site >= 0 && dr.enabled) {
+      const uint32_t c4 = (uint32_t)((st.col0 + col) >> 2);
+#pragma unroll
+      for (int pr = 0; pr < NPR; ++pr) {
+        const int lrA = grp + 32 * pr, lrB = lrA + 16;
+        const bool okA = cin && lrA < MT && r0 + lrA < RE, okB = cin && lrB < MT && r0 + lrB < RE;
+        uint32_t na, nbb;
+        const uint32_t byte = drop_nib2_r(dr, (uint32_t)st.drop_site, a.drop_row0 + (uint32_t)(r0 + lrA), a.drop_row0 + (uint32_t)(r0 + lrB), c4, na, nbb);
+        nb[2 * pr] = na; nb[2 * pr + 1] = nbb;
+        if (st.keep_out) {
+          const bool odd = (c4 & 1u) != 0u;
+          if (odd ? okB : okA) st1b_global(st.keep_out + (size_t)(r0 + (odd ? lrB : lrA)) * st.ld_keep + (c4 >> 1), (uint8_t)byte);
+        }
+      }
+    }
+#pragma unroll
+    for (int u = 0; u < NU; ++u) {
+      const int lr = grp + 16 * u, row = r0 + lr;
+      const bool ok = row < RE && cin && lr < MT;
+      float4 v = nv[u];
+      if ((F & MPF_BF16) && st.a_bf16) {
+        const uint32_t w0 = __float_as_uint(v.x), w1 = __float_as_uint(v.y);
+        v = make_float4(__uint_as_float(w0 << 16), __uint_as_float(w0 & 0xffff0000u), __uint_as_float(w1 << 16), __uint_as_float(w1 & 0xffff0000u));
+      }
+      if ((F & MPF_A2) && st.A2) v = cb_mul(v, n2[u]);
+      if (!ok) v = f4zero();
+      if ((F & MPF_DROP) && st.drop_site >= 0 && dr.enabled) v = f4_select(nb[u], make_float4(v.x * dr.scale, v.y * dr.scale, v.z * dr.scale, v.w * dr.scale));
+      const float inv = cb_store_operand(S, S + MP_ROWS * 256, lr, l32, v);
+      if (l32 == 0) ai[lr] = row < RE ? inv : 0.f;
+    }
+  };
+#define MP_STAMP(i) HUAL_STAMP_K(9, i)
+  MP_STAMP(0);
+  MProjStep cur = expand(0, 0);
+  rows_load(cur);
+  fill(cur, 0);
+  MP_STAMP(1);
+  int slot = 0, si = 0, ri = 0;
+  float4 acc[NT];
+  float4 qd[(F & MPF_QUAD) ? 4 : 1][NT];
+  float4 lastb = f4zero();
+  float4 vlast[(F & MPF_MATCH) ? NT : 1];
+  constexpr bool QPRE = (F & MPF_QUAD) && NT <= 3;
+  float4 qx[QPRE ? NT : 1], qc[QPRE ? NT : 1], qq[QPRE ? NT : 1];
+  if (QPRE && a.quad_x) {
+#pragma unroll
+    for (int rt = 0; rt < NT; ++rt) {
+      const size_t off = (size_t)min(r0 + 16 * rt + j, R - 1) * HUAL_D + ecol;
+      qx[rt] = ld4(a.quad_x + off); qc[rt] = ld4(a.quad_c2q + off); qq[rt] = ld4(a.quad_q2c + off);
+    }
+  }
+#pragma unroll
+  for (int rt = 0; rt < NT; ++rt) acc[rt] = f4zero();
+#pragma unroll 1
+  for (int k = 0; k < nflat; ++k) {
+    MP_STAMP(2 + 7 * k);
+    const MProjStep st = cur;
+    const bool more = k + 1 < nflat;
+    MProjStep nxt = st;
+    if (more) {
+      if (++ri == (int)__builtin_amdgcn_readfirstlane(sdesc[si * SW + offsetof(MProjStep, rep) / 4])) { ri = 0; ++si; }
+      nxt = expand(si, ri);
+    }
+    MP_STAMP(3 + 7 * k);
+    const bool closes = st.last && st.out && ecol < st.ncol;
+    const float* wdummy = st.wimg + 4 * lane;
+    const float4 bias = ld4(st.bias ? st.bias + ecol : wdummy);
+    float4 addv[NT];
+    if (F & MPF_ADD) {
+#pragma unroll
+      for (int rt = 0; rt < NT; ++rt) {
+        const int row = min(r0 + 16 * rt + j, R - 1);
+        addv[rt] = ld4((st.add && closes) ? st.add + (size_t)(row / st.add_div) * st.ldadd + ecol : wdummy);
+      }
+    }
+    tf_load_w(wn, nxt.wimg, wave, lane);
+    bool refill = true;
+    if (F & MPF_REUSE) {
+      refill = more && !nxt.reuse;
+      if (refill) rows_load(nxt);
+    } else {
+      rows_load(nxt);
+    }
+    MP_STAMP(4 + 7 * k);
+    cb_barrier();
+    MP_STAMP(5 + 7 * k);
+    const char* S = slot ? S1 : S0;
+    const float* ai = slot ? ainv1 : ainv0;
+    f32x4 accp[NT];
+    tf_mma<NT, MP_ROWS * 256>(S, wc, lane, accp);
+    MP_STAMP(6 + 7 * k);
+#pragma unroll
+    for (int rt = 0; rt < NT; ++rt) {
+      const float ir = ai[16 * rt + j];
+      const float4 o = st.first ? f4zero() : acc[rt];
+      acc[rt] = make_float4(fmaf(accp[rt][0], ir, o.x), fmaf(accp[rt][1], ir, o.y), fmaf(accp[rt][2], ir, o.z), fmaf(accp[rt][3], ir, o.w));
+    }
+    lastb = st.bias ? bias : f4zero();
+    {
+      float* outp = st.out ? st.out : const_cast<float*>(wdummy);
+#pragma unroll
+      for (int rt = 0; rt < NT; ++rt) {
+        const int row = r0 + 16 * rt + j;
+        float4 v = st.bias ? cb_add(acc[rt], bias) : acc[rt];
+        if (st.act) v = relu_nan4(v);
+        if ((F & MPF_ADD) && st.add) v = cb_add(v, addv[rt]);
+        if (closes && 16 * rt + j < MT && row < RE) st4(outp + (size_t)row * st.ldo + ecol, v);
+        if (F & MPF_MATCH) vlast[rt] = v;
+        if (F & MPF_QUAD) {
+#pragma unroll
+          for (int q = 0; q < 4; ++q) if (k == q) qd[q][rt] = v;
+        }
+      }
+    }
+    MP_STAMP(7 + 7 * k);
+    if (refill && more) { slot ^= 1; fill(nxt, slot); }
+    MP_STAMP(8 + 7 * k);
+    wc = wn;
+    cur = nxt;
+  }
+  if ((F & MPF_QUAD) && a.quad_x) {
+#pragma unroll
+    for (int rt = 0; rt < NT; ++rt) {
+      const int row = r0 + 16 * rt + j;
+      if (16 * rt + j >= MT || row >= RE) continue;
+      const size_t off = (size_t)row * HUAL_D + ecol;
+      const float4 x = QPRE ? qx[QPRE ? rt : 0] : ld4(a.quad_x + off), c2q = QPRE ? qc[QPRE ? rt : 0] : ld4(a.quad_c2q + off),
+                   q2c = QPRE ? qq[QPRE ? rt : 0] : ld4(a.quad_q2c + off);
+      const float4 d0 = qd[0][rt], d1 = qd[1][rt], d2 = qd[2][rt], d3 = qd[3][rt];
+      st4(a.quad_dc2q + off, make_float4(d1.x + d2.x * x.x, d1.y + d2.y * x.y, d1.z + d2.z * x.z, d1.w + d2.w * x.w));
+      st4(a.quad_dq2c + off, make_float4(d3.x * x.x, d3.y * x.y, d3.z * x.z, d3.w * x.w));
+      st4(a.quad_dx + off, make_float4(d0.x + d2.x * c2q.x + d3.x * q2c.x, d0.y + d2.y * c2q.y + d3.y * q2c.y,
+                                       d0.z + d2.z * c2q.z + d3.z * q2c.z, d0.w + d2.w * c2q.w + d3.w * q2c.w));
+    }
+    return;
+  }
+  if ((F & MPF_POOL) && a.pool_cat) {
+    const float4 bias = lastb;
+    const int C = a.pool_C;
+#pragma unroll
+    for (int rt = 0; rt < NT; ++rt) {
+      const int lr = 16 * rt + j, row = r0 + lr;
+      const int p = lr & (C - 1);
+      const float4 v4 = cb_add(acc[rt], bias);
+      const float vv[4] = {v4.x, v4.y, v4.z, v4.w};
+      float best[4];
+      int arg[4];
+#pragma unroll
+      for (int q = 0; q < 4; ++q) {
+        const int ch = ecol + q;
+        const int k = ch < 10 ? 1 : (ch < 30 ? 2 : (ch < 60 ? 3 : 4));
+        best[q] = (p + k <= C) ? vv[q] : -INFINITY;
+        arg[q] = p;
+      }
+      auto merge = [&](int step) {
+#pragma unroll
+        for (int q = 0; q < 4; ++q) {
+          const float ov = dpp_xor_partner(best[q], step);
+          const int oa = __builtin_bit_cast(int, dpp_xor_partner(__builtin_bit_cast(float, arg[q]), step));
+          const bool take = ov > best[q] || (ov == best[q] && oa < arg[q]);
+          best[q] = take ? ov : best[q];
+          arg[q] = take ? oa : arg[q];
+        }
+      };
+      if (C > 1) merge(1);
+      if (C > 2) merge(2);
+      if (C > 4) merge(4);
+      if (C > 8) merge(8);
+      if (p == 0 && lr < MT && row < RE && ecol < 100) {
+        const int word = row / C;
+        float o[4];
+        int oa[4];
+#pragma unroll
+        for (int q = 0; q < 4; ++q) {
+          const bool pos = best[q] > 0.f;
+          o[q] = pos ? best[q] : 0.f;
+          oa[q] = pos ? arg[q] : -1;
+        }
+        float* cp = a.pool_cat + (size_t)word * a.pool_ldcat + a.pool_col0 + ecol;
+        if (((a.pool_ldcat | a.pool_col0) & 3) == 0) st4(cp, make_float4(o[0], o[1], o[2], o[3]));
+        else { st1f_global(cp, o[0]); st1f_global(cp + 1, o[1]); st1f_global(cp + 2, o[2]); st1f_global(cp + 3, o[3]); }
+        st4i_global(a.pool_arg + (size_t)word * 100 + ecol, oa[0], oa[1], oa[2], oa[3]);
+      }
+    }
+    return;
+  }
+  if (F & MPF_MATCH) {
+    float4* D0 = reinterpret_cast<float4*>(S0);
+    __shared__ float mred[2][CB_THREADS / 32];
+    const MatchRowW mw = match_row_weights(*ma, col);
+    float mk[NU];
+#pragma unroll
+    for (int u = 0; u < NU; ++u) mk[u] = rowmask[min(r0 + grp + 16 * u, R - 1)];
+    cb_barrier();
+#pragma unroll
+    for (int rt = 0; rt < NT; ++rt) D0[(16 * rt + j) * 32 + (ecol >> 2)] = vlast[rt];
+    cb_barrier();
+    float ce_sum = 0.f, m_sum = 0.f;
+#pragma unroll
+    for (int u = 0; u < NU; ++u) {
+      const int lr = grp + 16 * u, row = r0 + lr;
+      if (lr >= MT || row >= RE) continue;
+      match_row(*ma, mw, row, l32, D0[lr * 32 + l32], mk[u], ce_sum, m_sum);
+    }
+    if (ma->labels && ma->loss_acc) {
+      if (l32 == 0) { mred[0][grp] = ce_sum; mred[1][grp] = m_sum; }
+      __syncthreads();
+      if (threadIdx.x == 0) {
+        float cs = 0.f, ms = 0.f;
+        for (int i = 0; i < CB_THREADS / 32; ++i) { cs += mred[0][i]; ms += mred[1][i]; }
+        ma->part[2 * tile] = cs; ma->part[2 * tile + 1] = ms;
+      }
+    }
+    return;
+  }
+  if (!(F & MPF_LN) || !a.ln_g) return;
+  float4* D0 = reinterpret_cast<float4*>(S0);
+  cb_barrier();
+  {
+#pragma unroll
+    for (int rt = 0; rt < NT; ++rt) D0[(16 * rt + j) * 32 + (ecol >> 2)] = cb_add(acc[rt], lastb);
+  }
+  const float4 gam = ld4(a.ln_g + col), bet = ld4(a.ln_b + col);
+  cb_barrier();
+#pragma unroll
+  for (int u = 0; u < NU; ++u) {
+    const int lr = grp + 16 * u, row = r0 + lr;
+    if (lr >= MT || row >= RE) continue;
+    const float4 x = D0[lr * 32 + l32];
+    float mean, rstd;
+    const float m0 = fast_sum32(cb_hsum(x)) * (1.0f / HUAL_D);
+    const float4 d = make_float4(x.x - m0, x.y - m0, x.z - m0, x.w - m0);
+    const float var = fast_sum32(cb_hsum(cb_mul(d, d))) * (1.0f / HUAL_D);
+    mean = m0; rstd = rsqrtf(var + LN_EPS);
+    float4 y = cb_fma(make_float4(d.x * rstd, d.y * rstd, d.z * rstd, d.w * rstd), gam, bet);
+    if (a.pos) y = cb_add(y, ld4(a.pos + (size_t)((row + a.row_in_clip0) % a.Tc) * HUAL_D + col));
+    const size_t off = (size_t)row * HUAL_D + col;
+    if (a.x_out) st4(a.x_out + off, x);
+    st4(a.y_out + off, y);
+    if (l32 == 0) { st1f_global(a.mean + row, mean); st1f_global(a.rstd + row, rstd); }
+  }
+}
+
+#undef ld4
+#undef st4
diff --git a/hual_amd/csrc/prof.cpp b/hual_amd/csrc/prof.cpp
--- a/hual_amd/csrc/prof.cpp
+++ b/hual_amd/csrc/prof.cpp
@@ -96,6 +96,7 @@
       {"conv_block_", HUAL_PIPE_MATRIX16, 3}, {"ln_proj", HUAL_PIPE_MATRIX16, 3}, {"da_post", HUAL_PIPE_MATRIX16, 3},
       {"da_mid_bwd", HUAL_PIPE_MATRIX16, 3},  {"ln2_mid_bwd", HUAL_PIPE_MATRIX16, 3}, {"mproj_", HUAL_PIPE_MATRIX16, 3},
       {"feature_", HUAL_PIPE_MATRIX16, 3},    {"dw_f16_", HUAL_PIPE_MATRIX16, 3},
+      {"fuse_fwd", HUAL_PIPE_MATRIX16, 3},
       {"attn_", HUAL_PIPE_MATRIX16, 3},      {"cq_fwd_staged", HUAL_PIPE_MATRIX16, 3}, {"cq_bwd_staged", HUAL_PIPE_MATRIX16, 3},
       {"cq_fwd_wide", HUAL_PIPE_MATRIX16, 3}, {"cq_bwd_wide", HUAL_PIPE_MATRIX16, 3},
       {"cq_", HUAL_PIPE_MATRIX32, 1},
diff --git a/hual_amd/csrc/seqpan.hip b/hual_amd/csrc/seqpan.hip
--- a/hual_amd/csrc/seqpan.hip
+++ b/hual_amd/csrc/seqpan.hip
@@ -394,6 +394,14 @@
   float *match_part, *d_that, *d_vhat, *align_scratch;
   float *align_rows;
 };
+bool fuse_stage_fused(const Ctx& c) {
+#ifndef HUAL_NO_FUSE_STAGE_FUSE
+  return c.sel_stage < 0;
+#else
+  return false;
+#endif
+}
+int match_part_pairs(const Ctx& c) { return fuse_stage_fused(c) ? fuse_fwd_tiles(c.rs.Nv) : match_fwd_blocks(c.rs.Nv); }
 FuseBufs fuse_bufs(const Res& r, float* cqf, const hual_labels* lab) {
   const Ctx& c = r.c;
   const int D = HUAL_D, B = c.B;
@@ -405,7 +413,7 @@
   ap.tpre = r("align.tpre", B, D); ap.vpre = r("align.vpre", B, D);
   ap.that = r("align.tv", B, 2 * D); ap.vhat = ap.that + D; ap.ld = 2 * D;
   f.fuse = r.actv("fuse"); f.outputs = r.actv("outputs");
-  f.probs = r("match.probs", c.rs.Nv, 4); f.match_part = r("match.part", (size_t)match_fwd_blocks(c.rs.Nv), 2);
+  f.probs = r("match.probs", c.rs.Nv, 4); f.match_part = r("match.part", (size_t)std::max(match_fwd_blocks(c.rs.Nv), fuse_fwd_tiles(c.rs.Nv)), 2);
   f.d_that = r("d.align.that", B, D); f.d_vhat = r("d.align.vhat", B, D);
   f.align_scratch = r("align.scratch", (size_t)2 * B, B); f.align_rows = r("align.rowloss", B, 1);
   return f;
@@ -674,11 +682,20 @@
   c.stage(ST_FUSE);
   const FuseBufs f = fuse_bufs(Res{c, true}, cqf, lab);
   if (c.live()) c.chk(launch_pool_align_fwd(f.pool, lab ? &f.align : nullptr, c.rs, c.stream));
+  const bool fused = fuse_stage_fused(c);
   if (c.live()) {
     MProjArgs pr = margs(c.rs.Nv); pr.nsteps = 1;
     pr.s[0] = mstep(cqf, D, D, c.timg(pm.cqcat.k), D, true, true);
     mstep_out(pr.s[0], f.fuse, D, c.p(pm.cqcat.b));
     pr.s[0].add = f.pool.PW; pr.s[0].ldadd = D; pr.s[0].add_div = c.T;
+    if (fused) {
+      MatchArgs ma = match_args(c, k, f, lab, opt);
+      ma.probs = out->match_scores;
+      ma.probs2 = lab ? f.probs : nullptr;
+      ma.part = f.match_part;
+      c.chk(launch_fuse_fwd(pr, c.drop, ma, c.rs, c.stream));
+      return f;
+    }
     c.chk(launch_mproj(&pr, 1, c.drop, c.stream));
   }
   if (c.live()) {
@@ -756,9 +773,11 @@
   if (lab) { ha.dZ[0] = b.dz[0]; ha.dZ[1] = b.dz[1]; ha.part[0] = b.part[0]; ha.part[1] = b.part[1]; }
   ha.loc_part = b.loc_part; ha.inv_batch = 1.0f / (float)B;
   if (!lab && c.novf) { ha.ovf = k.ovf; ha.novf = c.novf; }
-  c.chk(launch_heads(ha, B, c.T, c.stream));
+  AlignSim as{fu.align.that, fu.align.vhat, B, fu.align_scratch, fu.align_scratch + (size_t)B * B, fu.align_rows, fu.d_that, fu.d_vhat,
+              k.loss_acc, 1.0f, fu.align.ld, 0, B};
+  c.chk(launch_heads(ha, B, c.T, c.stream, (fuse_stage_fused(c) && lab && !opt->align_external) ? &as : nullptr));
   if (lab && c.ok() && !opt->deferred_loss_terms) {
-    LossTailArgs lt{k.loss_acc, fu.match_part, match_fwd_blocks(Nv), b.loc_part, B, c.cfg->match_lambda, opt->match_denom_override,
+    LossTailArgs lt{k.loss_acc, fu.match_part, match_part_pairs(c), b.loc_part, B, c.cfg->match_lambda, opt->match_denom_override,
                     opt->match_denom_dev, out->loss_terms, k.ovf, c.novf, opt->align_external ? nullptr : fu.align_rows, B};
     c.chk(launch_loss_tail(lt, c.stream));
   }
@@ -879,7 +898,7 @@
     mb.part = match_part_b;
     if (opt->deferred_loss_terms && c.sel_stage < 0) {
       mb.do_tail = 1;
-      mb.tail = LossTailArgs{k.loss_acc, f.match_part, match_fwd_blocks(Nv), hd.loc_part, B, c.cfg->match_lambda,
+      mb.tail = LossTailArgs{k.loss_acc, f.match_part, match_part_pairs(c), hd.loc_part, B, c.cfg->match_lambda,
                              opt->match_denom_override, opt->match_denom_dev, opt->deferred_loss_terms, k.ovf, c.novf,
                              opt->align_external ? nullptr : f.align_rows, B};
     }
```

New measurement: 54340 clips/s (median of 6 runs). About the same (+0.7%).
